# Huangtianyu-caas/MAGOT

Measured on AMD Instinct MI355X. Metric: CDS bases extracted+translated/sec, higher is better.
Workload: dtype u8

## Files before the change

include/magot.h:

```cpp
#ifndef MAGOT_H
#define MAGOT_H

#include <stdint.h>

#ifdef __cplusplus
extern "C" {
#endif

#define MAGOT_ABI_VERSION 1

enum magot_status {
  MAGOT_OK = 0,
  MAGOT_ERR_ARG = -1,
  MAGOT_ERR_HIP = -2,
  MAGOT_ERR_RANGE = -3,
  MAGOT_ERR_STATE = -4,
  MAGOT_ERR_UNSUPPORTED = -5
};

#define MAGOT_OUT_NUC 1u
#define MAGOT_OUT_PEP 2u
#define MAGOT_OUT_GENOME_ORDER 4u

typedef struct magot_exon {
  uint64_t start_rc;
  uint32_t contig;
  uint32_t len;
} magot_exon;

typedef struct magot_tx {
  uint64_t exon_begin;
  uint32_t n_exons;
  uint32_t flags;
} magot_tx;

typedef struct magot_ctx magot_ctx;
typedef struct magot_genome magot_genome;
typedef struct magot_plan magot_plan;

int magot_abi_version(void);

const char* magot_last_error(void);

int magot_device_count(void);

int magot_ctx_create(int device, magot_ctx** out);
void magot_ctx_destroy(magot_ctx* ctx);

int magot_genome_load(magot_ctx* ctx, const uint8_t* const* seqs, const uint64_t* lens,
                      uint32_t n_contigs, magot_genome** out);
#define MAGOT_PACK_HOST 1u
int magot_genome_load_ex(magot_ctx* ctx, const uint8_t* const* seqs, const uint64_t* lens,
                         uint32_t n_contigs, uint32_t flags, magot_genome** out);
int magot_genome_load_fasta(magot_ctx* ctx, const char* text, uint64_t len, int truncate_names,
                            magot_genome** out);
int magot_genome_contigs(const magot_genome* g, uint32_t* n, uint64_t* lens, char* names,
                         uint64_t names_cap, uint64_t* names_len);
int magot_fasta_read(const char* text, uint64_t len, int truncate_names, uint32_t* n,
                     uint64_t* lens, char* names, uint64_t names_cap, uint64_t* names_len,
                     uint8_t* seqs, uint64_t seqs_cap);

int magot_cds_scan(const char* text, uint64_t len, uint64_t* n_seg, uint64_t* seq_bytes,
                   uint64_t* seg_off, uint64_t* hdr_off, uint64_t* hdr_len, uint8_t* seq,
                   uint64_t seq_cap);
int magot_cds_render(const char* text, uint64_t n_seg, const uint64_t* seg_off,
                     const uint64_t* hdr_off, const uint64_t* hdr_len, const uint8_t* pep,
                     const uint64_t* poff, const int64_t* codons, uint8_t* out, uint64_t cap,
                     uint64_t* out_len);

int magot_genome_stats(const magot_genome* g, uint64_t* total_bases, uint64_t* n_exc_runs,
                       uint64_t* device_bytes);
void magot_genome_destroy(magot_genome* g);

int magot_genome_export(const magot_genome* g, uint8_t* meta, uint64_t cap, uint64_t* meta_len,
                        uint64_t* arena_bytes);
int magot_genome_copy_arena(const magot_genome* g, void* dst_dev);
int magot_genome_attach(magot_ctx* ctx, const uint8_t* meta, uint64_t meta_len, void* arena_dev,
                        magot_genome** out);
int magot_genome_wire_ranges(const magot_genome* g, uint64_t* off, uint64_t* len, uint32_t* n);
int magot_genome_attach_wire(magot_ctx* ctx, const uint8_t* meta, uint64_t meta_len,
                             void* arena_dev, magot_genome** out);
int magot_genome_wire_export(const magot_genome* g, void* wire_dev, uint64_t cap,
                             uint64_t* wire_bytes);
int magot_genome_wire_import(magot_ctx* ctx, const uint8_t* meta, uint64_t meta_len,
                             const void* wire_dev, uint64_t wire_bytes, magot_genome** out);

int magot_copy_segments(magot_ctx* ctx, const void* src_dev, uint64_t src_bytes, void* dst_dev,
                        const uint64_t* src_off, const uint64_t* dst_off, uint64_t n);

int magot_plan_create(magot_ctx* ctx, const magot_genome* g, const magot_exon* exons,
                      uint64_t n_exons, const magot_tx* txs, uint64_t n_tx, uint32_t outputs,
                      magot_plan** out, uint64_t* nuc_bytes, uint64_t* pep_bytes);
void magot_plan_destroy(magot_plan* p);

int magot_plan_execute(magot_ctx* ctx, magot_plan* p);

int magot_ctx_sync(magot_ctx* ctx);

int magot_ctx_mark(magot_ctx* ctx, int which);
int magot_ctx_elapsed(magot_ctx* ctx, double* ms);

int magot_ctx_info(const magot_ctx* ctx, int* n_cu, int* extract_blocks_per_cu);

int magot_plan_fetch(magot_ctx* ctx, magot_plan* p, uint8_t* nuc_out, uint64_t* nuc_off,
                     uint8_t* pep_out, uint64_t* pep_off);

int magot_run(magot_ctx* ctx, magot_plan* p, uint8_t* nuc_out, uint64_t* nuc_off,
              uint8_t* pep_out, uint64_t* pep_off);

int magot_plan_time(magot_ctx* ctx, magot_plan* p, int iters, double* avg_ms);
int magot_plan_time_b2b(magot_ctx* ctx, magot_plan* p, int iters, double* avg_ms);

int magot_plan_copy_outputs(magot_ctx* ctx, magot_plan* p, void* nuc_dst_dev, void* pep_dst_dev);

int magot_plan_device_outputs(magot_plan* p, void** nuc_dev, void** pep_dev);

int magot_plan_layout(const magot_plan* p, uint64_t* nuc_start, uint64_t* pep_start);

uint64_t magot_plan_algorithmic_bytes(const magot_plan* p);

int magot_debug_tile_blocks(const uint64_t* ex_g, const uint64_t* ex_out, const uint64_t* tx_nuc,
                            const uint64_t* tx_pep, uint64_t span, uint32_t lane_chunks,
                            const void* tiles, uint64_t n_tiles, uint32_t* geometry, void* blocks,
                            uint64_t* ovf_ex, uint64_t ovf_ex_cap, int64_t* ovf_tx,
                            uint64_t ovf_tx_cap, uint64_t* n_ovf);

int magot_debug_tile_cut(const uint64_t* ex_out, uint64_t n_ex, const uint64_t* tx_nuc,
                         const uint64_t* tx_pep, uint64_t n_rec, uint32_t lane_chunks, void* tiles,
                         uint64_t tiles_cap, uint64_t* n_tiles);

int magot_debug_orf6_tiles(const uint64_t* noff, uint64_t n_rec, const uint64_t* row_start,
                           uint64_t n_rows, uint64_t* t0, uint32_t* r0, uint32_t* e0, uint32_t* m,
                           uint64_t tiles_cap, uint64_t* n_tiles);

int magot_debug_plan(const uint8_t* const* seqs, const uint64_t* lens, uint32_t n_contigs,
                     const magot_exon* exons, uint64_t n_exons, const magot_tx* txs, uint64_t n_tx,
                     uint32_t outputs, uint64_t* info, uint64_t* ex_g, uint64_t* ex_out,
                     uint64_t* tx_nuc, uint64_t* tx_pep, uint64_t* lay_nuc, uint64_t* lay_pep,
                     void* tiles);

int magot_debug_text_index(magot_ctx* ctx, const uint8_t* text, uint64_t len, uint64_t index_len,
                           uint32_t byte, int32_t second_byte, uint64_t* pos_out, uint64_t* n_out,
                           uint64_t* second_count_out);

int magot_debug_text_lines(magot_ctx* ctx, const uint8_t* text, uint64_t len, uint64_t index_len,
                           int check_cr, uint32_t stray_reason, uint64_t* pos_out,
                           uint64_t* n_lines_out, uint64_t* stray_out);

int magot_debug_piece_copy(magot_ctx* ctx, const uint8_t* base, uint64_t base_len,
                           const uint64_t* src, const uint64_t* dst, const uint32_t* len,
                           uint64_t n, uint8_t* out, uint64_t out_len);

#define MAGOT_NO_RECORD 0xFFFFFFFFu
typedef struct magot_text_unit {
  uint64_t text_off;
  uint32_t text_len;
  uint32_t rec;
} magot_text_unit;
int magot_debug_text_assembly(magot_ctx* ctx, const magot_text_unit* units, uint64_t n,
                              const uint8_t* text, uint64_t text_len, const uint64_t* rspan,
                              uint64_t n_rec, const uint8_t* pay, uint64_t pay_len, int protein,
                              uint8_t* out, uint64_t out_len, uint64_t* written);

int magot_revcomp_batch(magot_ctx* ctx, const uint8_t* seqs, const uint64_t* seq_off, uint64_t n,
                        uint8_t* out);

int magot_translate_sizes(const uint64_t* seq_off, uint64_t n, const int32_t* frames,
                          uint64_t* pep_off, int64_t* codons_out);
int magot_translate_batch(magot_ctx* ctx, const uint8_t* seqs, const uint64_t* seq_off, uint64_t n,
                          const int32_t* frames, const uint8_t* strands, const uint8_t* lut64,
                          const uint64_t* pep_off, uint8_t* out);

int magot_revcomp(magot_ctx* ctx, const uint8_t* seq, uint64_t len, uint8_t* out);
int magot_translate(magot_ctx* ctx, const uint8_t* seq, uint64_t len, int frame, int strand,
                    int trimX, uint8_t* out, int64_t* out_len);

int magot_codon_symbols(magot_ctx* ctx, const uint8_t* seq, uint64_t n_codons,
                        const uint8_t* class256, uint32_t n_classes, const uint8_t* lut,
                        uint8_t* out);

int magot_orf6_sizes(const uint64_t* seq_off, uint64_t n, uint64_t* stream_off,
                     uint64_t* stream_len, uint8_t* none_mask);
int magot_orf6_batch(magot_ctx* ctx, const uint8_t* seqs, const uint64_t* seq_off, uint64_t n,
                     const uint8_t* lut64, const uint64_t* stream_off, uint8_t* out);
int magot_debug_orf6_batch(magot_ctx* ctx, const uint8_t* seqs, const uint64_t* seq_off, uint64_t n,
                           const uint8_t* lut64, const uint64_t* stream_off, uint8_t* out,
                           int32_t poison);
typedef struct magot_orf6 magot_orf6;
int magot_plan_orf6(magot_ctx* ctx, magot_plan* p, const uint8_t* lut64, magot_orf6** out,
                    uint64_t* total_res);
int magot_orf6_execute(magot_ctx* ctx, magot_orf6* o);
int magot_orf6_poison(magot_ctx* ctx, magot_orf6* o, uint8_t byte);
int magot_orf6_fetch(magot_ctx* ctx, magot_orf6* o, uint8_t* out, uint64_t* stream_off,
                     uint64_t* stream_len);
int magot_orf6_copy_outputs(magot_ctx* ctx, magot_orf6* o, void* dst_dev);
int magot_orf6_time(magot_ctx* ctx, magot_orf6* o, int iters, double* avg_ms);
int magot_orf6_time_b2b(magot_ctx* ctx, magot_orf6* o, int iters, double* avg_ms);
void magot_orf6_destroy(magot_orf6* o);

#define MAGOT_ORF_FROM_ATG 1u
#define MAGOT_ORF_LONGEST 2u
#define MAGOT_ORF_REC_NONE 1u
#define MAGOT_ORF_REC_NO_LONGEST 2u
typedef struct magot_orfcall magot_orfcall;
uint32_t magot_orfcall_tile(void);
int magot_orfcall_create(magot_ctx* ctx, magot_orf6* o, uint32_t flags, magot_orfcall** out,
                         uint64_t* n_orfs, uint64_t* payload_bytes);
int magot_orfcall_fetch(magot_ctx* ctx, magot_orfcall* c, uint32_t* record, uint8_t* stream,
                        uint32_t* start, uint32_t* length, uint64_t* payload_off,
                        uint8_t* payload, uint8_t* record_flags);
int magot_orfcall_text(magot_ctx* ctx, magot_orfcall* c, const uint64_t* name_off,
                       const uint8_t* names, uint64_t* out_len);
int magot_orfcall_text_fetch(magot_ctx* ctx, magot_orfcall* c, uint8_t* out, uint64_t cap);
int magot_orfcall_time(magot_ctx* ctx, magot_orfcall* c, int text, int iters, double* avg_ms);
void magot_orfcall_destroy(magot_orfcall* c);

typedef struct magot_longorf magot_longorf;
int magot_longorf_create(magot_ctx* ctx, magot_plan* p, const uint8_t* lut64, magot_longorf** out);
int magot_longorf_execute(magot_ctx* ctx, magot_longorf* h, uint64_t* payload_bytes);
int magot_longorf_fetch(magot_ctx* ctx, magot_longorf* h, uint8_t* stream, uint32_t* start,
                        uint32_t* length, uint64_t* payload_off, uint8_t* payload,
                        uint8_t* record_flags);
int magot_longorf_text(magot_ctx* ctx, magot_longorf* h, const uint64_t* name_off,
                       const uint8_t* names, uint64_t n_print, uint64_t* out_len);
int magot_longorf_text_fetch(magot_ctx* ctx, magot_longorf* h, uint8_t* out, uint64_t cap);
int magot_longorf_time(magot_ctx* ctx, magot_longorf* h, int text, int iters, double* avg_ms);
int magot_longorf_params(magot_ctx* ctx, const magot_longorf* h, uint32_t* step, uint64_t* waves);
void magot_longorf_destroy(magot_longorf* h);

#define MAGOT_GFF_PROTEIN 1u
#define MAGOT_GFF_ORDER_PY2 2u
#define MAGOT_GFF_LONGEST 4u
#define MAGOT_GFF_GENOMIC 8u
#define MAGOT_GFF_FROM_EXONS 16u
#define MAGOT_GFF_FOR_WRITE 32u
typedef struct magot_gffplan magot_gffplan;
int magot_gff_plan(const char* gff, uint64_t gff_len, const char* const* seqids,
                   const uint64_t* contig_lens, uint32_t n_contigs, const char* feature,
                   uint32_t flags, magot_gffplan** out, uint64_t* n_exons, uint64_t* n_tx);
int magot_gff_read(const char* gff, uint64_t gff_len, uint32_t flags, magot_gffplan** out);
int magot_gff_lower(magot_gffplan* p, const char* const* seqids, const uint64_t* contig_lens,
                    uint32_t n_contigs, const char* feature, uint32_t flags, uint64_t* n_exons,
                    uint64_t* n_tx);
#define MAGOT_CDS_NAMES_CDS 0u
#define MAGOT_CDS_NAMES_TRANSCRIPT 1u
#define MAGOT_CDS_NAMES_GENE 2u
int magot_gff_lower_cds(magot_gffplan* p, const char* const* seqids, const uint64_t* contig_lens,
                        uint32_t n_contigs, const char* const* filters, uint32_t n_filters,
                        const int64_t* length_filter, uint32_t names_from, uint32_t flags,
                        uint64_t* n_rec, uint64_t* n_groups);
int magot_gffplan_cds_views(const magot_gffplan* p, const uint64_t** name_off,
                            const uint8_t** names, const uint64_t** group_off);
int magot_flank_plan(const char* gff, uint64_t gff_len, const char* const* seqids,
                     const uint64_t* contig_lens, uint32_t n_contigs, const char* feature_type,
                     const char* namefrom, const char* sequence_length, const char* stream,
                     magot_gffplan** out, uint64_t* n_exons, uint64_t* n_tx);
int magot_gffplan_tables(const magot_gffplan* p, magot_exon* exons, magot_tx* txs);
int magot_gffplan_table_views(const magot_gffplan* p, const magot_exon** exons,
                              const magot_tx** txs);
int magot_gffplan_render(const magot_gffplan* p, const uint8_t* nuc, const uint64_t* noff,
                         const uint8_t* pep, const uint64_t* poff, uint8_t* out, uint64_t cap,
                         uint64_t* out_len);
int magot_gffplan_selections(const magot_gffplan* p, uint64_t* n_groups);
void magot_gffplan_destroy(magot_gffplan* p);

typedef struct magot_fasta_text magot_fasta_text;
int magot_fasta_text_create(magot_ctx* ctx, const magot_gffplan* gp, const magot_plan* p,
                            magot_fasta_text** out, uint64_t* max_bytes);
int magot_fasta_text_execute(magot_ctx* ctx, magot_fasta_text* t);
int magot_fasta_text_fetch(magot_ctx* ctx, magot_fasta_text* t, uint8_t* out, uint64_t cap,
                           uint64_t* out_len);
int magot_fasta_text_time(magot_ctx* ctx, magot_fasta_text* t, int iters, double* avg_ms);
void magot_fasta_text_destroy(magot_fasta_text* t);

#define MAGOT_MASK_HARD 1u
#define MAGOT_MASK_KEEP_CASE 2u
typedef struct magot_mask_interval {
  uint32_t contig;
  uint32_t start;
  uint32_t len;
} magot_mask_interval;
typedef struct magot_maskplan magot_maskplan;
typedef struct magot_mask magot_mask;
uint32_t magot_mask_piece(void);
int magot_mask_plan(const char* gff, uint64_t gff_len, const char* const* seqids,
                    const uint64_t* contig_lens, uint32_t n_contigs, const char* feature_type,
                    uint32_t flags, magot_maskplan** out, uint64_t* n_intervals);
int magot_maskplan_table(const magot_maskplan* p, const magot_mask_interval** rows,
                         uint64_t* n_intervals, uint32_t* flags);
void magot_maskplan_destroy(magot_maskplan* p);
int magot_mask_fasta_check(const char* text, uint64_t len, uint32_t n_contigs);
int magot_mask_create(magot_ctx* ctx, const magot_plan* p, const magot_maskplan* mp,
                      const uint32_t* rec_contig, const uint64_t* name_off, const uint8_t* names,
                      magot_mask** out, uint64_t* text_bytes);
int magot_mask_execute(magot_ctx* ctx, magot_mask* m);
int magot_mask_fetch(magot_ctx* ctx, magot_mask* m, uint8_t* out, uint64_t cap);
int magot_mask_coverage_fetch(magot_ctx* ctx, magot_mask* m, uint32_t* words, uint64_t cap_words,
                              uint64_t* n_words);
int magot_mask_time(magot_ctx* ctx, magot_mask* m, int iters, double* paint_ms, double* text_ms);
void magot_mask_destroy(magot_mask* m);

#define MAGOT_TRACK_GC 1u
#define MAGOT_TRACK_REPLACE 2u
typedef struct magot_track magot_track;
typedef struct magot_track_windows magot_track_windows;
uint32_t magot_track_rank_block(void);
int magot_track_create(magot_ctx* ctx, const magot_genome* g, magot_track** out,
                       uint64_t* n_words);
int magot_track_base_class(magot_ctx* ctx, magot_track* t, const magot_genome* g, uint32_t flags);
int magot_track_paint(magot_ctx* ctx, magot_track* t, const magot_mask_interval* rows,
                      uint64_t n_rows, int value);
int magot_track_set_bytes(magot_ctx* ctx, magot_track* t, uint32_t contig, const uint8_t* bytes,
                          uint64_t len);
int magot_track_get_bytes(magot_ctx* ctx, magot_track* t, uint32_t contig, uint8_t* bytes,
                          uint64_t len);
int magot_track_fetch(magot_ctx* ctx, magot_track* t, uint32_t* words, uint64_t cap_words,
                      uint64_t* n_words);
int magot_track_windows_create(magot_ctx* ctx, magot_track* t, uint64_t window, uint64_t jump,
                               const uint8_t* skip, magot_track_windows** out,
                               uint64_t* n_windows, uint64_t* first);
int magot_track_windows_fetch(magot_ctx* ctx, magot_track_windows* w, uint32_t* sums,
                              uint64_t cap);
int magot_track_transitions(magot_ctx* ctx, magot_track_windows* w, uint32_t s_min, uint64_t* n);
int magot_track_transitions_fetch(magot_ctx* ctx, magot_track_windows* w, uint64_t* index,
                                  uint64_t cap);
int magot_track_count(magot_ctx* ctx, magot_track* t, const magot_mask_interval* rows,
                      uint64_t n_rows, uint32_t* ones);
int magot_track_time(magot_ctx* ctx, magot_track* t, magot_track_windows* w, uint32_t s_min,
                     int iters, double* ms5);
void magot_track_windows_destroy(magot_track_windows* w);
void magot_track_destroy(magot_track* t);

#define MAGOT_DEPTH_EMPTY_LINE 1u
#define MAGOT_DEPTH_LEADING_BLANK 2u
#define MAGOT_DEPTH_BAD_BYTE 3u
#define MAGOT_DEPTH_NAME_LONG 4u
#define MAGOT_DEPTH_FEW_FIELDS 5u
#define MAGOT_DEPTH_SIGN 6u
#define MAGOT_DEPTH_NOT_NUMBER 7u
#define MAGOT_DEPTH_NUMBER_RANGE 8u
#define MAGOT_DEPTH_POS_SEQUENCE 9u
#define MAGOT_DEPTH_REPEATED_CONTIG 10u
#define MAGOT_DEPTH_LINE_LONG 11u
#define MAGOT_DEPTH_TOO_MANY_LINES 12u
#define MAGOT_DEPTH_TOO_MANY_RUNS 13u
typedef struct magot_depth magot_depth;
uint32_t magot_depth_block(void);
int magot_depth_parse(magot_ctx* ctx, const char* text, uint64_t len, uint64_t chunk_bytes,
                      uint32_t max_runs, magot_depth** out, uint64_t* n_lines, uint64_t* n_runs,
                      uint32_t* reason, uint64_t* line);
int magot_depth_runs(const magot_depth* t, uint64_t* first, uint64_t* offset, uint32_t* name_len,
                     uint64_t cap);
int magot_depth_values(magot_ctx* ctx, magot_depth* t, uint64_t start, uint64_t n, int32_t* out);
int magot_depth_sums(magot_ctx* ctx, magot_depth* t, const int64_t* start, const int64_t* length,
                     uint64_t n_rows, const uint64_t* group_offsets, uint64_t n_groups,
                     int64_t* sums, int64_t* group_sums);
int magot_depth_time(magot_ctx* ctx, magot_depth* t, int iters, double* ms4,
                     uint64_t* chunk_len);
void magot_depth_destroy(magot_depth* t);

typedef struct magot_fq magot_fq;
uint64_t magot_fq_dense(void);
int magot_fq_parse(magot_ctx* ctx, const char* text, uint64_t len, uint64_t chunk_bytes,
                   magot_fq** out);
int magot_fq_stats(const magot_fq* t, uint64_t* out8, uint32_t* flags);
int magot_fq_histogram(magot_ctx* ctx, magot_fq* t, int64_t* lengths, uint64_t* counts,
                       uint64_t cap, uint64_t* n);
int magot_fq_time(magot_ctx* ctx, magot_fq* t, int iters, double* ms4, uint64_t* chunk_len);
void magot_fq_destroy(magot_fq* t);

#define MAGOT_OVERLAP_NO_SEQ 0xffffffffu
enum {
  MAGOT_OVERLAP_BAD_INT_FIRST = 1,
  MAGOT_OVERLAP_BAD_INT_SECOND = 2,
  MAGOT_OVERLAP_COORD_RANGE = 3,
  MAGOT_OVERLAP_SEQIDS = 4
};
typedef struct magot_overlap magot_overlap;
typedef struct magot_ovplan magot_ovplan;
void magot_overlap_coord_range(int64_t* lo, int64_t* hi);
uint32_t magot_overlap_lane_scan(void);
int magot_overlap_create(magot_ctx* ctx, const uint32_t* seq, const int64_t* p0, const int64_t* p1,
                         uint64_t n, uint32_t n_seq, magot_overlap** out);
int magot_overlap_purge(magot_ctx* ctx, magot_overlap* h, const uint32_t* seq, const int64_t* c0,
                        const int64_t* c1, uint64_t n, uint8_t* drop);
int magot_overlap_counts(magot_ctx* ctx, magot_overlap* h, const uint32_t* seq, const int64_t* q0,
                         const int64_t* q1, uint64_t n, int64_t* counts);
int magot_overlap_time(magot_ctx* ctx, magot_overlap* h, int iters, double* ms6,
                       uint64_t* copy_bytes);
void magot_overlap_destroy(magot_overlap* h);
int magot_overlap_plan(const char* gff1, uint64_t len1, const char* gff2, uint64_t len2,
                       magot_ovplan** out, uint32_t* reason);
int magot_ovplan_table(const magot_ovplan* p, int which, uint64_t* n_lines, uint32_t* n_seq,
                       const uint8_t** flag, const uint32_t** seq, const int64_t** c0,
                       const int64_t** c1, const uint64_t** off, const uint64_t** len);
int magot_ovplan_render(const magot_ovplan* p, const char* gff2, uint64_t len2,
                        const uint8_t* drop, uint8_t* out, uint64_t cap, uint64_t* bytes);
void magot_ovplan_destroy(magot_ovplan* p);

enum {
  MAGOT_PSL_FEW_FIELDS = 1,
  MAGOT_PSL_INTEGER_FORM = 2,
  MAGOT_PSL_NUMBER_RANGE = 3,
  MAGOT_PSL_HASH_COLLISION = 4,
  MAGOT_PSL_TOO_LARGE = 5,
  MAGOT_PSL_TOO_MANY_LINES = 6
};
typedef struct magot_psl magot_psl;
int magot_psl_parse(magot_ctx* ctx, const char* text, uint64_t len, uint32_t hash_bits,
                    uint64_t max_bytes, magot_psl** out, uint32_t* reason, uint64_t* line);
int magot_psl_sizes(const magot_psl* p, uint64_t* n_lines, uint64_t* n_pass, uint64_t* n_data,
                    uint64_t* n_groups);
double magot_psl_upload_ms(const magot_psl* p);
int magot_psl_pass_lines(magot_ctx* ctx, magot_psl* p, uint64_t* off, uint64_t* len);
int magot_psl_groups(magot_ctx* ctx, magot_psl* p, uint64_t* hash, uint32_t* first_line,
                     uint32_t* best_line, int64_t* score, uint64_t* off, uint64_t* len);
int magot_psl_time(magot_ctx* ctx, magot_psl* p, int iters, double* ms8, uint64_t* text_bytes);
void magot_psl_destroy(magot_psl* p);
int magot_psl_order(const uint64_t* hash, uint64_t n, uint64_t* perm);
int magot_psl_render(const char* text, uint64_t len, const uint64_t* off, const uint64_t* row_len,
                     uint64_t n, int whole, uint8_t* out, uint64_t cap, uint64_t* bytes);

typedef struct magot_site magot_site;
int magot_site_create(magot_ctx* ctx, const magot_genome* g, const uint32_t* contig,
// ... 188 lines not shown
```

magot_amd/_lib.py:

```python

import ctypes
import os
import threading

import numpy as np

HERE = os.path.dirname(os.path.abspath(__file__))
LIB_PATH = os.environ.get('MAGOT_LIB') or os.path.join(HERE, 'libmagot.so')

OUT_NUC = 1
OUT_PEP = 2
OUT_GENOME_ORDER = 4

EXON_DTYPE = np.dtype([('start_rc', '<u8'), ('contig', '<u4'), ('len', '<u4')])
TX_DTYPE = np.dtype([('exon_begin', '<u8'), ('n_exons', '<u4'), ('flags', '<u4')])
RC_BIT = np.uint64(1 << 63)

EXPORTS = (
    'magot_abi_version', 'magot_last_error', 'magot_device_count',
    'magot_ctx_create', 'magot_ctx_destroy', 'magot_ctx_sync', 'magot_ctx_info',
    'magot_genome_load', 'magot_genome_stats', 'magot_genome_destroy',
    'magot_plan_create', 'magot_plan_destroy', 'magot_plan_execute', 'magot_plan_fetch',
    'magot_run', 'magot_plan_time', 'magot_plan_time_b2b', 'magot_plan_device_outputs',
    'magot_plan_layout',
    'magot_plan_algorithmic_bytes',
    'magot_revcomp_batch', 'magot_translate_sizes', 'magot_translate_batch',
    'magot_codon_symbols', 'magot_revcomp', 'magot_translate',
    'magot_gff_plan', 'magot_gff_read', 'magot_gff_lower', 'magot_flank_plan',
    'magot_gffplan_tables', 'magot_gffplan_table_views', 'magot_gffplan_render',
    'magot_gffplan_destroy',
    'magot_gffplan_selections', 'magot_cds_scan', 'magot_cds_render',
    'magot_genome_export', 'magot_genome_copy_arena', 'magot_genome_attach',
    'magot_plan_copy_outputs',
    'magot_orf6_sizes', 'magot_orf6_batch', 'magot_plan_orf6', 'magot_orf6_execute',
    'magot_orf6_fetch', 'magot_orf6_time', 'magot_orf6_time_b2b', 'magot_orf6_destroy',
    'magot_genome_load_fasta', 'magot_genome_contigs', 'magot_fasta_read',
    'magot_fasta_text_create', 'magot_fasta_text_execute', 'magot_fasta_text_fetch',
    'magot_fasta_text_time', 'magot_fasta_text_destroy',
    'magot_genome_load_ex', 'magot_genome_wire_ranges', 'magot_genome_attach_wire',
    'magot_copy_segments', 'magot_ctx_mark', 'magot_ctx_elapsed', 'magot_orf6_copy_outputs',
    'magot_genome_wire_export', 'magot_genome_wire_import',
    'magot_debug_tile_blocks', 'magot_debug_tile_cut', 'magot_debug_plan',
    'magot_debug_text_index', 'magot_debug_text_lines', 'magot_debug_piece_copy',
    'magot_debug_text_assembly', 'magot_debug_orf6_tiles', 'magot_debug_orf6_batch',
    'magot_orf6_poison',
    'magot_orfcall_tile', 'magot_orfcall_create', 'magot_orfcall_fetch', 'magot_orfcall_text',
    'magot_orfcall_text_fetch', 'magot_orfcall_time', 'magot_orfcall_destroy',
    'magot_mask_piece', 'magot_mask_plan', 'magot_maskplan_table', 'magot_maskplan_destroy',
    'magot_mask_fasta_check', 'magot_mask_create', 'magot_mask_execute', 'magot_mask_fetch',
    'magot_mask_coverage_fetch', 'magot_mask_time', 'magot_mask_destroy',
    'magot_track_rank_block', 'magot_track_create', 'magot_track_base_class', 'magot_track_paint',
    'magot_track_set_bytes', 'magot_track_get_bytes', 'magot_track_fetch',
    'magot_track_windows_create', 'magot_track_windows_fetch', 'magot_track_transitions',
    'magot_track_transitions_fetch', 'magot_track_count', 'magot_track_time',
    'magot_track_windows_destroy', 'magot_track_destroy',
    'magot_depth_block', 'magot_depth_parse', 'magot_depth_runs', 'magot_depth_values',
    'magot_depth_sums', 'magot_depth_time', 'magot_depth_destroy',
    'magot_fq_dense', 'magot_fq_parse', 'magot_fq_stats', 'magot_fq_histogram', 'magot_fq_time',
    'magot_fq_destroy',
    'magot_overlap_coord_range', 'magot_overlap_lane_scan', 'magot_overlap_create',
    'magot_overlap_purge', 'magot_overlap_counts', 'magot_overlap_time', 'magot_overlap_destroy',
    'magot_overlap_plan', 'magot_ovplan_table', 'magot_ovplan_render', 'magot_ovplan_destroy',
    'magot_psl_parse', 'magot_psl_sizes', 'magot_psl_upload_ms', 'magot_psl_pass_lines',
    'magot_psl_groups', 'magot_psl_time', 'magot_psl_destroy', 'magot_psl_order',
    'magot_psl_render',
    'magot_site_create', 'magot_site_execute', 'magot_site_counts', 'magot_site_time',
    'magot_site_params', 'magot_site_destroy', 'magot_site_render', 'magot_site_text_free',
    'magot_vcf_parse', 'magot_vcf_sizes', 'magot_vcf_upload_ms', 'magot_vcf_header_lines',
    'magot_vcf_runs', 'magot_vcf_resolve', 'magot_vcf_tables', 'magot_vcf_last_of',
    'magot_vcf_count', 'magot_vcf_time', 'magot_vcf_params', 'magot_vcf_destroy',
    'magot_vcf_render',
    'magot_fastarec_parse', 'magot_fastarec_sizes', 'magot_fastarec_upload_ms',
    'magot_fastarec_records', 'magot_fastarec_keys', 'magot_fastarec_exclude',
    'magot_fastarec_render', 'magot_fastarec_render_fetch', 'magot_fastarec_time',
    'magot_fastarec_params', 'magot_fastarec_destroy',
    'magot_rename_parse', 'magot_rename_sizes', 'magot_rename_upload_ms', 'magot_rename_hits',
    'magot_rename_render', 'magot_rename_render_fetch', 'magot_rename_time',
    'magot_rename_params', 'magot_rename_destroy',
    'magot_tabcut_parse', 'magot_tabcut_sizes', 'magot_tabcut_upload_ms', 'magot_tabcut_rows',
    'magot_tabcut_render', 'magot_tabcut_render_fetch', 'magot_tabcut_time',
    'magot_tabcut_params', 'magot_tabcut_destroy',
    'magot_gff_lower_write', 'magot_gffplan_write_views',
    'magot_gffwrite_open', 'magot_gffwrite_sizes', 'magot_gffwrite_upload_ms',
    'magot_gffwrite_render', 'magot_gffwrite_render_fetch', 'magot_gffwrite_time',
    'magot_gffwrite_params', 'magot_gffwrite_destroy',
    'magot_longorf_create', 'magot_longorf_execute', 'magot_longorf_fetch', 'magot_longorf_text',
    'magot_longorf_text_fetch', 'magot_longorf_time', 'magot_longorf_params',
    'magot_longorf_destroy', 'magot_gff_lower_cds', 'magot_gffplan_cds_views',
)

ERR_ARG = -1
ERR_HIP = -2
ERR_RANGE = -3
ERR_STATE = -4
ERR_UNSUPPORTED = -5
GFF_PROTEIN = 1
GFF_ORDER_PY2 = 2
GFF_LONGEST = 4
GFF_GENOMIC = 8
GFF_FROM_EXONS = 16
GFF_FOR_WRITE = 32
GFF_FORMATS = {'simple gff3': 0, 'gtf': 1, 'exon added gff3': 2}
CDS_NAMES = {'CDS': 0, 'transcript': 1, 'gene': 2}
GFFROW_LINE, GFFROW_EXON_TWIN, GFFROW_GTF, GFFROW_MADE_PARENT = 0, 1, 2, 3
GFFROW_HAS_PARENT = 0x100
PACK_HOST = 1
ORF_FROM_ATG = 1
ORF_LONGEST = 2
ORF_REC_NONE = 1
ORF_REC_NO_LONGEST = 2
MASK_HARD = 1
MASK_KEEP_CASE = 2
TRACK_GC = 1
TRACK_REPLACE = 2
DEPTH_REASONS = (None, 'empty line', 'leading blank', 'byte outside the grammar',
                 'name longer than 255 bytes', 'fewer than three fields', 'sign on a number',
                 'not a number', 'number out of range', 'position out of sequence',
                 'repeated contig', 'line longer than a chunk', 'more than 2^31-1 lines',
                 'too many runs')
OVERLAP_NO_SEQ = 0xffffffff
OVERLAP_REASONS = (None, 'bad integer in the first file', 'bad integer in the second file',
                   'coordinate beyond the key range', 'too many seqids')
PSL_REASONS = (None, 'few_fields', 'integer_form', 'number_range', 'hash_collision', 'too_large',
               'too_many_lines')
VCF_REASONS = (None, 'no_header', 'many_headers', 'header_after_data', 'no_samples',
               'too_many_samples', 'no_data', 'field_count', 'chrom_form', 'pos_form', 'pos_range',
               'no_gt', 'empty_gt', 'equals_fixed', 'too_large', 'too_many_lines', 'too_many_runs',
               'line_too_long', 'too_many_counts', 'carriage_return')
FASTAREC_REASONS = (None, 'leading_text', 'stray_cr', 'long_name', 'hash_collision', 'too_large',
                    'too_many_lines')
FASTAREC_STYLES = {'fasta': 0, 'tab': 1}
RENAME_REASONS = (None, 'too_large', 'hash_collision', 'table_too_large')
TABCUT_REASONS = (None, 'stray_cr', 'too_large', 'too_many_lines')
TABCUT_LITERAL, TABCUT_FIELDS = 0, 1
TABCUT_SHORT = {'skip': 0, 'error': 1}
TABCUT_SKIPPED, TABCUT_KEPT, TABCUT_SHORT_LINE = 0, 1, 2
TABCUT_ITEM_DTYPE = np.dtype([('kind', '<u4'), ('a', '<u4'), ('b', '<u4')])
GFFWRITE_REASONS = (None, 'too_large', 'score', 'columns')
GFFROW_DTYPE = np.dtype([('line_off', '<u8'), ('lo', '<i8'), ('hi', '<i8'), ('id_off', '<u8'),
                         ('parent_off', '<u8'), ('type_off', '<u8'), ('id_len', '<u4'),
                         ('parent_len', '<u4'), ('type_len', '<u4'), ('kind', '<u4')])
MASK_INTERVAL_DTYPE = np.dtype([('contig', '<u4'), ('start', '<u4'), ('len', '<u4')])


class MagotError(RuntimeError):
    """A libmagot call failed (status + magot_last_error text)."""


_u8p = ctypes.POINTER(ctypes.c_uint8)
_u64p = ctypes.POINTER(ctypes.c_uint64)
_i64p = ctypes.POINTER(ctypes.c_int64)
_i32p = ctypes.POINTER(ctypes.c_int32)
_vp = ctypes.c_void_p

_lib = None
_lib_lock = threading.RLock()


def _declare(lib):
    sig = {
        'magot_abi_version': (ctypes.c_int, []),
        'magot_last_error': (ctypes.c_char_p, []),
        'magot_device_count': (ctypes.c_int, []),
        'magot_ctx_create': (ctypes.c_int, [ctypes.c_int, ctypes.POINTER(_vp)]),
        'magot_ctx_destroy': (None, [_vp]),
        'magot_ctx_sync': (ctypes.c_int, [_vp]),
        'magot_ctx_info': (ctypes.c_int, [_vp, ctypes.POINTER(ctypes.c_int),
                                          ctypes.POINTER(ctypes.c_int)]),
        'magot_genome_load': (ctypes.c_int, [_vp, ctypes.POINTER(_u8p), _u64p, ctypes.c_uint32,
                                             ctypes.POINTER(_vp)]),
        'magot_genome_stats': (ctypes.c_int, [_vp, _u64p, _u64p, _u64p]),
        'magot_genome_destroy': (None, [_vp]),
        'magot_plan_create': (ctypes.c_int, [_vp, _vp, _vp, ctypes.c_uint64, _vp, ctypes.c_uint64,
                                             ctypes.c_uint32, ctypes.POINTER(_vp), _u64p, _u64p]),
        'magot_plan_destroy': (None, [_vp]),
        'magot_plan_execute': (ctypes.c_int, [_vp, _vp]),
        'magot_plan_fetch': (ctypes.c_int, [_vp, _vp, _vp, _vp, _vp, _vp]),
        'magot_run': (ctypes.c_int, [_vp, _vp, _vp, _vp, _vp, _vp]),
        'magot_plan_time': (ctypes.c_int, [_vp, _vp, ctypes.c_int,
                                           ctypes.POINTER(ctypes.c_double)]),
        'magot_plan_time_b2b': (ctypes.c_int, [_vp, _vp, ctypes.c_int,
                                               ctypes.POINTER(ctypes.c_double)]),
        'magot_plan_layout': (ctypes.c_int, [_vp, _vp, _vp]),
        'magot_plan_device_outputs': (ctypes.c_int, [_vp, ctypes.POINTER(_vp),
                                                     ctypes.POINTER(_vp)]),
        'magot_plan_algorithmic_bytes': (ctypes.c_uint64, [_vp]),
        'magot_debug_tile_blocks': (ctypes.c_int, [_vp, _vp, _vp, _vp, ctypes.c_uint64,
                                                   ctypes.c_uint32, _vp, ctypes.c_uint64, _vp, _vp,
                                                   _vp, ctypes.c_uint64, _vp, ctypes.c_uint64,
                                                   _vp]),
        'magot_debug_tile_cut': (ctypes.c_int, [_vp, ctypes.c_uint64, _vp, _vp, ctypes.c_uint64,
                                                ctypes.c_uint32, _vp, ctypes.c_uint64, _vp]),
        'magot_debug_plan': (ctypes.c_int, [_vp, _vp, ctypes.c_uint32, _vp, ctypes.c_uint64, _vp,
                                            ctypes.c_uint64, ctypes.c_uint32, _vp, _vp, _vp, _vp,
                                            _vp, _vp, _vp, _vp]),
        'magot_debug_text_index': (ctypes.c_int, [_vp, _vp, ctypes.c_uint64, ctypes.c_uint64,
                                                  ctypes.c_uint32, ctypes.c_int32, _vp, _u64p,
                                                  _u64p]),
        'magot_debug_text_lines': (ctypes.c_int, [_vp, _vp, ctypes.c_uint64, ctypes.c_uint64,
                                                  ctypes.c_int, ctypes.c_uint32, _vp, _u64p,
                                                  _u64p]),
        'magot_debug_piece_copy': (ctypes.c_int, [_vp, _vp, ctypes.c_uint64, _vp, _vp, _vp,
                                                  ctypes.c_uint64, _vp, ctypes.c_uint64]),
        'magot_debug_text_assembly': (ctypes.c_int, [_vp, _vp, ctypes.c_uint64, _vp,
                                                     ctypes.c_uint64, _vp, ctypes.c_uint64, _vp,
                                                     ctypes.c_uint64, ctypes.c_int, _vp,
                                                     ctypes.c_uint64, _u64p]),
        'magot_revcomp_batch': (ctypes.c_int, [_vp, _vp, _vp, ctypes.c_uint64, _vp]),
        'magot_translate_sizes': (ctypes.c_int, [_vp, ctypes.c_uint64, _vp, _vp, _vp]),
        'magot_translate_batch': (ctypes.c_int, [_vp, _vp, _vp, ctypes.c_uint64, _vp, _vp, _vp,
                                                 _vp, _vp]),
        'magot_codon_symbols': (ctypes.c_int, [_vp, _vp, ctypes.c_uint64, _vp, ctypes.c_uint32,
                                               _vp, _vp]),
        'magot_revcomp': (ctypes.c_int, [_vp, _vp, ctypes.c_uint64, _vp]),
        'magot_translate': (ctypes.c_int, [_vp, _vp, ctypes.c_uint64, ctypes.c_int, ctypes.c_int,
                                           ctypes.c_int, _vp, _i64p]),
        'magot_gff_plan': (ctypes.c_int, [_vp, ctypes.c_uint64,
                                          ctypes.POINTER(ctypes.c_char_p), _u64p, ctypes.c_uint32,
                                          ctypes.c_char_p, ctypes.c_uint32, ctypes.POINTER(_vp),
                                          _u64p, _u64p]),
        'magot_gff_read': (ctypes.c_int, [_vp, ctypes.c_uint64, ctypes.c_uint32,
                                          ctypes.POINTER(_vp)]),
        'magot_gff_lower': (ctypes.c_int, [_vp, ctypes.POINTER(ctypes.c_char_p), _u64p,
                                           ctypes.c_uint32, ctypes.c_char_p, ctypes.c_uint32,
                                           _u64p, _u64p]),
        'magot_flank_plan': (ctypes.c_int, [_vp, ctypes.c_uint64,
                                            ctypes.POINTER(ctypes.c_char_p), _u64p,
                                            ctypes.c_uint32, ctypes.c_char_p, ctypes.c_char_p,
                                            ctypes.c_char_p, ctypes.c_char_p, ctypes.POINTER(_vp),
                                            _u64p, _u64p]),
        'magot_gffplan_tables': (ctypes.c_int, [_vp, _vp, _vp]),
        'magot_gffplan_table_views': (ctypes.c_int, [_vp, ctypes.POINTER(_vp),
                                                     ctypes.POINTER(_vp)]),
        'magot_gffplan_render': (ctypes.c_int, [_vp, _vp, _vp, _vp, _vp, _vp, ctypes.c_uint64,
                                                _u64p]),
        'magot_gffplan_destroy': (None, [_vp]),
        'magot_gffplan_selections': (ctypes.c_int, [_vp, _u64p]),
        'magot_cds_scan': (ctypes.c_int, [_vp, ctypes.c_uint64, _u64p, _u64p, _vp, _vp, _vp, _vp,
                                          ctypes.c_uint64]),
        'magot_cds_render': (ctypes.c_int, [_vp, ctypes.c_uint64, _vp, _vp, _vp, _vp, _vp, _vp,
                                            _vp, ctypes.c_uint64, _u64p]),
        'magot_genome_export': (ctypes.c_int, [_vp, _vp, ctypes.c_uint64, _u64p, _u64p]),
        'magot_genome_copy_arena': (ctypes.c_int, [_vp, _vp]),
        'magot_genome_attach': (ctypes.c_int, [_vp, _vp, ctypes.c_uint64, _vp,
                                               ctypes.POINTER(_vp)]),
        'magot_plan_copy_outputs': (ctypes.c_int, [_vp, _vp, _vp, _vp]),
        'magot_orf6_sizes': (ctypes.c_int, [_vp, ctypes.c_uint64, _vp, _vp, _vp]),
        'magot_orf6_batch': (ctypes.c_int, [_vp, _vp, _vp, ctypes.c_uint64, _vp, _vp, _vp]),
        'magot_debug_orf6_batch': (ctypes.c_int, [_vp, _vp, _vp, ctypes.c_uint64, _vp, _vp, _vp,
                                                  ctypes.c_int32]),
        'magot_debug_orf6_tiles': (ctypes.c_int, [_vp, ctypes.c_uint64, _vp, ctypes.c_uint64, _vp,
                                                  _vp, _vp, _vp, ctypes.c_uint64, _u64p]),
        'magot_orf6_poison': (ctypes.c_int, [_vp, _vp, ctypes.c_uint8]),
        'magot_plan_orf6': (ctypes.c_int, [_vp, _vp, _vp, ctypes.POINTER(_vp), _u64p]),
        'magot_orf6_execute': (ctypes.c_int, [_vp, _vp]),
        'magot_orf6_fetch': (ctypes.c_int, [_vp, _vp, _vp, _vp, _vp]),
        'magot_orf6_time': (ctypes.c_int, [_vp, _vp, ctypes.c_int,
                                           ctypes.POINTER(ctypes.c_double)]),
        'magot_orf6_time_b2b': (ctypes.c_int, [_vp, _vp, ctypes.c_int,
                                               ctypes.POINTER(ctypes.c_double)]),
        'magot_orf6_destroy': (None, [_vp]),
        'magot_fasta_text_create': (ctypes.c_int, [_vp, _vp, _vp, ctypes.POINTER(_vp), _u64p]),
        'magot_fasta_text_execute': (ctypes.c_int, [_vp, _vp]),
        'magot_fasta_text_fetch': (ctypes.c_int, [_vp, _vp, _vp, ctypes.c_uint64, _u64p]),
        'magot_fasta_text_time': (ctypes.c_int, [_vp, _vp, ctypes.c_int,
                                                 ctypes.POINTER(ctypes.c_double)]),
        'magot_fasta_text_destroy': (None, [_vp]),
        'magot_genome_load_fasta': (ctypes.c_int, [_vp, _vp, ctypes.c_uint64,
                                                   ctypes.c_int, ctypes.POINTER(_vp)]),
        'magot_genome_contigs': (ctypes.c_int, [_vp, ctypes.POINTER(ctypes.c_uint32), _vp, _vp,
                                                ctypes.c_uint64, _u64p]),
        'magot_genome_load_ex': (ctypes.c_int, [_vp, ctypes.POINTER(_u8p), _u64p, ctypes.c_uint32,
                                                ctypes.c_uint32, ctypes.POINTER(_vp)]),
        'magot_genome_wire_ranges': (ctypes.c_int, [_vp, _u64p, _u64p,
                                                    ctypes.POINTER(ctypes.c_uint32)]),
        'magot_genome_attach_wire': (ctypes.c_int, [_vp, _vp, ctypes.c_uint64, _vp,
                                                    ctypes.POINTER(_vp)]),
        'magot_genome_wire_export': (ctypes.c_int, [_vp, _vp, ctypes.c_uint64, _u64p]),
        'magot_genome_wire_import': (ctypes.c_int, [_vp, _vp, ctypes.c_uint64, _vp,
                                                    ctypes.c_uint64, ctypes.POINTER(_vp)]),
        'magot_copy_segments': (ctypes.c_int, [_vp, _vp, ctypes.c_uint64, _vp, _vp, _vp,
                                               ctypes.c_uint64]),
        'magot_ctx_mark': (ctypes.c_int, [_vp, ctypes.c_int]),
        'magot_orf6_copy_outputs': (ctypes.c_int, [_vp, _vp, _vp]),
        'magot_ctx_elapsed': (ctypes.c_int, [_vp, ctypes.POINTER(ctypes.c_double)]),
        'magot_fasta_read': (ctypes.c_int, [_vp, ctypes.c_uint64, ctypes.c_int,
                                            ctypes.POINTER(ctypes.c_uint32), _vp, _vp,
                                            ctypes.c_uint64, _u64p, _vp, ctypes.c_uint64]),
        'magot_orfcall_tile': (ctypes.c_uint32, []),
        'magot_orfcall_create': (ctypes.c_int, [_vp, _vp, ctypes.c_uint32, ctypes.POINTER(_vp),
                                                _u64p, _u64p]),
        'magot_orfcall_fetch': (ctypes.c_int, [_vp, _vp, _vp, _vp, _vp, _vp, _vp, _vp, _vp]),
        'magot_orfcall_text': (ctypes.c_int, [_vp, _vp, _vp, _vp, _u64p]),
        'magot_orfcall_text_fetch': (ctypes.c_int, [_vp, _vp, _vp, ctypes.c_uint64]),
        'magot_orfcall_time': (ctypes.c_int, [_vp, _vp, ctypes.c_int, ctypes.c_int,
                                              ctypes.POINTER(ctypes.c_double)]),
        'magot_orfcall_destroy': (None, [_vp]),
        'magot_longorf_create': (ctypes.c_int, [_vp, _vp, _vp, ctypes.POINTER(_vp)]),
        'magot_longorf_execute': (ctypes.c_int, [_vp, _vp, _u64p]),
        'magot_longorf_fetch': (ctypes.c_int, [_vp, _vp, _vp, _vp, _vp, _vp, _vp, _vp]),
        'magot_longorf_text': (ctypes.c_int, [_vp, _vp, _vp, _vp, ctypes.c_uint64, _u64p]),
        'magot_longorf_text_fetch': (ctypes.c_int, [_vp, _vp, _vp, ctypes.c_uint64]),
        'magot_longorf_time': (ctypes.c_int, [_vp, _vp, ctypes.c_int, ctypes.c_int,
                                              ctypes.POINTER(ctypes.c_double)]),
        'magot_longorf_params': (ctypes.c_int, [_vp, _vp, ctypes.POINTER(ctypes.c_uint32), _u64p]),
        'magot_longorf_destroy': (None, [_vp]),
        'magot_gff_lower_cds': (ctypes.c_int, [_vp, ctypes.POINTER(ctypes.c_char_p), _u64p,
                                               ctypes.c_uint32, ctypes.POINTER(ctypes.c_char_p),
                                               ctypes.c_uint32, _i64p, ctypes.c_uint32,
                                               ctypes.c_uint32, _u64p, _u64p]),
        'magot_gffplan_cds_views': (ctypes.c_int, [_vp, ctypes.POINTER(_vp), ctypes.POINTER(_vp),
                                                   ctypes.POINTER(_vp)]),
        'magot_mask_piece': (ctypes.c_uint32, []),
        'magot_mask_plan': (ctypes.c_int, [_vp, ctypes.c_uint64, ctypes.POINTER(ctypes.c_char_p),
                                           _u64p, ctypes.c_uint32, ctypes.c_char_p,
                                           ctypes.c_uint32, ctypes.POINTER(_vp), _u64p]),
        'magot_maskplan_table': (ctypes.c_int, [_vp, ctypes.POINTER(_vp), _u64p,
                                                ctypes.POINTER(ctypes.c_uint32)]),
        'magot_maskplan_destroy': (None, [_vp]),
        'magot_mask_fasta_check': (ctypes.c_int, [_vp, ctypes.c_uint64, ctypes.c_uint32]),
        'magot_mask_create': (ctypes.c_int, [_vp, _vp, _vp, _vp, _vp, _vp, ctypes.POINTER(_vp),
                                             _u64p]),
        'magot_mask_execute': (ctypes.c_int, [_vp, _vp]),
        'magot_mask_fetch': (ctypes.c_int, [_vp, _vp, _vp, ctypes.c_uint64]),
        'magot_mask_coverage_fetch': (ctypes.c_int, [_vp, _vp, _vp, ctypes.c_uint64, _u64p]),
        'magot_mask_time': (ctypes.c_int, [_vp, _vp, ctypes.c_int,
                                           ctypes.POINTER(ctypes.c_double),
                                           ctypes.POINTER(ctypes.c_double)]),
        'magot_mask_destroy': (None, [_vp]),
        'magot_track_rank_block': (ctypes.c_uint32, []),
        'magot_track_create': (ctypes.c_int, [_vp, _vp, ctypes.POINTER(_vp), _u64p]),
        'magot_track_base_class': (ctypes.c_int, [_vp, _vp, _vp, ctypes.c_uint32]),
        'magot_track_paint': (ctypes.c_int, [_vp, _vp, _vp, ctypes.c_uint64, ctypes.c_int]),
        'magot_track_set_bytes': (ctypes.c_int, [_vp, _vp, ctypes.c_uint32, _vp,
                                                 ctypes.c_uint64]),
        'magot_track_get_bytes': (ctypes.c_int, [_vp, _vp, ctypes.c_uint32, _vp,
                                                 ctypes.c_uint64]),
        'magot_track_fetch': (ctypes.c_int, [_vp, _vp, _vp, ctypes.c_uint64, _u64p]),
        'magot_track_windows_create': (ctypes.c_int, [_vp, _vp, ctypes.c_uint64, ctypes.c_uint64,
                                                      _vp, ctypes.POINTER(_vp), _u64p, _vp]),
        'magot_track_windows_fetch': (ctypes.c_int, [_vp, _vp, _vp, ctypes.c_uint64]),
        'magot_track_transitions': (ctypes.c_int, [_vp, _vp, ctypes.c_uint32, _u64p]),
        'magot_track_transitions_fetch': (ctypes.c_int, [_vp, _vp, _vp, ctypes.c_uint64]),
        'magot_track_count': (ctypes.c_int, [_vp, _vp, _vp, ctypes.c_uint64, _vp]),
        'magot_track_time': (ctypes.c_int, [_vp, _vp, _vp, ctypes.c_uint32, ctypes.c_int, _vp]),
        'magot_track_windows_destroy': (None, [_vp]),
        'magot_track_destroy': (None, [_vp]),
        'magot_depth_block': (ctypes.c_uint32, []),
        'magot_depth_parse': (ctypes.c_int, [_vp, _vp, ctypes.c_uint64, ctypes.c_uint64,
                                             ctypes.c_uint32, ctypes.POINTER(_vp), _u64p, _u64p,
                                             ctypes.POINTER(ctypes.c_uint32), _u64p]),
        'magot_depth_runs': (ctypes.c_int, [_vp, _vp, _vp, _vp, ctypes.c_uint64]),
        'magot_depth_values': (ctypes.c_int, [_vp, _vp, ctypes.c_uint64, ctypes.c_uint64, _vp]),
        'magot_depth_sums': (ctypes.c_int, [_vp, _vp, _vp, _vp, ctypes.c_uint64, _vp,
                                            ctypes.c_uint64, _vp, _vp]),
        'magot_depth_time': (ctypes.c_int, [_vp, _vp, ctypes.c_int, _vp, _u64p]),
        'magot_depth_destroy': (None, [_vp]),
        'magot_fq_dense': (ctypes.c_uint64, []),
        'magot_fq_parse': (ctypes.c_int, [_vp, _vp, ctypes.c_uint64, ctypes.c_uint64,
                                          ctypes.POINTER(_vp)]),
        'magot_fq_stats': (ctypes.c_int, [_vp, _vp, ctypes.POINTER(ctypes.c_uint32)]),
        'magot_fq_histogram': (ctypes.c_int, [_vp, _vp, _vp, _vp, ctypes.c_uint64, _u64p]),
        'magot_fq_time': (ctypes.c_int, [_vp, _vp, ctypes.c_int, _vp, _u64p]),
        'magot_fq_destroy': (None, [_vp]),
        'magot_overlap_coord_range': (None, [_i64p, _i64p]),
        'magot_overlap_lane_scan': (ctypes.c_uint32, []),
        'magot_overlap_create': (ctypes.c_int, [_vp, _vp, _vp, _vp, ctypes.c_uint64,
                                                ctypes.c_uint32, ctypes.POINTER(_vp)]),
        'magot_overlap_purge': (ctypes.c_int, [_vp, _vp, _vp, _vp, _vp, ctypes.c_uint64, _vp]),
        'magot_overlap_counts': (ctypes.c_int, [_vp, _vp, _vp, _vp, _vp, ctypes.c_uint64, _vp]),
        'magot_overlap_time': (ctypes.c_int, [_vp, _vp, ctypes.c_int, _vp, _u64p]),
        'magot_overlap_destroy': (None, [_vp]),
        'magot_overlap_plan': (ctypes.c_int, [_vp, ctypes.c_uint64, _vp, ctypes.c_uint64,
                                              ctypes.POINTER(_vp),
                                              ctypes.POINTER(ctypes.c_uint32)]),
        'magot_ovplan_table': (ctypes.c_int, [_vp, ctypes.c_int, _u64p,
                                              ctypes.POINTER(ctypes.c_uint32)] +
                               [ctypes.POINTER(_vp)] * 6),
        'magot_ovplan_render': (ctypes.c_int, [_vp, _vp, ctypes.c_uint64, _vp, _vp,
                                               ctypes.c_uint64, _u64p]),
        'magot_ovplan_destroy': (None, [_vp]),
        'magot_psl_parse': (ctypes.c_int, [_vp, _vp, ctypes.c_uint64, ctypes.c_uint32,
                                           ctypes.c_uint64, ctypes.POINTER(_vp),
                                           ctypes.POINTER(ctypes.c_uint32), _u64p]),
        'magot_psl_sizes': (ctypes.c_int, [_vp, _u64p, _u64p, _u64p, _u64p]),
        'magot_psl_upload_ms': (ctypes.c_double, [_vp]),
        'magot_psl_pass_lines': (ctypes.c_int, [_vp, _vp, _vp, _vp]),
        'magot_psl_groups': (ctypes.c_int, [_vp, _vp, _vp, _vp, _vp, _vp, _vp, _vp]),
        'magot_psl_time': (ctypes.c_int, [_vp, _vp, ctypes.c_int, _vp, _u64p]),
        'magot_psl_destroy': (None, [_vp]),
        'magot_psl_order': (ctypes.c_int, [_vp, ctypes.c_uint64, _vp]),
        'magot_psl_render': (ctypes.c_int, [_vp, ctypes.c_uint64, _vp, _vp, ctypes.c_uint64,
                                            ctypes.c_int, _vp, ctypes.c_uint64, _u64p]),
        'magot_site_create': (ctypes.c_int, [_vp, _vp, _vp, _vp, ctypes.c_uint64, ctypes.c_uint64,
                                             ctypes.POINTER(_vp)]),
        'magot_site_execute': (ctypes.c_int, [_vp, _vp]),
        'magot_site_counts': (ctypes.c_int, [_vp, _vp, _vp]),
        'magot_site_time': (ctypes.c_int, [_vp, _vp, ctypes.c_int, ctypes.POINTER(ctypes.c_double)]),
        'magot_site_params': (None, [ctypes.POINTER(ctypes.c_uint32)] * 5),
        'magot_site_destroy': (None, [_vp]),
        'magot_site_render': (ctypes.c_int, [_vp, ctypes.c_uint64, ctypes.c_uint32,
                                             ctypes.POINTER(_vp), _u64p, _u64p]),
        'magot_site_text_free': (None, [_vp]),
        'magot_vcf_parse': (ctypes.c_int, [_vp, _vp, ctypes.c_uint64, ctypes.c_uint64,
                                           ctypes.c_uint32, ctypes.c_uint32, ctypes.POINTER(_vp),
                                           ctypes.POINTER(ctypes.c_uint32), _u64p]),
        'magot_vcf_sizes': (ctypes.c_int, [_vp, _u64p, _u64p, _u64p,
                                           ctypes.POINTER(ctypes.c_uint32),
                                           ctypes.POINTER(ctypes.c_uint32), _u64p, _u64p, _u64p]),
        'magot_vcf_upload_ms': (ctypes.c_double, [_vp]),
        'magot_vcf_header_lines': (ctypes.c_int, [_vp, _vp, _vp, _vp]),
        'magot_vcf_runs': (ctypes.c_int, [_vp, _vp, _vp, _vp]),
        'magot_vcf_resolve': (ctypes.c_int, [_vp, _vp, _vp, ctypes.c_uint64]),
        'magot_vcf_tables': (ctypes.c_int, [_vp] * 8),
        'magot_vcf_last_of': (ctypes.c_int, [_vp, _vp, ctypes.c_uint64, _u64p, _u64p, _u64p]),
        'magot_vcf_count': (ctypes.c_int, [_vp, _vp, _vp, _vp, _vp, ctypes.c_uint64, _vp, _vp,
                                           ctypes.POINTER(ctypes.c_uint32),
                                           ctypes.POINTER(ctypes.c_uint32)]),
        'magot_vcf_time': (ctypes.c_int, [_vp, _vp, ctypes.c_int, _vp, _u64p]),
        'magot_vcf_params': (None, [ctypes.POINTER(ctypes.c_uint32)] * 3 + [_u64p]),
        'magot_vcf_destroy': (None, [_vp]),
        'magot_vcf_render': (ctypes.c_int, [_vp, _vp, _vp, _vp, ctypes.c_uint64, ctypes.c_uint32,
                                            _vp, ctypes.c_uint32, ctypes.c_uint32,
                                            ctypes.POINTER(_vp), _u64p]),
        'magot_fastarec_parse': (ctypes.c_int, [_vp, _vp, ctypes.c_uint64, ctypes.c_uint32,
                                                ctypes.c_uint64, ctypes.POINTER(_vp),
                                                ctypes.POINTER(ctypes.c_uint32), _u64p]),
        'magot_fastarec_sizes': (ctypes.c_int, [_vp, _u64p, _u64p, _u64p, _u64p]),
        'magot_fastarec_upload_ms': (ctypes.c_double, [_vp]),
        'magot_fastarec_records': (ctypes.c_int, [_vp] * 11),
        'magot_fastarec_keys': (ctypes.c_int, [_vp] * 6),
        'magot_fastarec_exclude': (ctypes.c_int, [_vp, _vp, _vp, ctypes.c_uint64, _vp,
                                                  ctypes.c_uint64, ctypes.c_int, _vp]),
        'magot_fastarec_render': (ctypes.c_int, [_vp, _vp, _vp, ctypes.c_uint64, ctypes.c_uint32,
                                                 _u64p]),
        'magot_fastarec_render_fetch': (ctypes.c_int, [_vp, _vp, _vp, ctypes.c_uint64]),
        'magot_fastarec_time': (ctypes.c_int, [_vp, _vp, ctypes.c_int, _vp, _u64p, _u64p]),
        'magot_fastarec_params': (None, [ctypes.POINTER(ctypes.c_uint32)] * 3),
        'magot_fastarec_destroy': (None, [_vp]),
        'magot_rename_parse': (ctypes.c_int, [_vp, _vp, ctypes.c_uint64, _vp, _vp, _vp, _vp, _vp,
                                              ctypes.c_uint64, ctypes.c_uint32, ctypes.c_uint32,
                                              ctypes.c_uint64, ctypes.POINTER(_vp),
                                              ctypes.POINTER(ctypes.c_uint32)]),
        'magot_rename_sizes': (ctypes.c_int, [_vp, _u64p, _u64p, _u64p, _u64p]),
        'magot_rename_upload_ms': (ctypes.c_double, [_vp]),
        'magot_rename_hits': (ctypes.c_int, [_vp] * 4),
        'magot_rename_render': (ctypes.c_int, [_vp, _vp, _u64p]),
        'magot_rename_render_fetch': (ctypes.c_int, [_vp, _vp, _vp, ctypes.c_uint64]),
        'magot_rename_time': (ctypes.c_int, [_vp, _vp, ctypes.c_int, _vp, _u64p, _u64p]),
        'magot_rename_params': (None, [ctypes.POINTER(ctypes.c_uint32)] * 3),
        'magot_rename_destroy': (None, [_vp]),
        'magot_tabcut_parse': (ctypes.c_int, [_vp, _vp, ctypes.c_uint64, _vp, ctypes.c_uint32, _vp,
                                              ctypes.c_uint64, ctypes.c_uint32, ctypes.c_uint32,
                                              ctypes.c_uint32, ctypes.c_uint64,
                                              ctypes.POINTER(_vp),
                                              ctypes.POINTER(ctypes.c_uint32)]),
        'magot_tabcut_sizes': (ctypes.c_int, [_vp] + [_u64p] * 6),
        'magot_tabcut_upload_ms': (ctypes.c_double, [_vp]),
        'magot_tabcut_rows': (ctypes.c_int, [_vp] * 4),
        'magot_tabcut_render': (ctypes.c_int, [_vp, _vp, _u64p]),
        'magot_tabcut_render_fetch': (ctypes.c_int, [_vp, _vp, _vp, ctypes.c_uint64]),
        'magot_tabcut_time': (ctypes.c_int, [_vp, _vp, ctypes.c_int, _vp, _u64p, _u64p]),
        'magot_tabcut_params': (None, [ctypes.POINTER(ctypes.c_uint32)] * 3),
        'magot_tabcut_destroy': (None, [_vp]),
        'magot_gff_lower_write': (ctypes.c_int, [_vp, ctypes.c_uint32, ctypes.c_uint32, _u64p,
                                                 _u64p]),
        'magot_gffplan_write_views': (ctypes.c_int, [_vp, ctypes.POINTER(_vp), _u64p,
                                                     ctypes.POINTER(_vp), _u64p]),
        'magot_gffwrite_open': (ctypes.c_int, [_vp, _vp, ctypes.c_uint64, _vp, ctypes.c_uint64,
                                               _vp, ctypes.c_uint64, ctypes.c_uint64,
                                               ctypes.POINTER(_vp),
                                               ctypes.POINTER(ctypes.c_uint32), _u64p]),
        'magot_gffwrite_sizes': (ctypes.c_int, [_vp, _u64p, _u64p]),
        'magot_gffwrite_upload_ms': (ctypes.c_double, [_vp]),
        'magot_gffwrite_render': (ctypes.c_int, [_vp, _vp, _u64p]),
        'magot_gffwrite_render_fetch': (ctypes.c_int, [_vp, _vp, _vp, ctypes.c_uint64]),
        'magot_gffwrite_time': (ctypes.c_int, [_vp, _vp, ctypes.c_int, _vp, _u64p, _u64p]),
        'magot_gffwrite_params': (None, [ctypes.POINTER(ctypes.c_uint32)] * 3),
        'magot_gffwrite_destroy': (None, [_vp]),
    }
    for name, (res, args) in sig.items():
        fn = getattr(lib, name)
        fn.restype = res
        fn.argtypes = args
    return lib


def lib():
    global _lib
    if _lib is None:
# ... 74 lines not shown
```

magot_amd/csrc/abi_plan.hip:

```cpp
#include <cstdio>
#include <cstdlib>

#include "abi_internal.h"

using namespace magot;

namespace {

struct HostPiece {
  uint64_t dev_off;
  const void* src;
  uint64_t bytes;
};

int upload_pieces(magot_ctx* ctx, char* dev, const std::vector<HostPiece>& pieces) {
  std::lock_guard<std::mutex> lock(ctx->pin_mu);
  if (int rc = ensure_pin_ring(ctx)) return rc;
  const unsigned nt = host_threads();
  uint64_t k = 0;
  for (const HostPiece& pc : pieces)
    for (uint64_t q0 = 0; q0 < pc.bytes; q0 += kPinRing, ++k) {
      const int b = (int)(k & 1);
      const uint64_t q1 = std::min(pc.bytes, q0 + kPinRing);
      MAGOT_HIP_TRY(hipEventSynchronize(ctx->pin_ev[b]));
      const char* src = static_cast<const char*>(pc.src) + q0;
      uint8_t* ring = ctx->pin[b];
      parallel_ranges(q1 - q0, q1 - q0 >= (4ull << 20) ? nt : 1u,
                      [&](uint64_t lo, uint64_t hi, unsigned) { memcpy(ring + lo, src + lo, hi - lo); });
      MAGOT_HIP_TRY(hipMemcpyAsync(dev + pc.dev_off + q0, ring, q1 - q0, hipMemcpyHostToDevice,
                                   ctx->stream));
      MAGOT_HIP_TRY(hipEventRecord(ctx->pin_ev[b], ctx->stream));
    }
  MAGOT_HIP_TRY(hipStreamSynchronize(ctx->stream));
  return MAGOT_OK;
}

template <class F>
int upload_generated(magot_ctx* ctx, char* dev, uint64_t n, uint64_t item, unsigned threads, F fill) {
  std::lock_guard<std::mutex> lock(ctx->pin_mu);
  if (int rc = ensure_pin_ring(ctx)) return rc;
  const uint64_t per = kPinRing / item;
  for (uint64_t i0 = 0, k = 0; i0 < n; i0 += per, ++k) {
    const int b = (int)(k & 1);
    const uint64_t i1 = std::min(n, i0 + per);
    MAGOT_HIP_TRY(hipEventSynchronize(ctx->pin_ev[b]));
    uint8_t* ring = ctx->pin[b];
    parallel_ranges(i1 - i0, (i1 - i0) * item >= (1ull << 20) ? threads : 1u,
                    [&](uint64_t lo, uint64_t hi, unsigned) { fill(i0 + lo, i0 + hi, ring + lo * item); });
    MAGOT_HIP_TRY(hipMemcpyAsync(dev + i0 * item, ring, (i1 - i0) * item, hipMemcpyHostToDevice,
                                 ctx->stream));
    MAGOT_HIP_TRY(hipEventRecord(ctx->pin_ev[b], ctx->stream));
  }
  return MAGOT_OK;
}

int plan_reassemble(magot_ctx* ctx, const magot_plan* p, bool residues, void* dst) {
  if (!p->n_tx) return MAGOT_OK;
  launch_segments_copy(residues ? p->args.pep : p->args.nuc,
                       residues ? p->d_lay_pep : p->d_lay_nuc,
                       residues ? p->d_pep_off : p->d_nuc_off, p->n_tx,
                       static_cast<uint8_t*>(dst), ctx->stream);
  MAGOT_HIP_TRY(hipGetLastError());
  return MAGOT_OK;
}

constexpr uint64_t kFetchBatchBytes = 256ull << 20;

uint64_t fetch_batch_bytes() {
  const char* e = std::getenv("MAGOT_FETCH_BATCH_BYTES");
  const uint64_t v = e ? strtoull(e, nullptr, 10) : 0;
  return v ? v : kFetchBatchBytes;
}

int plan_fetch_reordered(magot_ctx* ctx, const magot_plan* p, bool residues, uint8_t* host) {
  const std::vector<uint64_t>& off = residues ? p->pep_off : p->nuc_off;
  const uint64_t T = p->n_tx;
  if (!T || off[T] == 0) return MAGOT_OK;
  uint64_t longest = 0;
  for (uint64_t t = 0; t < T; ++t) longest = std::max(longest, off[t + 1] - off[t]);
  const uint64_t cap = std::max(std::min(off[T], fetch_batch_bytes()), longest);
  DevBuf scratch;
  MAGOT_HIP_TRY(hipMalloc(&scratch.p, cap + 16));
  uint8_t* S = static_cast<uint8_t*>(scratch.p);
  const uint8_t* src = residues ? p->args.pep : p->args.nuc;
  const uint64_t* lay = residues ? p->d_lay_pep : p->d_lay_nuc;
  const uint64_t* doff = residues ? p->d_pep_off : p->d_nuc_off;
  for (uint64_t r0 = 0; r0 < T;) {
    uint64_t r1 = r0 + 1;
    while (r1 < T && off[r1 + 1] - off[r0] <= cap) ++r1;
    const uint64_t base = off[r0], bytes = off[r1] - base;
    if (bytes) {
      launch_segments_copy(src, lay + r0, doff + r0, r1 - r0, S - (base & ~15ull), ctx->stream);
      MAGOT_HIP_TRY(hipGetLastError());
      MAGOT_HIP_TRY(hipMemcpyAsync(host + base, S + (base & 15), bytes, hipMemcpyDeviceToHost,
                                   ctx->stream));
    }
    r0 = r1;
  }
  MAGOT_HIP_TRY(hipStreamSynchronize(ctx->stream));
  return MAGOT_OK;
}

}

extern "C" {

int magot_plan_create(magot_ctx* ctx, const magot_genome* g, const magot_exon* exons,
                      uint64_t n_exons, const magot_tx* txs, uint64_t n_tx, uint32_t outputs,
                      magot_plan** out, uint64_t* nuc_bytes, uint64_t* pep_bytes) {
  if (int rc = bind(ctx)) return rc;
  if (!g || !out) {
    set_error("magot_plan_create: null argument");
    return MAGOT_ERR_ARG;
  }
  if (int rc = plan_check_tables(exons, n_exons, txs, n_tx, outputs)) return rc;
  *out = nullptr;
  Lap lap("MAGOT_PLAN_TIMING", "plan");
  const PlanInput in{GenomeView{g->contig_base.data(), g->contig_len.data(), g->contig_base.size(),
                                g->span, g->host_runs.data(), g->host_dir.data()},
                     exons, n_exons, txs, n_tx, plan_options(outputs)};
  const bool by_genome = in.opt.by_genome;
  PlanCount cnt;
  if (int rc = plan_count(in, &cnt)) return rc;
  const uint64_t T = n_tx, B = cnt.B, P = cnt.P;
  const uint64_t out_nuc = (in.opt.outputs & MAGOT_OUT_NUC) ? B + 64 : 64;
  const uint64_t out_pep = (in.opt.outputs & MAGOT_OUT_PEP) ? P + 64 : 64;
  const uint64_t out_bytes = ((out_nuc + 255) & ~255ull) + out_pep;
  AsyncAlloc out_alloc(ctx->device, out_bytes);
  TilePlan pl;
  if (int rc = plan_build(in, std::move(cnt), lap, &pl)) return rc;
  const uint32_t n_tiles = (uint32_t)pl.tiles.size();
  const TileGeometry geo = pl.geo;

  std::unique_ptr<magot_plan> p(new magot_plan());
  p->ctx = ctx;
  p->g = g;
  Carve cv;
  const uint64_t o_blocks = cv.take(&p->args.blocks, (uint64_t)n_tiles * geo.stride);
  const uint64_t o_ovf_ex = cv.take(&p->args.ovf_ex, pl.n_ovf_ex + 1);
  const uint64_t o_ovf_tx = cv.take(&p->args.ovf_tx, pl.n_ovf_tx + 1);
  const uint64_t lay_rows = by_genome ? T : 0;
  const uint64_t o_lay_nuc = cv.take<uint64_t>(lay_rows);
  const uint64_t o_rec_nuc = cv.take<uint64_t>(by_genome ? T + 1 : 0);
  const uint64_t o_lay_pep = cv.take<uint64_t>(lay_rows);
  const uint64_t o_rec_pep = cv.take<uint64_t>(by_genome ? T + 1 : 0);
  MAGOT_HIP_TRY(hipMalloc(&p->arena, cv.used));
  cv.place(p->arena);
  p->arena_bytes = cv.used;
  const hipError_t out_err = out_alloc.take(&p->out_arena);
  MAGOT_HIP_TRY(out_err);
  p->out_bytes = out_bytes;
  lap("malloc");
  char* base = static_cast<char*>(p->arena);
  HostBuf<uint64_t> ovf_ex(pl.n_ovf_ex + 1);
  HostBuf<TxRow> ovf_tx(pl.n_ovf_tx + 1);
  ovf_ex[pl.n_ovf_ex] = 0;
  ovf_tx[pl.n_ovf_tx] = TxRow{0, 0};
  const TileTables tb{pl.ex_g.data(), pl.ex_out.data(), pl.tn.data(), pl.tp.data(), g->span,
                      pl.lane_chunks};
  if (int rc = upload_generated(
          ctx, base + o_blocks, n_tiles, geo.stride, n_tiles >= (1u << 12) ? pl.nth : 1u,
          [&](uint64_t t0, uint64_t t1, uint8_t* dst) {
            for (uint64_t t = t0; t < t1; ++t)
              pack_tile_block(tb, geo, pl.tiles[t], pl.ovf_at[2 * t], pl.ovf_at[2 * t + 1],
                              dst + (t - t0) * geo.stride, ovf_ex.data(), ovf_tx.data());
          }))
    return rc;
  lap("blocks");
  std::vector<HostPiece> pieces = {{o_ovf_ex, ovf_ex.data(), (pl.n_ovf_ex + 1) * 8},
                                   {o_ovf_tx, ovf_tx.data(), (pl.n_ovf_tx + 1) * sizeof(TxRow)}};
  if (by_genome) {
    pieces.push_back({o_lay_nuc, pl.lay_nuc.data(), T * 8});
    pieces.push_back({o_rec_nuc, pl.nuc_off.data(), (T + 1) * 8});
    pieces.push_back({o_lay_pep, pl.lay_pep.data(), T * 8});
    pieces.push_back({o_rec_pep, pl.pep_off.data(), (T + 1) * 8});
  }
  if (int rc = upload_pieces(ctx, base, pieces)) return rc;
  if (by_genome) {
    p->genome_order = true;
    p->d_lay_nuc = reinterpret_cast<const uint64_t*>(base + o_lay_nuc);
    p->d_nuc_off = reinterpret_cast<const uint64_t*>(base + o_rec_nuc);
    p->d_lay_pep = reinterpret_cast<const uint64_t*>(base + o_lay_pep);
    p->d_pep_off = reinterpret_cast<const uint64_t*>(base + o_rec_pep);
  }
  lap("upload");
  if (lap.on) {
    uint64_t up = (uint64_t)n_tiles * geo.stride;
    for (const HostPiece& pc : pieces) up += pc.bytes;
    fprintf(stderr,
            "[plan] tiles %u, block rows %u + %u (%u bytes), overflow rows %llu + %llu, arena %llu "
            "bytes, uploaded %llu\n",
            n_tiles, geo.ex_rows, geo.tx_rows, geo.stride, (unsigned long long)pl.n_ovf_ex,
            (unsigned long long)pl.n_ovf_tx, (unsigned long long)cv.used, (unsigned long long)up);
  }

  ExtractArgs& a = p->args;
  a.nib = g->nib;
  a.span = g->span;
  a.runs = g->runs;
  a.dir = g->dir;
  a.blk = geo;
  a.nuc = static_cast<uint8_t*>(p->out_arena);
  a.pep = static_cast<uint8_t*>(p->out_arena) + ((out_nuc + 255) & ~255ull);
  a.total_nuc = B;
  a.total_pep = P;
  a.n_tiles = n_tiles;
  a.outputs = in.opt.outputs;
  a.lane_chunks = pl.lane_chunks;
  if (const char* dbg = std::getenv("MAGOT_DEBUG_PATHS")) {
    const int v = std::atoi(dbg);
    if (v & 1) a.outputs |= kDebugSlowNuc;
    if (v & 2) a.outputs |= kDebugSlowPep;
  }
  uint8_t lut[64];
  standard_lut(lut);
  std::memcpy(a.lut, lut, 64);

  p->nuc_off = std::move(pl.nuc_off);
  p->pep_off = std::move(pl.pep_off);
  p->lay_nuc = std::move(pl.lay_nuc);
  p->lay_pep = std::move(pl.lay_pep);
  p->n_exons = n_exons;
  p->n_ex_c = pl.Ec;
  p->n_tx = T;
  if (!by_genome) {
    p->host_ex_g = std::move(pl.ex_g.p);
    p->host_ex_out = std::move(pl.ex_out.p);
  }
  if (nuc_bytes) *nuc_bytes = B;
  if (pep_bytes) *pep_bytes = P;
  *out = p.release();
  return MAGOT_OK;
}

void magot_plan_destroy(magot_plan* p) {
  if (!p) return;
  if (p->ctx) (void)hipSetDevice(p->ctx->device);
  if (p->arena) (void)hipFree(p->arena);
  if (p->out_arena) (void)hipFree(p->out_arena);
  delete p;
}

int magot_plan_execute(magot_ctx* ctx, magot_plan* p) {
  if (int rc = bind(ctx)) return rc;
  if (!p) {
    set_error("magot_plan_execute: null plan");
    return MAGOT_ERR_ARG;
  }
  launch_extract(p->args, ctx->stream);
  MAGOT_HIP_TRY(hipGetLastError());
  p->executed = true;
  return MAGOT_OK;
}

int magot_plan_fetch(magot_ctx* ctx, magot_plan* p, uint8_t* nuc_out, uint64_t* nuc_off,
                     uint8_t* pep_out, uint64_t* pep_off) {
  if (int rc = bind(ctx)) return rc;
  if (!p) {
    set_error("magot_plan_fetch: null plan");
    return MAGOT_ERR_ARG;
  }
  if (!p->executed) {
    set_error("magot_plan_fetch: plan not executed");
    return MAGOT_ERR_STATE;
  }
  MAGOT_HIP_TRY(hipStreamSynchronize(ctx->stream));
  if ((nuc_out && p->args.total_nuc && !(p->args.outputs & MAGOT_OUT_NUC)) ||
      (pep_out && p->args.total_pep && !(p->args.outputs & MAGOT_OUT_PEP))) {
    set_error(std::string("magot_plan_fetch: plan built without ") +
              (nuc_out && !(p->args.outputs & MAGOT_OUT_NUC) ? "MAGOT_OUT_NUC" : "MAGOT_OUT_PEP"));
    return MAGOT_ERR_STATE;
  }
  const bool want_nuc = nuc_out && p->args.total_nuc, want_pep = pep_out && p->args.total_pep;
  if (want_nuc) {
    if (p->genome_order) {
      if (int rc = plan_fetch_reordered(ctx, p, false, nuc_out)) return rc;
    } else {
      MAGOT_HIP_TRY(hipMemcpyAsync(nuc_out, p->args.nuc, p->args.total_nuc,
                                   hipMemcpyDeviceToHost, ctx->stream));
      MAGOT_HIP_TRY(hipStreamSynchronize(ctx->stream));
    }
  }
  if (want_pep) {
    if (p->genome_order) {
      if (int rc = plan_fetch_reordered(ctx, p, true, pep_out)) return rc;
    } else {
      MAGOT_HIP_TRY(hipMemcpyAsync(pep_out, p->args.pep, p->args.total_pep,
                                   hipMemcpyDeviceToHost, ctx->stream));
      MAGOT_HIP_TRY(hipStreamSynchronize(ctx->stream));
    }
  }
  if (nuc_off) std::memcpy(nuc_off, p->nuc_off.data(), p->nuc_off.size() * 8);
  if (pep_off) std::memcpy(pep_off, p->pep_off.data(), p->pep_off.size() * 8);
  return MAGOT_OK;
}

int magot_run(magot_ctx* ctx, magot_plan* p, uint8_t* nuc_out, uint64_t* nuc_off, uint8_t* pep_out,
              uint64_t* pep_off) {
  if (int rc = magot_plan_execute(ctx, p)) return rc;
  return magot_plan_fetch(ctx, p, nuc_out, nuc_off, pep_out, pep_off);
}

int magot_plan_time(magot_ctx* ctx, magot_plan* p, int iters, double* avg_ms) {
  if (int rc = bind(ctx)) return rc;
  if (!p || iters <= 0 || !avg_ms) {
    set_error("magot_plan_time: bad argument");
    return MAGOT_ERR_ARG;
  }
  if (int rc = time_passes(ctx, iters, 1, avg_ms, [&](int) {
        launch_extract(p->args, ctx->stream);
        return hipGetLastError();
      }))
    return rc;
  p->executed = true;
  return MAGOT_OK;
}

int magot_plan_time_b2b(magot_ctx* ctx, magot_plan* p, int iters, double* avg_ms) {
  if (int rc = bind(ctx)) return rc;
  if (!p || iters <= 0 || !avg_ms) {
    set_error("magot_plan_time_b2b: bad argument");
    return MAGOT_ERR_ARG;
  }
  double ms = 0.0;
  if (int rc = time_pass(ctx, &ms, [&] {
        for (int i = 0; i < iters; ++i) launch_extract(p->args, ctx->stream);
        return hipGetLastError();
      }))
    return rc;
  p->executed = true;
  *avg_ms = ms / iters;
  return MAGOT_OK;
}

int magot_plan_copy_outputs(magot_ctx* ctx, magot_plan* p, void* nuc_dst_dev, void* pep_dst_dev) {
  if (int rc = bind(ctx)) return rc;
  if (!p) {
    set_error("magot_plan_copy_outputs: null plan");
    return MAGOT_ERR_ARG;
  }
  if (p->genome_order && ((nuc_dst_dev && (reinterpret_cast<uintptr_t>(nuc_dst_dev) & 15)) ||
                          (pep_dst_dev && (reinterpret_cast<uintptr_t>(pep_dst_dev) & 15)))) {
    set_error("magot_plan_copy_outputs: a genome-ordered plan needs 16-byte aligned destinations");
    return MAGOT_ERR_ARG;
  }
  if (nuc_dst_dev && p->args.total_nuc && (p->args.outputs & MAGOT_OUT_NUC)) {
    if (p->genome_order) {
      if (int rc = plan_reassemble(ctx, p, false, nuc_dst_dev)) return rc;
    } else {
      MAGOT_HIP_TRY(hipMemcpyAsync(nuc_dst_dev, p->args.nuc, p->args.total_nuc,
                                   hipMemcpyDeviceToDevice, ctx->stream));
    }
  }
  if (pep_dst_dev && p->args.total_pep && (p->args.outputs & MAGOT_OUT_PEP)) {
    if (p->genome_order) {
      if (int rc = plan_reassemble(ctx, p, true, pep_dst_dev)) return rc;
    } else {
      MAGOT_HIP_TRY(hipMemcpyAsync(pep_dst_dev, p->args.pep, p->args.total_pep,
                                   hipMemcpyDeviceToDevice, ctx->stream));
    }
  }
  MAGOT_HIP_TRY(hipStreamSynchronize(ctx->stream));
  return MAGOT_OK;
}

int magot_plan_layout(const magot_plan* p, uint64_t* nuc_start, uint64_t* pep_start) {
  if (!p) {
    set_error("magot_plan_layout: null plan");
    return MAGOT_ERR_ARG;
  }
  const uint64_t T = p->n_tx;
  if (nuc_start) {
    if (p->genome_order) std::memcpy(nuc_start, p->lay_nuc.data(), T * 8);
    else std::memcpy(nuc_start, p->nuc_off.data(), T * 8);
  }
  if (pep_start) {
    if (p->genome_order) std::memcpy(pep_start, p->lay_pep.data(), T * 8);
    else std::memcpy(pep_start, p->pep_off.data(), T * 8);
  }
  return MAGOT_OK;
}

int magot_plan_device_outputs(magot_plan* p, void** nuc_dev, void** pep_dev) {
  if (!p) {
    set_error("magot_plan_device_outputs: null plan");
    return MAGOT_ERR_ARG;
  }
  if (nuc_dev) *nuc_dev = p->args.nuc;
  if (pep_dev) *pep_dev = p->args.pep;
  return MAGOT_OK;
}

uint64_t magot_plan_algorithmic_bytes(const magot_plan* p) {
  if (!p) return 0;
  const uint64_t B = p->args.total_nuc, P = p->args.total_pep;
  uint64_t bytes = (B + 3) / 4 + 16 * p->n_exons + 32 * p->n_tx;
  if (p->args.outputs & MAGOT_OUT_NUC) bytes += B;
  if (p->args.outputs & MAGOT_OUT_PEP) bytes += P;
  return bytes;
}

}


struct magot_fasta_text {
  magot_ctx* ctx = nullptr;
  const magot_plan* plan = nullptr;
  void* arena = nullptr;
  const TextUnit* units = nullptr;
  const uint64_t* roff = nullptr;
  const uint8_t* text = nullptr;
  uint64_t* len = nullptr;
  uint64_t* psrc = nullptr;
  uint64_t* end = nullptr;
  void* scan_tmp = nullptr;
  size_t scan_bytes = 0;
  uint8_t* out = nullptr;
  uint64_t n_units = 0, cap = 0;
  int protein = 0;
  void launch(hipStream_t s) const {
    launch_text_assembly(units, n_units, roff, protein ? plan->args.pep : plan->args.nuc,
                         protein, text, len, psrc, end, scan_tmp, scan_bytes, out, s);
  }
};

extern "C" {

int magot_fasta_text_create(magot_ctx* ctx, const magot_gffplan* gp, const magot_plan* p,
                            magot_fasta_text** out, uint64_t* max_bytes) {
  if (int rc = bind(ctx)) return rc;
  if (!gp || !p || !out) {
    set_error("magot_fasta_text_create: null argument");
    return MAGOT_ERR_ARG;
  }
  *out = nullptr;
  const std::string* text = nullptr;
  std::vector<TextUnit> units;
  bool protein = false;
  uint64_t n_rec = 0;
  if (!gffplan_units(gp, &text, &units, &protein, &n_rec)) {
    set_error("magot_fasta_text_create: too many records, or longest=True protein choices "
              "(magot_gffplan_selections; render those on the host)");
    return MAGOT_ERR_ARG;
  }
  if (n_rec != p->n_tx || !(p->args.outputs & (protein ? MAGOT_OUT_PEP : MAGOT_OUT_NUC))) {
    set_error("magot_fasta_text_create: the plan was not built from this skeleton's tables");
    return MAGOT_ERR_ARG;
  }
  std::unique_ptr<magot_fasta_text> o(new magot_fasta_text());
  o->ctx = ctx;
  o->plan = p;
  o->protein = protein;
  o->n_units = units.size();
  const std::vector<uint64_t>& roff = protein ? p->pep_off : p->nuc_off;
  const std::vector<uint64_t>& lay = p->genome_order ? (protein ? p->lay_pep : p->lay_nuc) : roff;
  std::vector<uint64_t> span(2 * n_rec);
  for (uint64_t r = 0; r < n_rec; ++r) {
    span[2 * r] = lay[r];
    span[2 * r + 1] = lay[r] + (roff[r + 1] - roff[r]);
  }
  o->cap = text->size() + (roff.empty() ? 0 : roff.back());
  o->scan_bytes = text_scan_bytes(o->n_units);
// ... 79 lines not shown
```

magot_amd/csrc/common.h:

```cpp
#pragma once

#include <hip/hip_runtime.h>

#include <cstdint>
#include <memory>
#include <string>
#include <vector>

#include "../../include/magot.h"
#include "hostutil.h"
#include "textindex.h"

namespace magot {

constexpr uint64_t kOrigin = 64;
constexpr int kDirShift = 12;
constexpr uint32_t kDirClean = 0x80000000u;
constexpr uint64_t kRcBit = 1ull << 63;

struct ExcRun {
  uint64_t start;
  uint32_t len;
  uint32_t byte;
};
static_assert(sizeof(ExcRun) == 16, "ExcRun must be 16 bytes");

struct HostPacked {
  std::unique_ptr<uint32_t[]> nib;
  uint64_t nib_words = 0;
  uint64_t span = 0;
  std::vector<ExcRun> runs;
  std::vector<uint32_t> dir;
  std::vector<uint64_t> contig_base;
  std::vector<uint64_t> contig_len;
  uint64_t extent = 0;
};

struct ContigSource {
  const uint8_t* ptr;
  uint64_t len;
  uint64_t width;
  uint32_t term;
};

struct FastaContigs {
  std::vector<std::string> names;
  std::vector<ContigSource> src;
  std::vector<std::string> storage;
};
int scan_fasta(const char* text, uint64_t n, bool truncate, FastaContigs* out);
void copy_contig(const ContigSource& src, uint8_t* dst);

void pack_genome(const ContigSource* src, uint32_t n, HostPacked* out);
void pack_layout(const ContigSource* src, uint32_t n, HostPacked* out);
void exc_runs_directory(HostPacked* out);
void copy_bases(const ContigSource& src, uint64_t pos, uint64_t n, uint8_t* dst);

size_t devpack_scan_bytes(uint64_t n_groups);
hipError_t launch_run_count(const uint8_t* raw, uint64_t n, uint32_t* count, uint64_t* slot,
                            void* scan_tmp, size_t scan_bytes, hipStream_t s);
void launch_run_write(const uint8_t* raw, uint64_t n, const uint64_t* slot, uint64_t* run_start,
                      uint64_t* run_end, uint8_t* run_byte, hipStream_t s);
void launch_nib_pack(const uint8_t* raw, uint64_t n, uint32_t* nib, uint64_t nib_words,
                     hipStream_t s);
void launch_segments_copy(const uint8_t* src, const uint64_t* src_off, const uint64_t* dst_off,
                          uint64_t n, uint8_t* dst, hipStream_t s);

constexpr uint64_t kWireMagic = 0x3257544f47414d00ull;
struct WireHeader {
  uint64_t magic;
  uint64_t span;
  uint64_t n_mask;
  uint64_t n_mdir;
  uint64_t o_code2, o_mask, o_mdir, o_exc;
  uint64_t exc_bytes;
  uint64_t total;
  uint64_t meta_hash;
};
size_t wire_scan_bytes(uint64_t groups);
hipError_t launch_wire_count(const uint32_t* nib, uint64_t span, uint32_t* count, uint64_t* slot,
                             void* scan_tmp, size_t scan_bytes, hipStream_t s);
void launch_wire_runs(const uint32_t* nib, uint64_t span, const uint64_t* slot, uint32_t* runs,
                      hipStream_t s);
void launch_wire_mdir(const uint32_t* runs, uint64_t n, uint64_t n_blocks, uint32_t* mdir,
                      hipStream_t s);
void launch_wire_unpack(const uint32_t* code2, const uint32_t* mask, uint64_t n_mask,
                        const uint32_t* mdir, uint64_t n_mdir, const ExcRun* exc, uint64_t n_exc,
                        const uint32_t* edir, uint64_t n_edir, uint64_t span, uint32_t* nib,
                        hipStream_t s);

constexpr int kThreads = 256;
constexpr int kWaves = kThreads / 64;
constexpr int kChunk = 16;
constexpr int kLaneChunksLarge = 6, kLaneChunksSmall = 3;
constexpr int tile_bytes(int lane_chunks) { return (64 * lane_chunks - 3) * 16; }
constexpr uint64_t kSmallTilePlan = 40000;
constexpr uint64_t kTileAlign = 128;
constexpr int kPepPerLane = 2;
constexpr int kHalo = 3 * kChunk;
constexpr int kExonCap = 128;
static_assert((kExonCap & (kExonCap - 1)) == 0, "kExonCap must be a power of two (row index masks)");
constexpr int kTxCap = 64;
constexpr int kPepSlots = 64 * kPepPerLane;
constexpr uint64_t kExcBit = 1ull << 62;
constexpr uint64_t kSlowLitBit = 1ull << 61;
constexpr uint64_t kExFlagBits = kRcBit | kExcBit | kSlowLitBit;

__host__ __device__ constexpr uint32_t lit_class(uint32_t b) {
  return b == 'N' ? 0u : b == 'n' ? 1u : b == '-' ? 2u : b == 'R' ? 3u : b == 'Y' ? 4u
       : b == 'K' ? 5u : b == 'M' ? 6u : 7u;
}
constexpr uint32_t kLitLo = 0x522D6E4Eu;
constexpr uint32_t kLitHi = 0x4E4D4B59u;

__device__ __forceinline__ void store16(uint8_t* dst, uint4 v) {
  typedef uint32_t u32x4 __attribute__((ext_vector_type(4)));
  u32x4 x = {v.x, v.y, v.z, v.w};
  __builtin_nontemporal_store(x, reinterpret_cast<u32x4*>(dst));
}

constexpr uint32_t kDebugSlowNuc = 1u << 8;
constexpr uint32_t kDebugSlowPep = 1u << 9;

struct TileRec {
  uint64_t T0, T1, Q0, Q1;
  uint32_t e1, e2, j1, j2;
};
static_assert(sizeof(TileRec) == 48, "TileRec is 48 bytes");

constexpr uint32_t kFlagRc = 1u;
constexpr uint32_t kFlagExc = 2u;
constexpr uint32_t kFlagSlowLit = 4u;
constexpr uint32_t kBlkExMax = 64;
constexpr uint32_t kBlkTxMax = 14;
constexpr uint32_t kBlkNoChunk = 511;
struct TxRow {
  int64_t tn, tp;
};
struct TileHead {
  uint64_t T0, Q0;
  uint32_t span_res;
  uint32_t counts;
  uint32_t ovf_ex;
  uint32_t ovf_tx;
};
static_assert(sizeof(TileHead) == 32, "TileHead is 32 bytes");
struct TileGeometry {
  uint32_t ex_rows, tx_rows;
  uint32_t stride;
};
constexpr uint32_t tile_block_stride(uint32_t ex_rows, uint32_t tx_rows) {
  return ((uint32_t)sizeof(TileHead) + 8u * ex_rows + 16u * tx_rows + 15u) & ~15u;
}
static_assert(tile_block_stride(kBlkExMax, kBlkTxMax) == 768, "the largest block is six lines");
static_assert(kExonCap <= (int)kBlkExMax + 64 && kTxCap + 1 <= 1 + 64,
              "one inline and one overflow row per lane");
static_assert(tile_bytes(kLaneChunksLarge) + 4 * kHalo < (1 << 13) &&
              (tile_bytes(kLaneChunksLarge) + kHalo + kChunk - 1) / kChunk < (int)kBlkNoChunk,
              "interval row fields");
struct TileTables {
  const uint64_t* ex_g;
  const uint64_t* ex_out;
  const uint64_t* tx_nuc;
  const uint64_t* tx_pep;
  uint64_t span;
  uint32_t lane_chunks;
};
inline uint32_t tile_ovf_ex(const TileGeometry& g, const TileRec& r) {
  return r.e2 - r.e1 > g.ex_rows ? r.e2 - r.e1 - g.ex_rows : 0u;
}
inline uint32_t tile_ovf_tx(const TileGeometry& g, const TileRec& r) {
  const uint32_t rows = r.j2 > r.j1 ? r.j2 - r.j1 + 1 : 0u;
  return rows > g.tx_rows ? rows - g.tx_rows : 0u;
}
TileGeometry tile_geometry(const TileRec* tiles, uint64_t n_tiles, uint32_t force_ex,
                           uint32_t force_tx);
void pack_tile_block(const TileTables& tb, const TileGeometry& g, const TileRec& r, uint32_t oe,
                     uint32_t ot, uint8_t* b, uint64_t* ovf_ex, TxRow* ovf_tx);

struct GenomeView {
  const uint64_t* contig_base;
  const uint64_t* contig_len;
  uint64_t n_contigs;
  uint64_t span;
  const ExcRun* runs;
  const uint32_t* dir;
};
struct PlanOptions {
  uint32_t outputs;
  bool by_genome;
  int lane_chunks;
  uint32_t block_ex, block_tx;
};
int plan_check_tables(const magot_exon* exons, uint64_t n_exons, const magot_tx* txs,
                      uint64_t n_tx, uint32_t outputs);
PlanOptions plan_options(uint32_t outputs);
struct PlanInput {
  GenomeView g;
  const magot_exon* exons;
  uint64_t E;
  const magot_tx* txs;
  uint64_t T;
  PlanOptions opt;
};
struct PlanCount {
  std::vector<uint64_t> rec_ex, rec_len;
  uint64_t Ec = 0, B = 0, P = 0;
  unsigned nth = 1;
};
int plan_count(const PlanInput& in, PlanCount* out);
struct TilePlan {
  HostBuf<uint64_t> ex_g, ex_out;
  std::vector<uint64_t> tn, tp;
  std::vector<uint64_t> nuc_off, pep_off;
  std::vector<uint64_t> lay_nuc, lay_pep;
  uint64_t Ec = 0, Tc = 0;
  uint32_t lane_chunks = 0;
  std::vector<TileRec> tiles;
  TileGeometry geo{};
  std::vector<uint32_t> ovf_at;
  uint64_t n_ovf_ex = 0, n_ovf_tx = 0;
  unsigned nth = 1;
};
int plan_build(const PlanInput& in, PlanCount&& cnt, Lap& lap, TilePlan* out);
int cut_tiles(const uint64_t* ex_out, uint64_t Ec, const uint64_t* tn, const uint64_t* tp,
              uint64_t Tc, uint64_t tile, std::vector<TileRec>* tiles);

struct ExtractArgs {
  const uint32_t* nib;
  uint64_t span;
  const ExcRun* runs;
  const uint32_t* dir;
  const uint8_t* blocks;
  const uint64_t* ovf_ex;
  const TxRow* ovf_tx;
  TileGeometry blk;
  uint8_t* nuc;
  uint8_t* pep;
  uint64_t total_nuc;
  uint64_t total_pep;
  uint32_t n_tiles;
  uint32_t outputs;
  uint32_t lut[16];
  uint32_t lane_chunks;
};

#if defined(__HIP_DEVICE_COMPILE__) && !defined(__GFX9__)
#error "wave_scan uses DPP row_bcast:15/31, which exists only on gfx9 wave64 (gfx950) targets"
#endif
__device__ __forceinline__ uint32_t wave_scan(uint32_t v) {
  v += (uint32_t)__builtin_amdgcn_update_dpp(0, (int)v, 0x111, 0xF, 0xF, true);
  v += (uint32_t)__builtin_amdgcn_update_dpp(0, (int)v, 0x112, 0xF, 0xF, true);
  v += (uint32_t)__builtin_amdgcn_update_dpp(0, (int)v, 0x114, 0xF, 0xF, true);
  v += (uint32_t)__builtin_amdgcn_update_dpp(0, (int)v, 0x118, 0xF, 0xF, true);
  v += (uint32_t)__builtin_amdgcn_update_dpp(0, (int)v, 0x142, 0xA, 0xF, false);
  v += (uint32_t)__builtin_amdgcn_update_dpp(0, (int)v, 0x143, 0xC, 0xF, false);
  return v;
}

__device__ __forceinline__ uint32_t byte_eq_mask4(uint32_t x, uint32_t pat) {
  x ^= pat;
  const uint32_t t = (x & 0x7f7f7f7fu) + 0x7f7f7f7fu;
  const uint32_t z = ~(t | x | 0x7f7f7f7fu) >> 7;
  return (z * 0x00204081u) >> 21 & 0xFu;
}

__device__ __forceinline__ uint32_t byte_eq_mask16(uint4 v, uint32_t pat) {
  return byte_eq_mask4(v.x, pat) | byte_eq_mask4(v.y, pat) << 4 | byte_eq_mask4(v.z, pat) << 8 |
         byte_eq_mask4(v.w, pat) << 12;
}

inline size_t occupancy_lds_pad(const void* fn, int threads, int want) {
  if (want <= 0) return 0;
  int dev = 0, lds_cu = 0, n = 0;
  hipFuncAttributes at{};
  if (hipGetDevice(&dev) != hipSuccess || hipFuncGetAttributes(&at, fn) != hipSuccess ||
      hipDeviceGetAttribute(&lds_cu, hipDeviceAttributeMaxSharedMemoryPerMultiprocessor, dev) !=
          hipSuccess ||
      hipOccupancyMaxActiveBlocksPerMultiprocessor(&n, fn, threads, 0) != hipSuccess || n <= want)
    return 0;
  const size_t need = (size_t)lds_cu / (size_t)(want + 1) + 1;
  return need > at.sharedSizeBytes ? need - at.sharedSizeBytes : 0;
}

void launch_extract(const ExtractArgs& a, hipStream_t s);
int extract_blocks_per_cu();
void launch_mirror_planes(uint32_t* nib, uint64_t span, hipStream_t s);

void launch_revcomp(const uint8_t* in, const uint64_t* off, uint64_t n, uint64_t total,
                    uint8_t* out, hipStream_t s);
constexpr uint32_t kOrf6RowCap = 123;
constexpr uint64_t kOrf6ExcRow = 1ull << 63;
struct Orf6Args {
  const uint8_t* nuc;
  const uint32_t* nib;
  uint64_t nib_words;
  const uint32_t* code2;
  uint64_t code2_words;
  const uint32_t* exc1;
  uint64_t exc1_words;
  const uint64_t* rows;
  uint64_t n_rows;
  const uint64_t* noff;
  uint64_t n_rec;
  uint64_t total;
  const uint64_t* boff;
  const uint64_t* tile_t0;
  const uint32_t* tile_r0;
  const uint32_t* tile_e0;
  const uint32_t* tile_m;
  uint64_t n_tiles;
  const uint8_t* tables;
  uint8_t* out;
};
struct Orf6Tiles {
  std::vector<uint64_t> t0;
  std::vector<uint32_t> r0, e0, m;
};
void orf6_tables(const uint8_t lut64[64], uint8_t out[256]);
void orf6_plan_tiles(const uint64_t* noff, uint64_t n_rec, const uint64_t* row_start,
                     uint64_t n_rows, Orf6Tiles* out);
void launch_orf6(const Orf6Args& a, bool genome, hipStream_t s);
void launch_code2(const uint32_t* nib, uint64_t nib_words, uint32_t* code2, hipStream_t s);
void launch_exc1(const uint32_t* nib, uint64_t nib_words, uint32_t* exc1, hipStream_t s);
void launch_translate(const uint8_t* in, const uint64_t* off, uint64_t n, const int32_t* frames,
                      const uint8_t* strands, const uint64_t* pep_off, uint64_t total_pep,
                      const uint32_t* lut16, uint8_t* out, hipStream_t s);
constexpr uint32_t kMaxSymbolLut = 32768;
void launch_codon_symbols(const uint8_t* in, uint64_t n_codons, const uint8_t* cls, uint32_t K,
                          const uint8_t* lut, uint8_t* out, hipStream_t s);

constexpr uint32_t kNoRecord = 0xFFFFFFFFu;
struct TextUnit {
  uint64_t text_off;
  uint32_t text_len;
  uint32_t rec;
};
void radix_order(const std::vector<uint64_t>& key, std::vector<uint32_t>* out);
bool gffplan_units(const magot_gffplan* p, const std::string** text, std::vector<TextUnit>* units,
                   bool* protein, uint64_t* n_rec);
size_t text_scan_bytes(uint64_t n);
void launch_text_assembly(const TextUnit* units, uint64_t n, const uint64_t* rspan,
                          const uint8_t* pay, int protein, const uint8_t* text, uint64_t* len,
                          uint64_t* psrc, uint64_t* end, void* scan_tmp, size_t scan_bytes,
                          uint8_t* out, hipStream_t s);

constexpr uint32_t kOrfCallTile = 1024;
constexpr uint8_t kOrfFlagNone = 1;
constexpr uint8_t kOrfFlagNoLongest = 2;
constexpr uint32_t kOrfDigits = 12;
struct OrfCallArgs {
  uint32_t mode;
  const uint8_t* res;
  const uint64_t* soff;
  const uint64_t* noff;
  uint64_t n_rec;
  uint32_t* scnt;
  uint64_t* tile_first;
  uint8_t* flags;
  uint64_t n_tiles;
  uint32_t* tile_stream;
  uint32_t *orfs, *kept;
  uint32_t* extra;
  uint8_t *tflags, *tseen;
  uint64_t *obase, *kbase;
  uint64_t n_orfs;
  uint32_t* rec;
  uint8_t* j;
  uint32_t *k, *len;
  uint64_t* poff;
  uint8_t* payload;
  uint64_t* sel;
  uint32_t *valid, *sellen;
  uint64_t *slot, *cpoff;
  uint64_t n_sel;
  uint32_t* c_rec;
  uint8_t* c_j;
  uint32_t *c_k, *c_len;
  uint64_t* c_poff;
  uint8_t* c_payload;
  uint64_t *src_off, *dst_off;
  void* scan_tmp;
  size_t scan_bytes;
};
struct OrfTextArgs {
  int longest;
  uint64_t n;
  const uint32_t* rec;
  const uint8_t* j;
  const uint32_t *k, *len;
  const uint64_t* poff;
  const uint8_t* payload;
  const uint64_t* noff;
  const uint64_t* hoff;
  uint8_t* text;
  uint64_t dig_off;
  uint32_t* tlen;
  uint64_t* tstart;
  uint8_t* out;
  void* scan_tmp;
  size_t scan_bytes;
};
size_t orfcall_scan_bytes(uint64_t n);
hipError_t launch_orfcall_streams(const OrfCallArgs& a, hipStream_t s);
hipError_t launch_orfcall_count(const OrfCallArgs& a, hipStream_t s);
hipError_t launch_orfcall_write(const OrfCallArgs& a, hipStream_t s);
hipError_t launch_orfcall_longest(const OrfCallArgs& a, hipStream_t s);
hipError_t launch_orfcall_compact(const OrfCallArgs& a, hipStream_t s);
hipError_t launch_orftext_sizes(const OrfTextArgs& a, hipStream_t s);
hipError_t launch_orftext_copy(const OrfTextArgs& a, hipStream_t s);

constexpr uint32_t kLongOrfStep = 64;
struct LongOrfArgs {
  const uint8_t* nuc;
  const uint64_t* start;
  const uint64_t* noff;
  uint64_t n;
  const uint8_t* lut;
  uint32_t waves;
  uint8_t* j;
  uint32_t* k;
  uint32_t* ku;
  uint32_t* len;
  uint8_t* flags;
  uint64_t* poff;
  uint8_t* payload;
  void* scan_tmp;
  size_t scan_bytes;
};
struct LongOrfTextArgs {
  uint64_t n_print;
  const uint64_t* name_off;
  const uint8_t* names;
  uint32_t* tlen;
  uint64_t* tstart;
  uint8_t* out;
  void* scan_tmp;
  size_t scan_bytes;
};
size_t longorf_scan_bytes(uint64_t n);
hipError_t launch_longorf_call(const LongOrfArgs& a, hipStream_t s);
hipError_t launch_longorf_write(const LongOrfArgs& a, hipStream_t s);
hipError_t launch_longorf_text_sizes(const LongOrfArgs& a, const LongOrfTextArgs& t, hipStream_t s);
hipError_t launch_longorf_text_write(const LongOrfArgs& a, const LongOrfTextArgs& t, hipStream_t s);

constexpr uint32_t kMaskPiece = 2048;
struct MaskArgs {
  uint32_t flags;
  const uint8_t* src;
  uint64_t src_bytes;
  const magot_mask_interval* rows;
  uint64_t n_rows;
  const uint64_t* contig_src;
  uint32_t* cov;
  uint64_t cov_words;
  uint64_t n_rec;
  const uint64_t* tstart;
  const uint64_t* rsrc;
  const uint32_t* hlen;
  const uint64_t* hoff;
  const uint8_t* hdr;
  uint8_t* out;
  uint64_t text_bytes;
};
hipError_t launch_mask_paint(const MaskArgs& a, hipStream_t s);
hipError_t launch_mask_text(const MaskArgs& a, hipStream_t s);
hipError_t launch_mask_paint_rows(const magot_mask_interval* rows, uint64_t n_rows,
                                  const uint64_t* contig_src, uint32_t* cov, uint64_t n_bits,
                                  hipStream_t s);

constexpr int kRankWords = 16;
constexpr uint64_t track_blocks(uint64_t span) { return (span / 32 + kRankWords - 1) / kRankWords; }
constexpr uint64_t track_plane_words(uint64_t span) { return (track_blocks(span) + 1) * kRankWords; }
struct TrackWindowArgs {
  const uint32_t* track;
  const uint32_t* rank;
  const uint64_t* contig_base;
  const uint64_t* first;
  uint64_t n_contigs;
  uint64_t n_windows;
  uint64_t W, jump;
  uint32_t* sums;
  uint32_t* flip_count;
  uint64_t* flip_slot;
  uint64_t* flip_index;
};
constexpr uint64_t track_flip_groups(uint64_t n_windows) { return (n_windows + 63) / 64; }
size_t track_scan_bytes(uint64_t n);
hipError_t launch_track_class(const uint32_t* nib, uint64_t n_words, uint64_t lo, uint64_t hi,
                              bool gc, bool replace, uint32_t* track, hipStream_t s);
hipError_t launch_track_andnot(uint32_t* track, const uint32_t* clear, uint64_t n_words,
                               hipStream_t s);
hipError_t launch_track_bytes_set(const uint8_t* stage, uint64_t lo, uint64_t hi, uint32_t* track,
                                  hipStream_t s);
hipError_t launch_track_bytes_get(const uint32_t* track, uint64_t lo, uint64_t hi, uint8_t* stage,
                                  hipStream_t s);
hipError_t launch_track_rank(const uint32_t* track, uint64_t n_blocks, uint32_t* count,
                             uint32_t* rank, void* scan_tmp, size_t scan_bytes, hipStream_t s);
hipError_t launch_track_windows(const TrackWindowArgs& a, hipStream_t s);
hipError_t launch_track_flip_count(const TrackWindowArgs& a, uint32_t s_min, void* scan_tmp,
                                   size_t scan_bytes, hipStream_t s);
hipError_t launch_track_flip_write(const TrackWindowArgs& a, uint32_t s_min, uint64_t cap,
                                   hipStream_t s);
hipError_t launch_track_count(const magot_mask_interval* rows, uint64_t n_rows,
                              const uint64_t* contig_base, const uint32_t* track,
                              const uint32_t* rank, uint64_t span, uint32_t* ones, hipStream_t s);

constexpr int kDepthBlock = 256;
constexpr uint64_t depth_blocks(uint64_t n_lines) { return (n_lines + kDepthBlock - 1) / kDepthBlock; }
struct DepthCarry {
  uint64_t lines;
  uint32_t has_prev, name_len, pos, pad;
  uint8_t name[256];
};
struct DepthHead {
  uint64_t line, offset;
  uint32_t name_len, pad;
};
struct DepthParseArgs {
  const uint8_t* text;
  int64_t n;
  uint64_t file_off;
  const uint32_t* blk_first;
  const DepthCarry* in;
  DepthCarry* out;
  int32_t* arena;
  uint64_t arena_cap;
  DepthHead* heads;
  uint32_t* n_heads;
// ... 417 lines not shown
```

magot_amd/csrc/extract.hip:

```cpp
#include "common.h"

namespace magot {
namespace {

constexpr int kGuard = 4;

template <int LC>
struct WaveLds {
  static constexpr int kS = 64 * LC;
  uint4 ex[kExonCap];
  uint32_t vb[kExonCap];
  int64_t tn[kTxCap + 1];
  int64_t tp[kTxCap + 1];
  uint32_t codes_g[kGuard + kS + 8];
  uint32_t valid_g[kGuard + (kS > 2 * kPepSlots ? kS : 2 * kPepSlots) / 2 + 8];
  uint8_t cmap[kS];
  uint8_t pmap[kPepSlots];
};

constexpr uint32_t kFlagRevFwd = 32u;

__device__ __forceinline__ uint32_t funnel(uint32_t hi, uint32_t lo, uint32_t sh) {
  return __builtin_amdgcn_alignbit(hi, lo, sh);
}

__device__ __forceinline__ uint32_t bfi(uint32_t mask, uint32_t a, uint32_t b) {
  return (a & mask) | (b & ~mask);
}

__device__ __forceinline__ uint32_t spread_bits(uint32_t m4) {
  const uint32_t x = m4 | (m4 << 7);
  return (x | (x << 14)) & 0x01010101u;
}

__device__ __forceinline__ uint32_t rc_literal(uint32_t b) {
  return (b == 'n' || b == 'N' || b == '-') ? b : (uint32_t)'n';
}

struct Chunk {
  uint32_t x0, x1;
  uint32_t exc;
  uint32_t lit[4];
};

__device__ __forceinline__ void put_literal(Chunk& o, int ka, int kb, uint32_t byte) {
  const uint32_t n = (uint32_t)(kb - ka + 1);
  const uint32_t bits = ((n >= 32u) ? 0xFFFFFFFFu : ((1u << n) - 1u)) << ka;
  o.exc |= bits;
  const uint32_t rep = byte | (byte << 8) | (byte << 16) | (byte << 24);
#pragma unroll
  for (int q = 0; q < 4; ++q) {
    const uint32_t b01 = spread_bits((bits >> (4 * q)) & 0xFu);
    const uint32_t bm = (b01 << 8) - b01;
    o.lit[q] = (o.lit[q] & ~bm) | (rep & bm);
  }
}

__device__ __forceinline__ void spread_nibbles(uint32_t x, uint32_t& s0, uint32_t& s1) {
  const uint32_t lo = x & 0x0F0F0F0Fu;
  const uint32_t hi = (x >> 4) & 0x0F0F0F0Fu;
  s0 = __builtin_amdgcn_perm(hi, lo, 0x05010400u);
  s1 = __builtin_amdgcn_perm(hi, lo, 0x07030602u);
}

__device__ __forceinline__ uint4 chunk_ascii(uint32_t x0, uint32_t x1, uint32_t exc,
                                             const uint32_t lit[4]) {
  uint32_t s[4];
  spread_nibbles(x0, s[0], s[1]);
  spread_nibbles(x1, s[2], s[3]);
  uint32_t w[4];
#pragma unroll
  for (int q = 0; q < 4; ++q) w[q] = __builtin_amdgcn_perm(0x74676361u, 0x54474341u, s[q]);
  if (exc) {
#pragma unroll
    for (int q = 0; q < 4; ++q) {
      const uint32_t b01 = spread_bits((exc >> (4 * q)) & 0xFu);
      const uint32_t em = (b01 << 8) - b01;
      w[q] = (w[q] & ~em) | (lit[q] & em);
    }
  }
  return make_uint4(w[0], w[1], w[2], w[3]);
}

__device__ __forceinline__ uint4 chunk_ascii_lit(uint32_t x0, uint32_t x1, uint32_t exc,
                                                 const uint32_t lit[4]) {
  uint32_t s[4];
  spread_nibbles(x0, s[0], s[1]);
  spread_nibbles(x1, s[2], s[3]);
  uint32_t w[4];
#pragma unroll
  for (int q = 0; q < 4; ++q) {
    const uint32_t base = __builtin_amdgcn_perm(0x74676361u, 0x54474341u, s[q] & 0x07070707u);
    const uint32_t lits = __builtin_amdgcn_perm(kLitHi, kLitLo, s[q] & 0x07070707u);
    const uint32_t m = ((s[q] >> 3) & 0x01010101u) * 0xFFu;
    w[q] = bfi(m, lits, base);
  }
  if (exc) {
#pragma unroll
    for (int q = 0; q < 4; ++q) {
      const uint32_t b01 = spread_bits((exc >> (4 * q)) & 0xFu);
      const uint32_t em = (b01 << 8) - b01;
      w[q] = (w[q] & ~em) | (lit[q] & em);
    }
  }
  return make_uint4(w[0], w[1], w[2], w[3]);
}

__device__ __forceinline__ uint32_t exc_bits(uint32_t x0, uint32_t x1) {
  uint32_t e0 = (x0 >> 3) & 0x11111111u, e1 = (x1 >> 3) & 0x11111111u;
  e0 = (e0 | (e0 >> 3)) & 0x03030303u;
  e1 = (e1 | (e1 >> 3)) & 0x03030303u;
  e0 = (e0 | (e0 >> 6)) & 0x000F000Fu;
  e1 = (e1 | (e1 >> 6)) & 0x000F000Fu;
  e0 = (e0 | (e0 >> 12)) & 0xFFu;
  e1 = (e1 | (e1 >> 12)) & 0xFFu;
  return e0 | (e1 << 8);
}

__device__ __forceinline__ uint32_t pack_codes(uint32_t x0, uint32_t x1) {
  const uint32_t y0 = bfi(0x03030303u, x0, x0 >> 2), y1 = bfi(0x03030303u, x1, x1 >> 2);
  const uint32_t z0 = bfi(0x0F0F0F0Fu, y0, y0 >> 4), z1 = bfi(0x0F0F0F0Fu, y1, y1 >> 4);
  return __builtin_amdgcn_perm(z1, z0, 0x06040200u);
}

__device__ __forceinline__ void store16_edge(uint8_t* dst, uint4 v, bool edge) {
  if (edge)
    *reinterpret_cast<uint4*>(dst) = v;
  else
    store16(dst, v);
}

struct Planes {
  const uint32_t* __restrict__ nib;
  const uint32_t* __restrict__ dir;
  const ExcRun* __restrict__ runs;
  uint64_t span;
};

__device__ __forceinline__ void window(const uint32_t* nib, uint64_t u, uint32_t& x0,
                                       uint32_t& x1) {
  const uint32_t* w = nib + (u >> 3);
  const uint32_t sh = 4u * (uint32_t)(u & 7);
  const uint32_t w0 = w[0], w1 = w[1], w2 = w[2];
  x0 = funnel(w1, w0, sh);
  x1 = funnel(w2, w1, sh);
}

__device__ __forceinline__ void patch_runs(const Planes& a, uint64_t glo, uint64_t ghi, bool rc,
                                           int j0, Chunk& o) {
  const uint32_t d0 = a.dir[glo >> kDirShift];
  const uint32_t d1 = a.dir[ghi >> kDirShift];
  if ((d0 & kDirClean) && (d1 & kDirClean)) return;
  for (uint32_t d = d0 & ~kDirClean;; ++d) {
    const ExcRun r = a.runs[d];
    if (r.start > ghi) break;
    const uint64_t rend = r.start + r.len;
    if (rend > glo) {
      const uint64_t ovl = max(glo, r.start);
      const uint64_t ovh = min(ghi, rend - 1);
      if (!rc) put_literal(o, j0 + (int)(ovl - glo), j0 + (int)(ovh - glo), r.byte);
      else put_literal(o, j0 + (int)(ghi - ovh), j0 + (int)(ghi - ovl), rc_literal(r.byte));
    }
  }
}

constexpr uint64_t kUMask = (1ull << 33) - 1;

__device__ __noinline__ Chunk build_chunk_slow(Planes a, int p, int lim, int i,
                                               const uint4* ex) {
  Chunk o;
  o.x0 = 0;
  o.x1 = 0;
  o.exc = 0;
  o.lit[0] = o.lit[1] = o.lit[2] = o.lit[3] = 0;
  const int end = min(p + kChunk, lim);
  int pos = p;
  while (pos < end) {
    uint4 X = ex[i];
    while ((int)X.z <= pos) X = ex[++i];
    const int j0 = pos - p;
    const int n = min((int)X.z, end) - pos;
    const bool rc = (X.w & kFlagRc) != 0;
    const uint64_t U = (uint64_t)X.y | ((uint64_t)((X.w >> 12) & 1u) << 32);
    uint32_t x0, x1;
    window(a.nib, (U + (uint64_t)p) & kUMask, x0, x1);
    const uint64_t m = (n >= 16 ? ~0ull : ((1ull << (4 * n)) - 1ull)) << (4 * j0);
    o.x0 = bfi((uint32_t)m, x0, o.x0);
    o.x1 = bfi((uint32_t)(m >> 32), x1, o.x1);
    if (X.w & kFlagExc) {
      const uint64_t u0 = (U + (uint64_t)pos) & kUMask;
      const uint64_t glo = rc ? 2 * a.span - 1 - (u0 + (uint64_t)(n - 1)) : u0;
      patch_runs(a, glo, glo + (uint64_t)(n - 1), rc, j0, o);
    }
    pos += n;
  }
  return o;
}

struct TileDesc {
  uint64_t T0, T1, Q0, Q1;
  uint32_t m, nt, ovf_ex, ovf_tx;
};

struct TileRows {
  uint2 ex[2];
  TxRow tx[2];
};

__device__ __forceinline__ TileDesc load_tile(const ExtractArgs& a, uint32_t t, int lane,
                                              TileRows& r) {
  const uint32_t E = a.blk.ex_rows, X = a.blk.tx_rows;
  const uint8_t* blk = a.blocks + (uint64_t)t * a.blk.stride;
  const uint2* exr = reinterpret_cast<const uint2*>(blk + sizeof(TileHead));
  const TxRow* txr = reinterpret_cast<const TxRow*>(blk + sizeof(TileHead) + 8 * (size_t)E);
  r.ex[0] = make_uint2(0u, 0u);
  r.tx[0] = TxRow{0, 0};
  if ((uint32_t)lane < E) r.ex[0] = exr[lane];
  if ((uint32_t)lane < X) r.tx[0] = txr[lane];
  typedef const __attribute__((address_space(4))) TileHead CT;
  CT* h = (CT*)blk;
  TileDesc d;
  d.T0 = h->T0;
  d.Q0 = h->Q0;
  const uint32_t sr = h->span_res, cn = h->counts;
  d.ovf_ex = h->ovf_ex;
  d.ovf_tx = h->ovf_tx;
  d.T1 = d.T0 + (sr & 0xFFFFu);
  d.Q1 = d.Q0 + (sr >> 16);
  d.m = cn & 0xFFu;
  d.nt = cn >> 8;
  r.ex[1] = make_uint2(0u, 0u);
  r.tx[1] = TxRow{0, 0};
  if (d.m > E && E + (uint32_t)lane < d.m)
    r.ex[1] = reinterpret_cast<const uint2*>(a.ovf_ex)[d.ovf_ex + (uint32_t)lane];
  if (d.nt >= X && X + (uint32_t)lane <= d.nt)
    r.tx[1] = a.ovf_tx[d.ovf_tx + (uint32_t)lane];
  return d;
}

struct TileGeom {
  int span, lim, n_out, n_all, qshift, n_res, n_pc;
  uint64_t qbase;
};

__device__ __forceinline__ TileGeom geom(const ExtractArgs& a, const TileDesc& d) {
  TileGeom g;
  g.span = (int)(d.T1 - d.T0);
  g.lim = (int)min((uint64_t)(g.span + kHalo), a.total_nuc - d.T0);
  g.n_out = (g.span + kChunk - 1) / kChunk;
  g.n_all = (g.lim + kChunk - 1) / kChunk;
  g.qbase = d.Q0 & ~15ull;
  g.qshift = (int)(d.Q0 - g.qbase);
  g.n_res = (int)(d.Q1 - d.Q0);
  g.n_pc = (g.n_res + g.qshift + 15) >> 4;
  return g;
}

template <int LC>
__device__ __forceinline__ void stage(WaveLds<LC>& L, uint32_t* codes, uint32_t* valid32,
                                      const TileDesc& d, const TileGeom& g, const TileRows& rows,
                                      uint64_t span, const TileGeometry& blk, int lane) {
  const int m = (int)d.m, nt = (int)d.nt;
#pragma unroll
  for (int h = 0; h < LC; ++h) codes[lane + 64 * h] = 0;
#pragma unroll
  for (int h = 0; h < kPepPerLane; ++h) valid32[lane + 64 * h] = 0;
  __builtin_amdgcn_wave_barrier();
  const uint64_t vbase = 2 * span - 16;
#pragma unroll
  for (int h = 0; h < 2; ++h) {
    const int j = h ? (int)blk.ex_rows + lane : lane;
    if ((h || lane < (int)blk.ex_rows) && j < m) {
      const uint32_t lo = rows.ex[h].x, hi = rows.ex[h].y;
      const uint32_t u32 = hi & 1u, end32 = (hi >> 1) & 0x1FFFu, f3 = (hi >> 14) & 7u;
      const uint32_t cj = (hi >> 17) & 0x1FFu;
      const bool revfwd = (f3 & (kFlagRc | kFlagExc)) == kFlagRc;
      const uint64_t V = vbase - ((uint64_t)lo | (uint64_t)u32 << 32);
      const uint32_t vlo = (uint32_t)V, v32 = (uint32_t)(V >> 32) & 1u;
      const uint32_t fl = f3 | (lo & 7u) << 8 | u32 << 12 |
                          (revfwd ? kFlagRevFwd | (vlo & 7u) << 13 : 0u);
      L.vb[j] = (vlo >> 3 | v32 << 29) << 2;
      const uint32_t bN = (lo >> 3 | u32 << 29) << 2;
      L.ex[j] = make_uint4(bN, lo, end32, fl);
      if ((int)cj < g.n_all) atomicAdd(&codes[cj], 1u);
    }
  }
#pragma unroll
  for (int h = 0; h < 2; ++h) {
    const int r = h ? (int)blk.tx_rows + lane : lane;
    if ((h || lane < (int)blk.tx_rows) && r <= nt && nt > 0) {
      const int64_t tp = rows.tx[h].tp;
      L.tn[r] = rows.tx[h].tn;
      L.tp[r] = tp;
      if (r >= 1 && r < nt) {
        const int pj = ((int)tp + g.qshift + 15) >> 4;
        if (pj < g.n_pc) atomicAdd(&valid32[pj], 1u);
      }
    }
  }
  __builtin_amdgcn_wave_barrier();
  uint32_t hc[LC], pc[kPepPerLane];
#pragma unroll
  for (int i = 0; i < LC; ++i) hc[i] = codes[LC * lane + i] + (i ? hc[i - 1] : 0u);
#pragma unroll
  for (int i = 0; i < kPepPerLane; ++i) pc[i] = valid32[kPepPerLane * lane + i] + (i ? pc[i - 1] : 0u);
  const uint32_t ct = hc[LC - 1], pt = pc[kPepPerLane - 1];
  const uint32_t sc = wave_scan(ct | (pt << 16));
  const uint32_t cx = (sc & 0xFFFFu) - ct;
  const uint32_t px = (sc >> 16) - pt;
#pragma unroll
  for (int i = 0; i < LC; ++i) L.cmap[LC * lane + i] = (uint8_t)(cx + hc[i]);
#pragma unroll
  for (int i = 0; i < kPepPerLane; ++i) L.pmap[kPepPerLane * lane + i] = (uint8_t)(px + pc[i]);
  __builtin_amdgcn_wave_barrier();
}

__device__ __forceinline__ __amdgpu_buffer_rsrc_t plane_rsrc(const uint32_t* plane) {
  return __builtin_amdgcn_make_buffer_rsrc(const_cast<uint32_t*>(plane), (short)0,
                                           (int)0xFFFFFFFFu, 0x00020000);
}

__device__ __forceinline__ uint3 load_window(__amdgpu_buffer_rsrc_t plane, uint32_t off) {
  const auto v = __builtin_amdgcn_raw_buffer_load_b96(plane, off, 0, 0);
  return make_uint3(v[0], v[1], v[2]);
}

__device__ __forceinline__ uint2 seg_masks(uint32_t n1) {
  const uint32_t mlo = n1 >= 8 ? 0xFFFFFFFFu : ((1u << (4 * n1)) - 1u);
  const uint32_t mhi = n1 >= 16 ? 0xFFFFFFFFu : (n1 <= 8 ? 0u : ((1u << (4 * (n1 - 8))) - 1u));
  return make_uint2(mlo, mhi);
}

__device__ __forceinline__ uint32_t revcomp8(uint32_t w) {
  const uint32_t b = __builtin_amdgcn_perm(0u, w, 0x00010203u);
  return bfi(0x0F0F0F0Fu, b >> 4, b << 4) ^ 0x33333333u;
}

__device__ __forceinline__ void fast_chunk(uint3 A, uint3 B, uint32_t mt, const uint2* masks,
                                           uint32_t& x0, uint32_t& x1) {
  const uint32_t sa = (mt >> 6) & 28u, sb = (mt >> 14) & 28u;
  const uint32_t a0 = funnel(A.y, A.x, sa), a1 = funnel(A.z, A.y, sa);
  const uint32_t b0 = funnel(B.y, B.x, sb), b1 = funnel(B.z, B.y, sb);
  const uint2 m = masks[(mt >> 24) & 63u];
  x0 = bfi(m.x, a0, b0);
  x1 = bfi(m.y, a1, b1);
}

template <int LC>
__global__ __launch_bounds__(kThreads) void extract_kernel(ExtractArgs a) {
  __shared__ WaveLds<LC> s_wave[kWaves];
  __shared__ __attribute__((aligned(16))) uint8_t s_lut[64];
  __shared__ uint2 s_mask[34];

  const int lane = threadIdx.x & 63;
  const int wave = __builtin_amdgcn_readfirstlane(threadIdx.x >> 6);
  WaveLds<LC>& L = s_wave[wave];
  uint32_t* const codes = L.codes_g + kGuard;
  uint32_t* const valid32 = L.valid_g + kGuard;
  uint16_t* const valid16 = reinterpret_cast<uint16_t*>(valid32);
  const bool want_nuc = (a.outputs & MAGOT_OUT_NUC) != 0;
  const bool want_pep = (a.outputs & MAGOT_OUT_PEP) != 0;

  constexpr uint32_t kXcdRun = 16;
  const uint32_t xb = blockIdx.x, grp = xb / (8 * kXcdRun);
  const uint32_t vb = (grp + 1) * 8 * kXcdRun <= gridDim.x
                          ? grp * 8 * kXcdRun + (xb % 8) * kXcdRun + (xb / 8) % kXcdRun : xb;
  const uint32_t t = vb * kWaves + wave;
  if (t >= a.n_tiles) return;
  {
    int v = 0;
#pragma unroll
    for (int i = 0; i < 16; ++i) asm("v_writelane_b32 %0, %1, %2" : "+v"(v) : "s"(a.lut[i]), "i"(i));
    if (lane < 16) reinterpret_cast<uint32_t*>(s_lut)[lane] = (uint32_t)v;
    if (lane < 34) {
      const uint2 lo = seg_masks(lane <= 16 ? (uint32_t)lane : (uint32_t)(33 - lane));
      s_mask[lane] = lane <= 16 ? lo : make_uint2(~lo.x, ~lo.y);
    }
  }
  if (lane < kGuard) {
    L.codes_g[lane] = 0;
    L.valid_g[lane] = 0;
  }
  TileRows rows;
  const TileDesc d = load_tile(a, t, lane, rows);
  const TileGeom g = geom(a, d);
  stage(L, codes, valid32, d, g, rows, a.span, a.blk, lane);
  const uint64_t T0 = d.T0;

  const int edge_lo = (int)((((T0 + 127) >> 7) << 7) - T0);
  const int edge_hi = (int)(((d.T1 >> 7) << 7) - T0);

  const __amdgpu_buffer_rsrc_t nib_rs = plane_rsrc(a.nib);
  uint3 wA[LC], wB[LC];
  uint32_t meta[LC];
#pragma unroll
  for (int k = 0; k < LC; ++k) {
    const int c = min(lane + 64 * k, g.n_all - 1);
    const int p = c * kChunk;
    const int i = L.cmap[c];
    const uint4 X = L.ex[i];
    const uint4 Y = L.ex[min(i + 1, (int)d.m - 1)];
    const int cend = min(p + kChunk, g.lim);
    const int n1 = min((int)X.z, cend) - p;
    const bool two = n1 < cend - p;
    const uint32_t fb = two ? Y.w : X.w;
    const bool slow = ((X.w | fb) & kFlagSlowLit) != 0 || (two && (int)Y.z < cend) ||
                      (a.outputs & kDebugSlowNuc);
    const bool rev = (X.w & fb & kFlagRevFwd) != 0;
    const uint32_t c8 = 8u * (uint32_t)c;
    uint32_t fa = X.x + c8, ra = L.vb[i] - c8;
    const uint32_t ib = (uint32_t)min(i + 1, (int)d.m - 1) & (kExonCap - 1);
    uint32_t fb2 = Y.x + c8, rb = L.vb[ib] - c8;
    __asm__("" : "+v"(fa), "+v"(ra), "+v"(fb2), "+v"(rb));
    const uint32_t offa = rev ? ra : fa;
    const uint32_t offb = two ? (rev ? rb : fb2) : offa;
    const uint32_t sha = (rev ? X.w >> 5 : X.w) & 0x700u, shb = (rev ? fb >> 5 : fb) & 0x700u;
    const uint32_t mi = (uint32_t)(two ? n1 : 16) + (rev ? 17u : 0u);
    meta[k] = ((lane + 64 * k) < g.n_all ? 1u : 0u) | (rev ? 4u : 0u) | (slow ? 16u : 0u) |
              sha | (shb << 8) | (mi << 24);
    wA[k] = load_window(nib_rs, offa);
    wB[k] = load_window(nib_rs, offb);
  }
  uint32_t x0k[LC], x1k[LC];
#pragma unroll
  for (int k = 0; k < LC; ++k) {
    fast_chunk(wA[k], wB[k], meta[k], s_mask, x0k[k], x1k[k]);
    const uint32_t r0 = revcomp8(x1k[k]), r1 = revcomp8(x0k[k]);
    const bool rv = (meta[k] & 4u) != 0;
    x0k[k] = rv ? r0 : x0k[k];
    x1k[k] = rv ? r1 : x1k[k];
  }
  uint32_t slow_any = 0, exc_any = 0;
#pragma unroll
  for (int k = 0; k < LC; ++k) {
    slow_any |= meta[k] & 16u;
    exc_any |= (meta[k] & 1u) ? (x0k[k] | x1k[k]) & 0x88888888u : 0u;
  }
  const bool any_slow = __builtin_amdgcn_readfirstlane(__ballot(slow_any != 0) != 0);
  const bool any_exc = __builtin_amdgcn_readfirstlane(__ballot(exc_any != 0) != 0);
#pragma unroll
  for (int k = 0; k < LC; ++k) {
    const int c = lane + 64 * k;
    const int p = c * kChunk;
    const uint32_t mt = meta[k];
    uint32_t ex = 0;
    uint32_t lit[4] = {0u, 0u, 0u, 0u};
    if (any_slow && (mt & 17u) == 17u) {
      const Planes pl{a.nib, a.dir, a.runs, a.span};
      const Chunk o = build_chunk_slow(pl, p, g.lim, L.cmap[c], L.ex);
      x0k[k] = o.x0;
      x1k[k] = o.x1;
      ex = o.exc;
      lit[0] = o.lit[0];
      lit[1] = o.lit[1];
      lit[2] = o.lit[2];
      lit[3] = o.lit[3];
    }
    if (mt & 1u) {
      if (want_nuc && c < g.n_out)
        store16_edge(a.nuc + T0 + (uint64_t)p,
                     any_exc ? chunk_ascii_lit(x0k[k], x1k[k], ex, lit) : chunk_ascii(x0k[k], x1k[k], ex, lit),
                     p < edge_lo || p >= edge_hi);
      if (want_pep) {
        codes[c] = pack_codes(x0k[k], x1k[k]);
        valid16[c] = (uint16_t)~(any_exc ? (ex | exc_bits(x0k[k], x1k[k])) : ex);
      }
    }
  }
  if (!want_pep || g.n_res <= 0) return;
  if (lane < 5) {
    codes[g.n_all + lane] = 0;
    valid16[g.n_all + lane] = 0;
  }
  __builtin_amdgcn_wave_barrier();

#pragma unroll 1
  for (int c = lane; c < g.n_pc; c += 64) {
  const int q_first = c * 16 - g.qshift;
  const int kk0 = c == 0 ? g.qshift : 0;
  const int kk1 = min(16, g.n_res - q_first);
  const int j = L.pmap[c];
  const int64_t tpj = L.tp[j], tpn = L.tp[j + 1];
  const int r1 = (int)(L.tn[j] + 3 * ((int64_t)q_first - tpj));
  const int s = (int)min(tpn - (int64_t)q_first, (int64_t)16);
  const bool two = s < kk1;
  int r2 = 0;
  bool slow = (a.outputs & kDebugSlowPep) != 0;
  if (two) {
    r2 = (int)L.tn[j + 1] - 3 * s;
    slow = slow || (L.tp[j + 2] - (int64_t)q_first) < (int64_t)kk1;
  }
  uint32_t w[4] = {0u, 0u, 0u, 0u};
  if (!slow) {
    uint32_t Y[2][3], OK[2][2];
#pragma unroll
    for (int seg = 0; seg < 2; ++seg) {
      const int r0 = (seg == 1 && two) ? r2 : r1;
      const int cw = r0 >> 4;
      const uint32_t sh = (uint32_t)(2 * (r0 & 15));
      const uint32_t X0 = codes[cw], X1 = codes[cw + 1], X2 = codes[cw + 2], X3 = codes[cw + 3];
      Y[seg][0] = funnel(X1, X0, sh);
      Y[seg][1] = funnel(X2, X1, sh);
      Y[seg][2] = funnel(X3, X2, sh);
      const int vw = r0 >> 5;
      const uint32_t vsh = (uint32_t)(r0 & 31);
      const uint32_t V0 = valid32[vw], V1 = valid32[vw + 1], V2 = valid32[vw + 2];
      const uint32_t Z0 = funnel(V1, V0, vsh), Z1 = funnel(V2, V1, vsh);
      OK[seg][0] = Z0 & funnel(Z1, Z0, 1) & funnel(Z1, Z0, 2);
      OK[seg][1] = Z1 & (Z1 >> 1) & (Z1 >> 2);
    }
    const int sc = min(s, 16);
    uint32_t Ym[3], ok0, ok1;
#pragma unroll
    for (int q = 0; q < 3; ++q) {
      const int nb = min(max(6 * sc - 32 * q, 0), 32);
      Ym[q] = bfi(nb >= 32 ? 0xFFFFFFFFu : ((1u << nb) - 1u), Y[0][q], Y[1][q]);
    }
    {
      const int n0 = min(3 * sc, 32), n1 = max(3 * sc - 32, 0);
      ok0 = bfi(n0 >= 32 ? 0xFFFFFFFFu : ((1u << n0) - 1u), OK[0][0], OK[1][0]);
      ok1 = bfi((1u << n1) - 1u, OK[0][1], OK[1][1]);
    }
#pragma unroll
    for (int k = 0; k < 16; ++k) {
      const int ob = 6 * k;
      const uint32_t idx = ((ob & 31) <= 26 ? (Ym[ob >> 5] >> (ob & 31))
                                            : funnel(Ym[(ob >> 5) + 1], Ym[ob >> 5], ob & 31)) &
                           63u;
      w[k >> 2] |= (uint32_t)s_lut[idx] << (8 * (k & 3));
    }
    const uint32_t bad0 = ~ok0 & 0x49249249u;
    const uint32_t bad1 = ~ok1 & 0x00002492u;
    if (__builtin_amdgcn_ballot_w64((bad0 | bad1) != 0)) {
      const uint32_t f[4] = {bad0 & 0xFFFu, (bad0 >> 12) & 0xFFFu,
                             ((bad0 >> 24) | (bad1 << 8)) & 0xFFFu, (bad1 >> 4) & 0xFFFu};
#pragma unroll
      for (int q = 0; q < 4; ++q) {
        const uint32_t m = ((f[q] * 0x8421u) & 0x01010101u) * 0xFFu;
        w[q] = (w[q] & ~m) | (0x58585858u & m);
      }
    }
  } else {
    int jj = j;
    for (int kk = kk0; kk < kk1; ++kk) {
      const int q = q_first + kk;
      while ((int64_t)q >= L.tp[jj + 1]) ++jj;
      const int r = (int)(L.tn[jj] + 3 * ((int64_t)q - L.tp[jj]));
      const int cw = r >> 4;
      const uint32_t x = funnel(codes[cw + 1], codes[cw], (uint32_t)(2 * (r & 15))) & 63u;
      const uint32_t vv = funnel(valid32[(r >> 5) + 1], valid32[r >> 5], (uint32_t)(r & 31));
      const uint32_t aa = ((vv & 7u) == 7u) ? s_lut[x] : (uint32_t)'X';
      w[kk >> 2] |= aa << (8 * (kk & 3));
    }
  }
  uint8_t* const pdst = a.pep + g.qbase + 16 * (uint64_t)c;
  if (kk0 == 0 && kk1 == 16) {
    const uint64_t pq = (uint64_t)(pdst - a.pep);
    store16_edge(pdst, make_uint4(w[0], w[1], w[2], w[3]),
                 (pq >> 7) == (d.Q0 >> 7) || (pq >> 7) == ((d.Q1 - 1) >> 7));
  } else {
#pragma unroll
    for (int kk = 0; kk < 16; ++kk)
      if (kk >= kk0 && kk < kk1) pdst[kk] = (uint8_t)(w[kk >> 2] >> (8 * (kk & 3)));
  }
  }
}

__global__ __launch_bounds__(256) void mirror_planes_kernel(uint32_t* __restrict__ nib,
                                                            uint64_t nw) {
  const uint64_t w = (uint64_t)blockIdx.x * blockDim.x + threadIdx.x;
  if (w >= nw) return;
  const uint32_t b = __builtin_bswap32(nib[nw - 1 - w]);
  const uint32_t x = ((b >> 4) & 0x0F0F0F0Fu) | ((b << 4) & 0xF0F0F0F0u);
  const uint32_t e = (x >> 3) & 0x11111111u;
  const uint32_t emask = e * 0xFu;
  const uint32_t cls = x & 0x77777777u;
  const uint32_t big = ((cls + 0x55555555u) >> 3) & 0x11111111u;
  const uint32_t rc = (cls & ~(big * 7u)) | big;
  nib[nw + w] = ((x ^ 0x33333333u) & ~emask) | ((0x88888888u | rc) & emask);
}

}

void launch_mirror_planes(uint32_t* nib, uint64_t span, hipStream_t s) {
  const uint64_t nw = span / 8;
  if (nw == 0) return;
  hipLaunchKernelGGL(mirror_planes_kernel, dim3((uint32_t)((nw + 255) / 256)), dim3(256), 0, s,
                     nib, nw);
}

constexpr int kExtractBlocksPerCu = 6;

template <int LC>
size_t extract_lds_pad() {
  static const size_t pad = occupancy_lds_pad(reinterpret_cast<const void*>(extract_kernel<LC>),
                                              kThreads, kExtractBlocksPerCu);
  return pad;
}

void launch_extract(const ExtractArgs& a, hipStream_t s) {
  if (a.n_tiles == 0) return;
  const uint32_t grid = (a.n_tiles + kWaves - 1) / kWaves;
  if (a.lane_chunks == kLaneChunksSmall)
    hipLaunchKernelGGL(extract_kernel<kLaneChunksSmall>, dim3(grid), dim3(kThreads),
                       extract_lds_pad<kLaneChunksSmall>(), s, a);
  else
    hipLaunchKernelGGL(extract_kernel<kLaneChunksLarge>, dim3(grid), dim3(kThreads),
                       extract_lds_pad<kLaneChunksLarge>(), s, a);
}

int extract_blocks_per_cu() {
  int n = 0;
  if (hipOccupancyMaxActiveBlocksPerMultiprocessor(&n, extract_kernel<kLaneChunksLarge>, kThreads,
                                                   extract_lds_pad<kLaneChunksLarge>()) !=
      hipSuccess)
    return 0;
  return n;
}

}
```

magot_amd/csrc/tileblocks.cpp:

```cpp
#include <algorithm>
#include <cstring>

#include "common.h"

namespace magot {

TileGeometry tile_geometry(const TileRec* tiles, uint64_t n_tiles, uint32_t force_ex,
                           uint32_t force_tx) {
  uint64_t hm[kExonCap + 1] = {0}, hr[kTxCap + 2] = {0};
  uint32_t max_m = 0, max_r = 0;
  for (uint64_t t = 0; t < n_tiles; ++t) {
    const uint32_t m = std::min<uint32_t>(tiles[t].e2 - tiles[t].e1, kExonCap);
    const uint32_t nt = std::min<uint32_t>(tiles[t].j2 - tiles[t].j1, kTxCap);
    const uint32_t r = nt ? nt + 1 : 0u;
    ++hm[m];
    ++hr[r];
    max_m = std::max(max_m, m);
    max_r = std::max(max_r, r);
  }
  auto pct98 = [&](const uint64_t* h, uint32_t top) -> uint32_t {
    uint64_t acc = 0;
    for (uint32_t v = 0; v <= top; ++v) {
      acc += h[v];
      if (acc * 50 >= n_tiles * 49) return v;
    }
    return top;
  };
  uint32_t ex = force_ex ? force_ex : pct98(hm, kExonCap);
  uint32_t tx = force_tx ? force_tx : pct98(hr, kTxCap + 1);
  ex = std::min((std::max({ex, 1u, max_m > 64u ? max_m - 64u : 0u}) + 1u) & ~1u, kBlkExMax);
  tx = std::min(std::max({tx, 1u, max_r > 64u ? max_r - 64u : 0u}), kBlkTxMax);
  return TileGeometry{ex, tx, tile_block_stride(ex, tx)};
}

void pack_tile_block(const TileTables& tb, const TileGeometry& g, const TileRec& r, uint32_t oe,
                     uint32_t ot, uint8_t* b, uint64_t* ovf_ex, TxRow* ovf_tx) {
  const uint32_t m = r.e2 - r.e1, nt = r.j2 - r.j1;
  const uint32_t rows = nt ? nt + 1 : 0u;
  TileHead h;
  h.T0 = r.T0;
  h.Q0 = r.Q0;
  h.span_res = (uint32_t)(r.T1 - r.T0) | (uint32_t)(r.Q1 - r.Q0) << 16;
  h.counts = m | nt << 8;
  h.ovf_ex = m > g.ex_rows ? oe : 0u;
  h.ovf_tx = rows > g.tx_rows ? ot : 0u;
  std::memcpy(b, &h, sizeof h);
  uint64_t* const ex = reinterpret_cast<uint64_t*>(b + sizeof(TileHead));
  TxRow* const tx = reinterpret_cast<TxRow*>(b + sizeof(TileHead) + 8 * (size_t)g.ex_rows);
  const int64_t end_cap = tile_bytes((int)tb.lane_chunks) + 4 * kHalo;
  for (uint32_t j = 0; j < m; ++j) {
    const uint64_t gw = tb.ex_g[r.e1 + j];
    const uint64_t o0 = tb.ex_out[r.e1 + j], o1 = tb.ex_out[r.e1 + j + 1];
    const uint64_t gs = gw & ~kExFlagBits;
    const uint64_t s = o0 - r.T0;
    const uint64_t U = (gw & kRcBit) ? 2 * tb.span - gs - (o1 - o0) - s : gs - s;
    const uint64_t end = (uint64_t)std::min<int64_t>((int64_t)(o1 - r.T0), end_cap);
    const uint64_t cj = j == 0 ? kBlkNoChunk
                               : std::min<uint64_t>((s + kChunk - 1) / kChunk, kBlkNoChunk);
    const uint64_t fl = ((gw & kRcBit) ? kFlagRc : 0u) | ((gw & kExcBit) ? kFlagExc : 0u) |
                        ((gw & kSlowLitBit) ? kFlagSlowLit : 0u);
    const uint64_t hi = ((U >> 32) & 1u) | end << 1 | fl << 14 | cj << 17;
    const uint64_t row = (U & 0xFFFFFFFFull) | hi << 32;
    if (j < g.ex_rows) ex[j] = row;
    else ovf_ex[oe + (j - g.ex_rows)] = row;
  }
  for (uint32_t j = m; j < g.ex_rows; ++j) ex[j] = 0;
  for (uint32_t k = 0; k < rows; ++k) {
    const TxRow x{(int64_t)(tb.tx_nuc[r.j1 + k] - r.T0), (int64_t)(tb.tx_pep[r.j1 + k] - r.Q0)};
    if (k < g.tx_rows) tx[k] = x;
    else ovf_tx[ot + (k - g.tx_rows)] = x;
  }
  for (uint32_t k = rows; k < g.tx_rows; ++k) tx[k] = TxRow{0, 0};
  const size_t used = sizeof(TileHead) + 8 * (size_t)g.ex_rows + 16 * (size_t)g.tx_rows;
  std::memset(b + used, 0, g.stride - used);
}

}

using namespace magot;

extern "C" int magot_debug_tile_blocks(const uint64_t* ex_g, const uint64_t* ex_out,
                                       const uint64_t* tx_nuc, const uint64_t* tx_pep,
                                       uint64_t span, uint32_t lane_chunks, const void* tiles,
                                       uint64_t n_tiles, uint32_t* geometry, void* blocks,
                                       uint64_t* ovf_ex, uint64_t ovf_ex_cap, int64_t* ovf_tx,
                                       uint64_t ovf_tx_cap, uint64_t* n_ovf) {
  if (!ex_g || !ex_out || !tx_nuc || !tx_pep || !n_ovf || !geometry || (n_tiles && !tiles) ||
      geometry[0] > kBlkExMax || geometry[1] > kBlkTxMax ||
      (lane_chunks != (uint32_t)kLaneChunksLarge && lane_chunks != (uint32_t)kLaneChunksSmall)) {
    set_error("magot_debug_tile_blocks: bad argument");
    return MAGOT_ERR_ARG;
  }
  const TileRec* tr = static_cast<const TileRec*>(tiles);
  for (uint64_t t = 0; t < n_tiles; ++t) {
    const uint64_t m = (uint64_t)tr[t].e2 - tr[t].e1, nt = (uint64_t)tr[t].j2 - tr[t].j1;
    if (tr[t].e2 < tr[t].e1 || tr[t].j2 < tr[t].j1 || m > (uint64_t)kExonCap ||
        nt > (uint64_t)kTxCap || tr[t].T1 - tr[t].T0 > 0xFFFFull ||
        tr[t].Q1 - tr[t].Q0 > 0xFFFFull) {
      set_error("magot_debug_tile_blocks: tile " + std::to_string(t) + " out of range");
      return MAGOT_ERR_RANGE;
    }
  }
  const TileGeometry g = tile_geometry(tr, n_tiles, geometry[0], geometry[1]);
  geometry[0] = g.ex_rows;
  geometry[1] = g.tx_rows;
  geometry[2] = g.stride;
  uint64_t ne = 0, nx = 0;
  for (uint64_t t = 0; t < n_tiles; ++t) {
    ne += tile_ovf_ex(g, tr[t]);
    nx += tile_ovf_tx(g, tr[t]);
  }
  n_ovf[0] = ne;
  n_ovf[1] = nx;
  if (!blocks) return MAGOT_OK;
  if (ne > ovf_ex_cap || nx > ovf_tx_cap || (ne && !ovf_ex) || (nx && !ovf_tx) ||
      ne > 0xFFFFFFFFull || nx > 0xFFFFFFFFull) {
    set_error("magot_debug_tile_blocks: overflow arrays too small");
    return MAGOT_ERR_ARG;
  }
  const TileTables tb{ex_g, ex_out, tx_nuc, tx_pep, span, lane_chunks};
  uint64_t oe = 0, ot = 0;
  for (uint64_t t = 0; t < n_tiles; ++t) {
    pack_tile_block(tb, g, tr[t], (uint32_t)oe, (uint32_t)ot,
                    static_cast<uint8_t*>(blocks) + t * g.stride, ovf_ex,
                    reinterpret_cast<TxRow*>(ovf_tx));
    oe += tile_ovf_ex(g, tr[t]);
    ot += tile_ovf_tx(g, tr[t]);
  }
  return MAGOT_OK;
}
```

magot_amd/csrc/tileplan.cpp:

```cpp
#include <algorithm>
#include <cstdio>
#include <cstdlib>
#include <cstring>

#include "common.h"

namespace magot {

int plan_check_tables(const magot_exon* exons, uint64_t n_exons, const magot_tx* txs,
                      uint64_t n_tx, uint32_t outputs) {
  if ((n_exons && !exons) || (n_tx && !txs)) {
    set_error("magot_plan_create: null argument");
    return MAGOT_ERR_ARG;
  }
  if (outputs & ~(MAGOT_OUT_NUC | MAGOT_OUT_PEP | MAGOT_OUT_GENOME_ORDER)) {
    set_error("magot_plan_create: unknown output flags");
    return MAGOT_ERR_ARG;
  }
  if (n_tx >= 0xFFFFFFFFull || n_exons >= 0xFFFFFFFFull) {
    set_error("magot_plan_create: table too large for one plan (split it)");
    return MAGOT_ERR_ARG;
  }
  return MAGOT_OK;
}

PlanOptions plan_options(uint32_t outputs) {
  PlanOptions o{outputs & ~MAGOT_OUT_GENOME_ORDER, (outputs & MAGOT_OUT_GENOME_ORDER) != 0, 0, 0, 0};
  if (const char* e = std::getenv("MAGOT_EXTRACT_LANE_CHUNKS")) o.lane_chunks = std::atoi(e);
  if (const char* e = std::getenv("MAGOT_TILE_BLOCK_ROWS")) {
    unsigned fe = 0, fx = 0;
    if (sscanf(e, "%u,%u", &fe, &fx) == 2) {
      o.block_ex = std::min(fe, kBlkExMax);
      o.block_tx = std::min(fx, kBlkTxMax);
    }
  }
  return o;
}

namespace {


int check_records(const PlanInput& in) {
  uint64_t expect = 0;
  for (uint64_t t = 0; t < in.T; ++t) {
    if (in.txs[t].exon_begin != expect) {
      set_error("magot_plan_create: record " + std::to_string(t) +
                " does not start where the previous one ended");
      return MAGOT_ERR_ARG;
    }
    expect += in.txs[t].n_exons;
    if (expect > in.E) {
      set_error("magot_plan_create: records reference more exons than given");
      return MAGOT_ERR_ARG;
    }
  }
  if (expect != in.E) {
    set_error("magot_plan_create: exons not covered by records");
    return MAGOT_ERR_ARG;
  }
  return MAGOT_OK;
}

uint64_t count_sweep(const PlanInput& in, PlanCount* c) {
  const GenomeView& g = in.g;
  std::vector<uint64_t> first_bad(c->nth, ~0ull);
  parallel_ranges(in.T, c->nth, [&](uint64_t t0, uint64_t t1, unsigned part) {
    for (uint64_t t = t0; t < t1; ++t) {
      uint64_t len = 0, nz = 0;
      const uint64_t e0 = in.txs[t].exon_begin, e1 = e0 + in.txs[t].n_exons;
      for (uint64_t e = e0; e < e1; ++e) {
        const magot_exon& x = in.exons[e];
        const uint64_t st = x.start_rc & ~kRcBit;
        if (x.contig >= g.n_contigs || st > g.contig_len[x.contig] ||
            st + x.len > g.contig_len[x.contig]) {
          first_bad[part] = e;
          return;
        }
        len += x.len;
        nz += x.len != 0;
      }
      c->rec_len[t] = len;
      c->rec_ex[t] = nz;
    }
  });
  for (uint64_t e : first_bad)
    if (e != ~0ull) return e;
  return ~0ull;
}


void word_sweep(const PlanInput& in, const PlanCount& c, uint64_t* w_g, uint32_t* w_len) {
  const GenomeView& g = in.g;
  parallel_ranges(in.T, c.nth, [&](uint64_t t0, uint64_t t1, unsigned) {
    for (uint64_t t = t0; t < t1; ++t) {
      uint64_t k = c.rec_ex[t];
      const uint64_t e0 = in.txs[t].exon_begin, e1 = e0 + in.txs[t].n_exons;
      for (uint64_t e = e0; e < e1; ++e) {
        const magot_exon& x = in.exons[e];
        if (x.len == 0) continue;
        const uint64_t gs = g.contig_base[x.contig] + (x.start_rc & ~kRcBit);
        uint64_t d = g.dir[gs >> kDirShift] & ~kDirClean;
        while (g.runs[d].start + g.runs[d].len <= gs) ++d;
        uint64_t exc = g.runs[d].start < gs + x.len ? kExcBit : 0;
        if (exc && !(x.start_rc & kRcBit)) {
          for (uint64_t r = d; g.runs[r].start < gs + x.len; ++r)
            if (lit_class(g.runs[r].byte) == 7u) {
              exc |= kSlowLitBit;
              break;
            }
        }
        w_g[k] = gs | (x.start_rc & kRcBit) | exc;
        w_len[k] = x.len;
        ++k;
      }
    }
  });
}

std::vector<uint32_t> layout_order(const PlanInput& in, const PlanCount& c, const uint64_t* w_g) {
  std::vector<uint32_t> order;
  if (in.opt.by_genome) {
    std::vector<uint64_t> key(in.T);
    for (uint64_t t = 0; t < in.T; ++t)
      key[t] = c.rec_ex[t] < c.rec_ex[t + 1] ? w_g[c.rec_ex[t]] & ~kExFlagBits : in.g.span;
    radix_order(key, &order);
  }
  return order;
}

void lay_out(const PlanInput& in, const PlanCount& c, const std::vector<uint32_t>& order,
             HostBuf<uint64_t>&& w_g, const uint32_t* w_len, TilePlan* p) {
  const uint64_t T = in.T, Ec = c.Ec;
  const bool by_genome = in.opt.by_genome;
  p->lay_nuc.resize(T);
  p->lay_pep.resize(T);
  uint64_t* const lay_nuc = p->lay_nuc.data();
  uint64_t* const lay_pep = p->lay_pep.data();
  HostBuf<uint64_t> lay_ex(T);
  uint64_t acc = 0, q = 0, ek = 0;
  for (uint64_t k = 0; k < T; ++k) {
    const uint64_t t = by_genome ? order[k] : k;
    lay_nuc[t] = acc;
    lay_pep[t] = q;
    lay_ex[t] = ek;
    acc += c.rec_len[t];
    q += c.rec_len[t] / 3;
    ek += c.rec_ex[t + 1] - c.rec_ex[t];
  }
  p->ex_g = by_genome ? HostBuf<uint64_t>(Ec + 1) : std::move(w_g);
  p->ex_out = HostBuf<uint64_t>(Ec + 2);
  uint64_t* const ex_g = p->ex_g.data();
  uint64_t* const ex_out = p->ex_out.data();
  parallel_ranges(T, c.nth, [&](uint64_t t0, uint64_t t1, unsigned) {
    for (uint64_t t = t0; t < t1; ++t) {
      uint64_t k = lay_ex[t], o = lay_nuc[t];
      for (uint64_t i = c.rec_ex[t]; i < c.rec_ex[t + 1]; ++i, ++k) {
        if (by_genome) ex_g[k] = w_g[i];
        ex_out[k] = o;
        o += w_len[i];
      }
    }
  });
  ex_g[Ec] = 0;
  ex_out[Ec] = c.B;
  ex_out[Ec + 1] = c.B;
}

void record_tables(const PlanInput& in, const PlanCount& c, const std::vector<uint32_t>& order,
                   TilePlan* p) {
  const uint64_t T = in.T;
  std::vector<uint64_t> tn, tp;
  tn.reserve(T + 3);
  tp.reserve(T + 3);
  for (uint64_t k = 0; k < T; ++k) {
    const uint64_t t = in.opt.by_genome ? order[k] : k;
    if (c.rec_len[t] >= 3) {
      tn.push_back(p->lay_nuc[t]);
      tp.push_back(p->lay_pep[t]);
    }
  }
  std::vector<uint64_t> nuc_off(T + 1), pep_off(T + 1);
  nuc_off[0] = pep_off[0] = 0;
  for (uint64_t t = 0; t < T; ++t) {
    nuc_off[t + 1] = nuc_off[t] + c.rec_len[t];
    pep_off[t + 1] = pep_off[t] + c.rec_len[t] / 3;
  }
  p->Tc = tn.size();
  tn.push_back(c.B);
  tp.push_back(c.P);
  p->tn = std::move(tn);
  p->tp = std::move(tp);
  p->nuc_off = std::move(nuc_off);
  p->pep_off = std::move(pep_off);
}

struct Cursor {
  const uint64_t* v;
  uint64_t n, j;
  uint64_t operator()(uint64_t x) {
    while (j < n && v[j] <= x) ++j;
    return j;
  }
};

}

int cut_tiles(const uint64_t* ex_out, uint64_t Ec, const uint64_t* tn, const uint64_t* tp,
              uint64_t Tc, uint64_t tile, std::vector<TileRec>* tiles) {
  const uint64_t B = ex_out[Ec], P = tp[Tc];
  auto pcount = [&](Cursor& c, uint64_t T) -> uint64_t {
    const uint64_t j = c(T);
    if (j == 0) return 0;
    const uint64_t into = T - tn[j - 1];
    return tp[j - 1] + std::min((into + 2) / 3, tp[j] - tp[j - 1]);
  };
  auto rec_of = [&](Cursor& c, uint64_t q) -> uint64_t {
    return c(q) - 1;
  };
  Cursor c_end{tn, Tc, 0}, c_dec{tn, Tc, 0};
  Cursor c_r0{tp, Tc, 0}, c_r1{tp, Tc, 0};
  uint64_t e1 = 0, e2 = 0;
  uint64_t T0 = 0, R0 = 0;
  while (T0 < B) {
    while (e1 < Ec && ex_out[e1 + 1] <= T0) ++e1;
    const uint64_t j1 = R0 < P ? rec_of(c_r0, R0) : Tc;
    uint64_t T1 = std::min<uint64_t>(T0 + tile, B);
    if (e1 + kExonCap < Ec) T1 = std::min<uint64_t>(T1, ex_out[e1 + kExonCap] - kHalo);
    if (j1 + kTxCap - kChunk < Tc) T1 = std::min<uint64_t>(T1, tn[j1 + kTxCap - kChunk]);
    if (T1 < B) T1 = (T1 & ~(uint64_t)(kTileAlign - 1)) > T0 ? T1 & ~(uint64_t)(kTileAlign - 1)
                                                           : T1 & ~(uint64_t)(kChunk - 1);
    if (T1 < T0 + kChunk) T1 = std::min<uint64_t>(T0 + kChunk, B);
    const uint64_t dec_end = std::min<uint64_t>(T1 + kHalo, B);
    uint64_t R1 = P;
    if (T1 < B) {
      R1 = std::min<uint64_t>((pcount(c_end, T1) + kChunk - 1) & ~(uint64_t)(kChunk - 1), P);
      R1 = std::min<uint64_t>(R1, pcount(c_dec, dec_end - 2));
      R1 = std::min<uint64_t>(R1, (R0 & ~(uint64_t)(kChunk - 1)) + kPepSlots * kChunk);
    }
    if (R1 < R0) R1 = R0;
    if (e2 < e1) e2 = e1;
    while (e2 < Ec && ex_out[e2] < dec_end) ++e2;
    const uint64_t jl = R1 > R0 ? rec_of(c_r1, R1 - 1) : 0;
    const uint64_t j2 = R1 > R0 ? jl + 1 : j1;
    if (e2 - e1 > (uint64_t)kExonCap || (R1 > R0 && j2 - j1 > (uint64_t)kTxCap) ||
        (R1 > R0 && tn[jl] + 3 * (R1 - 1 - tp[jl]) + 3 > dec_end)) {
      set_error("magot_plan_create: internal tiling error");
      return MAGOT_ERR_STATE;
    }
    tiles->push_back(TileRec{T0, T1, R0, R1, (uint32_t)e1, (uint32_t)e2,
                             (uint32_t)(R1 > R0 ? j1 : 0), (uint32_t)(R1 > R0 ? j2 : 0)});
    T0 = T1;
    R0 = R1;
  }
  if (R0 != P) {
    set_error("magot_plan_create: internal tiling error (residues)");
    return MAGOT_ERR_STATE;
  }
  return MAGOT_OK;
}

namespace {

int choose_tiles(const PlanOptions& opt, TilePlan* p) {
  auto cut = [&](int lane_chunks) {
    p->lane_chunks = (uint32_t)lane_chunks;
    p->tiles.clear();
    return cut_tiles(p->ex_out.data(), p->Ec, p->tn.data(), p->tp.data(), p->Tc,
                     tile_bytes(lane_chunks), &p->tiles);
  };
  if (int rc = cut(kLaneChunksLarge)) return rc;
  if (opt.lane_chunks == kLaneChunksSmall ||
      (opt.lane_chunks != kLaneChunksLarge && (opt.outputs & MAGOT_OUT_PEP) &&
       p->tiles.size() < kSmallTilePlan))
    return cut(kLaneChunksSmall);
  return MAGOT_OK;
}

void launch_order(TilePlan* p) {
  const uint64_t n = p->tiles.size();
  const uint64_t* ex_g = p->ex_g.data();
  const uint64_t* ex_out = p->ex_out.data();
  const std::vector<TileRec> cut = std::move(p->tiles);
  std::vector<uint8_t> slow_tile(n);
  parallel_ranges(n, n >= (1u << 14) ? p->nth : 1u, [&](uint64_t t0, uint64_t t1, unsigned) {
    for (uint64_t t = t0; t < t1; ++t) {
      bool slow = false;
      for (uint32_t e = cut[t].e1; e < cut[t].e2 && !slow; ++e)
        slow = (ex_g[e] & kSlowLitBit) || ex_out[e + 1] - ex_out[e] < (uint64_t)kChunk;
      slow_tile[t] = slow;
    }
  });
  p->tiles.assign(n, TileRec{});
  const uint64_t n_first = std::count(slow_tile.begin(), slow_tile.end(), 1);
  uint64_t at[2] = {n_first, 0};
  for (uint64_t t = 0; t < n; ++t) p->tiles[at[slow_tile[t]]++] = cut[t];
}

int place_overflow(const PlanOptions& opt, TilePlan* p) {
  const uint64_t n = p->tiles.size();
  p->geo = tile_geometry(p->tiles.data(), n, opt.block_ex, opt.block_tx);
  p->ovf_at.resize(2 * n);
  for (uint64_t t = 0; t < n; ++t) {
    const TileRec& r = p->tiles[t];
    if (r.T1 - r.T0 > 0xFFFFull || r.Q1 - r.Q0 > 0xFFFFull) {
      set_error("magot_plan_create: internal tiling error (tile block fields)");
      return MAGOT_ERR_STATE;
    }
    p->ovf_at[2 * t] = (uint32_t)p->n_ovf_ex;
    p->ovf_at[2 * t + 1] = (uint32_t)p->n_ovf_tx;
    p->n_ovf_ex += tile_ovf_ex(p->geo, r);
    p->n_ovf_tx += tile_ovf_tx(p->geo, r);
  }
  if (p->n_ovf_ex >= 0xFFFFFFFFull || p->n_ovf_tx >= 0xFFFFFFFFull) {
    set_error("magot_plan_create: table too large for one plan (split it)");
    return MAGOT_ERR_ARG;
  }
  return MAGOT_OK;
}

}

int plan_count(const PlanInput& in, PlanCount* c) {
  if (int rc = check_records(in)) return rc;
  c->nth = in.T >= (1u << 15) ? host_threads() : 1u;
  c->rec_ex.resize(in.T + 1);
  c->rec_len.resize(in.T);
  const uint64_t bad = count_sweep(in, c);
  if (bad != ~0ull) {
    set_error("magot_plan_create: exon " + std::to_string(bad) + " outside its contig");
    return MAGOT_ERR_RANGE;
  }
  for (uint64_t t = 0; t < in.T; ++t) {
    const uint64_t n = c->rec_ex[t];
    c->rec_ex[t] = c->Ec;
    c->Ec += n;
    c->B += c->rec_len[t];
    c->P += c->rec_len[t] / 3;
  }
  c->rec_ex[in.T] = c->Ec;
  return MAGOT_OK;
}

int plan_build(const PlanInput& in, PlanCount&& c, Lap& lap, TilePlan* p) {
  p->Ec = c.Ec;
  p->nth = c.nth;
  HostBuf<uint64_t> w_g(c.Ec + 1);
  HostBuf<uint32_t> w_len(c.Ec);
  word_sweep(in, c, w_g.data(), w_len.data());
  lap("pass1");
  const std::vector<uint32_t> order = layout_order(in, c, w_g.data());
  lap("order");
  lay_out(in, c, order, std::move(w_g), w_len.data(), p);
  record_tables(in, c, order, p);
  lap("pass2");
  if (p->Ec >= 0xFFFFFFFFull || p->Tc >= 0xFFFFFFFFull) {
    set_error("magot_plan_create: table too large for one plan (split it)");
    return MAGOT_ERR_ARG;
  }
  if (int rc = choose_tiles(in.opt, p)) return rc;
  lap("tiles");
  if (p->tiles.size() >= 0x7FFFFFFFull) {
    set_error("magot_plan_create: output too large for one launch");
    return MAGOT_ERR_ARG;
  }
  launch_order(p);
  if (int rc = place_overflow(in.opt, p)) return rc;
  lap("launch_ord");
  return MAGOT_OK;
}

}

using namespace magot;

extern "C" int magot_debug_tile_cut(const uint64_t* ex_out, uint64_t n_ex, const uint64_t* tx_nuc,
                                    const uint64_t* tx_pep, uint64_t n_rec, uint32_t lane_chunks,
                                    void* tiles, uint64_t tiles_cap, uint64_t* n_tiles) {
  if (!ex_out || !tx_nuc || !tx_pep || !n_tiles ||
      (lane_chunks != (uint32_t)kLaneChunksLarge && lane_chunks != (uint32_t)kLaneChunksSmall)) {
    set_error("magot_debug_tile_cut: bad argument");
    return MAGOT_ERR_ARG;
  }
  std::vector<TileRec> cut;
  if (int rc = cut_tiles(ex_out, n_ex, tx_nuc, tx_pep, n_rec, tile_bytes((int)lane_chunks), &cut))
    return rc;
  *n_tiles = cut.size();
  if (!tiles) return MAGOT_OK;
  if (cut.size() > tiles_cap) {
    set_error("magot_debug_tile_cut: tile array too small");
    return MAGOT_ERR_ARG;
  }
  if (!cut.empty()) std::memcpy(tiles, cut.data(), cut.size() * sizeof(TileRec));
  return MAGOT_OK;
}

extern "C" int magot_debug_plan(const uint8_t* const* seqs, const uint64_t* lens,
                                uint32_t n_contigs, const magot_exon* exons, uint64_t n_exons,
                                const magot_tx* txs, uint64_t n_tx, uint32_t outputs,
                                uint64_t* info, uint64_t* ex_g, uint64_t* ex_out, uint64_t* tx_nuc,
                                uint64_t* tx_pep, uint64_t* lay_nuc, uint64_t* lay_pep,
                                void* tiles) {
  if (!info || (n_contigs && (!seqs || !lens))) {
    set_error("magot_debug_plan: null argument");
    return MAGOT_ERR_ARG;
  }
  if (int rc = plan_check_tables(exons, n_exons, txs, n_tx, outputs)) return rc;
  std::vector<ContigSource> src(n_contigs);
  for (uint32_t i = 0; i < n_contigs; ++i) src[i] = ContigSource{seqs[i], lens[i], 0, 0};
  HostPacked hp;
  pack_genome(src.data(), n_contigs, &hp);
  if (hp.runs.size() >= (size_t)kDirClean) {
    set_error("magot_debug_plan: too many exception runs");
    return MAGOT_ERR_ARG;
  }
  const PlanInput in{GenomeView{hp.contig_base.data(), hp.contig_len.data(), n_contigs, hp.span,
                                hp.runs.data(), hp.dir.data()},
                     exons, n_exons, txs, n_tx, plan_options(outputs)};
  Lap lap("MAGOT_PLAN_TIMING", "plan");
  PlanCount cnt;
  if (int rc = plan_count(in, &cnt)) return rc;
  const uint64_t B = cnt.B, P = cnt.P;
  TilePlan p;
  if (int rc = plan_build(in, std::move(cnt), lap, &p)) return rc;
  const uint64_t sizes[9] = {B, P, p.Ec, p.Tc, p.tiles.size(), p.lane_chunks, p.geo.ex_rows,
                             p.geo.tx_rows, p.geo.stride};
  if (!tiles) {
    std::memcpy(info, sizes, sizeof sizes);
    return MAGOT_OK;
  }
  if (!ex_g || !ex_out || !tx_nuc || !tx_pep || !lay_nuc || !lay_pep ||
      std::memcmp(info, sizes, sizeof sizes) != 0) {
    set_error("magot_debug_plan: tables need the sizes of a first call in info");
    return MAGOT_ERR_ARG;
  }
  std::memcpy(ex_g, p.ex_g.data(), (p.Ec + 1) * 8);
  std::memcpy(ex_out, p.ex_out.data(), (p.Ec + 1) * 8);
  std::memcpy(tx_nuc, p.tn.data(), (p.Tc + 1) * 8);
  std::memcpy(tx_pep, p.tp.data(), (p.Tc + 1) * 8);
  if (n_tx) std::memcpy(lay_nuc, p.lay_nuc.data(), n_tx * 8);
  if (n_tx) std::memcpy(lay_pep, p.lay_pep.data(), n_tx * 8);
  if (!p.tiles.empty()) std::memcpy(tiles, p.tiles.data(), p.tiles.size() * sizeof(TileRec));
  return MAGOT_OK;
}
```

Measured before the change: 2598 billion.

## Shrink extract kernel LDS and registers, add per-tile path bits for fast/slow dispatch

The extract kernel's per-wave LDS shrinks: the separate vb array is dropped (the mirror offset is folded into ex rows), tx offsets narrow to 32 bits, and per-slot metadata packs two slots per register. Launch bounds now request 6 waves per SIMD. Tile headers carry may-slow and may-exception path bits so the kernel can pick specialised fused or slow slot routines. Lane-chunk support is widened up to 8 with parametrised row field widths, though the default huge setting still equals the large one. The risk is register spilling under the tighter launch bound and added complexity in the row encodings.

After: 2583 billion. About the same (-0.6%).

```diff
diff --git a/include/magot.h b/include/magot.h
--- a/include/magot.h
+++ b/include/magot.h
@@ -120,6 +120,11 @@
 uint64_t magot_plan_algorithmic_bytes(const magot_plan* p);
 
 int magot_debug_tile_blocks(const uint64_t* ex_g, const uint64_t* ex_out, const uint64_t* tx_nuc,
+                            const uint64_t* tx_pep, uint64_t span, uint32_t lane_chunks,
+                            const void* tiles, uint64_t n_tiles, uint32_t* geometry, void* blocks,
+                            uint64_t* ovf_ex, uint64_t ovf_ex_cap, int64_t* ovf_tx,
+                            uint64_t ovf_tx_cap, uint64_t* n_ovf);
+int magot_debug_plan_blocks(const uint64_t* ex_g, const uint64_t* ex_out, const uint64_t* tx_nuc,
                             const uint64_t* tx_pep, uint64_t span, uint32_t lane_chunks,
                             const void* tiles, uint64_t n_tiles, uint32_t* geometry, void* blocks,
                             uint64_t* ovf_ex, uint64_t ovf_ex_cap, int64_t* ovf_tx,
diff --git a/magot_amd/_lib.py b/magot_amd/_lib.py
--- a/magot_amd/_lib.py
+++ b/magot_amd/_lib.py
@@ -40,7 +40,8 @@
     'magot_genome_load_ex', 'magot_genome_wire_ranges', 'magot_genome_attach_wire',
     'magot_copy_segments', 'magot_ctx_mark', 'magot_ctx_elapsed', 'magot_orf6_copy_outputs',
     'magot_genome_wire_export', 'magot_genome_wire_import',
-    'magot_debug_tile_blocks', 'magot_debug_tile_cut', 'magot_debug_plan',
+    'magot_debug_tile_blocks', 'magot_debug_plan_blocks', 'magot_debug_tile_cut',
+    'magot_debug_plan',
     'magot_debug_text_index', 'magot_debug_text_lines', 'magot_debug_piece_copy',
     'magot_debug_text_assembly', 'magot_debug_orf6_tiles', 'magot_debug_orf6_batch',
     'magot_orf6_poison',
@@ -186,6 +187,10 @@
                                                      ctypes.POINTER(_vp)]),
         'magot_plan_algorithmic_bytes': (ctypes.c_uint64, [_vp]),
         'magot_debug_tile_blocks': (ctypes.c_int, [_vp, _vp, _vp, _vp, ctypes.c_uint64,
+                                                   ctypes.c_uint32, _vp, ctypes.c_uint64, _vp, _vp,
+                                                   _vp, ctypes.c_uint64, _vp, ctypes.c_uint64,
+                                                   _vp]),
+        'magot_debug_plan_blocks': (ctypes.c_int, [_vp, _vp, _vp, _vp, ctypes.c_uint64,
                                                    ctypes.c_uint32, _vp, ctypes.c_uint64, _vp, _vp,
                                                    _vp, ctypes.c_uint64, _vp, ctypes.c_uint64,
                                                    _vp]),
diff --git a/magot_amd/csrc/abi_plan.hip b/magot_amd/csrc/abi_plan.hip
--- a/magot_amd/csrc/abi_plan.hip
+++ b/magot_amd/csrc/abi_plan.hip
@@ -157,7 +157,7 @@
   ovf_ex[pl.n_ovf_ex] = 0;
   ovf_tx[pl.n_ovf_tx] = TxRow{0, 0};
   const TileTables tb{pl.ex_g.data(), pl.ex_out.data(), pl.tn.data(), pl.tp.data(), g->span,
-                      pl.lane_chunks};
+                      pl.lane_chunks, true};
   if (int rc = upload_generated(
           ctx, base + o_blocks, n_tiles, geo.stride, n_tiles >= (1u << 12) ? pl.nth : 1u,
           [&](uint64_t t0, uint64_t t1, uint8_t* dst) {
diff --git a/magot_amd/csrc/common.h b/magot_amd/csrc/common.h
--- a/magot_amd/csrc/common.h
+++ b/magot_amd/csrc/common.h
@@ -93,15 +93,24 @@
 constexpr int kWaves = kThreads / 64;
 constexpr int kChunk = 16;
 constexpr int kLaneChunksLarge = 6, kLaneChunksSmall = 3;
+constexpr int kLaneChunksMax = 8;
+constexpr int kLaneChunksHuge = kLaneChunksLarge;
+constexpr bool lane_chunks_ok(int lc) {
+  return lc == kLaneChunksSmall || (lc >= kLaneChunksLarge && lc <= kLaneChunksMax);
+}
 constexpr int tile_bytes(int lane_chunks) { return (64 * lane_chunks - 3) * 16; }
+constexpr int pep_per_lane(int lane_chunks) { return lane_chunks > kLaneChunksLarge ? 3 : 2; }
+constexpr int pep_slots(int lane_chunks) { return 64 * pep_per_lane(lane_chunks); }
+static_assert((tile_bytes(kLaneChunksLarge) / 3 + 2 * kChunk - 1) / kChunk <= pep_slots(kLaneChunksLarge) &&
+              (tile_bytes(kLaneChunksMax) / 3 + 2 * kChunk - 1) / kChunk <= pep_slots(kLaneChunksMax),
+              "a tile's residues fit its residue chunk slots");
 constexpr uint64_t kSmallTilePlan = 40000;
+constexpr uint64_t kHugeTilePlan = 12 * 6144;
 constexpr uint64_t kTileAlign = 128;
-constexpr int kPepPerLane = 2;
 constexpr int kHalo = 3 * kChunk;
 constexpr int kExonCap = 128;
 static_assert((kExonCap & (kExonCap - 1)) == 0, "kExonCap must be a power of two (row index masks)");
 constexpr int kTxCap = 64;
-constexpr int kPepSlots = 64 * kPepPerLane;
 constexpr uint64_t kExcBit = 1ull << 62;
 constexpr uint64_t kSlowLitBit = 1ull << 61;
 constexpr uint64_t kExFlagBits = kRcBit | kExcBit | kSlowLitBit;
@@ -133,7 +142,13 @@
 constexpr uint32_t kFlagSlowLit = 4u;
 constexpr uint32_t kBlkExMax = 64;
 constexpr uint32_t kBlkTxMax = 14;
-constexpr uint32_t kBlkNoChunk = 511;
+constexpr uint32_t row_end_bits(int lane_chunks) { return lane_chunks > kLaneChunksLarge ? 14u : 13u; }
+constexpr uint32_t row_chunk_bits(int lane_chunks) { return lane_chunks > kLaneChunksLarge ? 10u : 9u; }
+constexpr uint32_t row_flag_shift(int lane_chunks) { return 1u + row_end_bits(lane_chunks); }
+constexpr uint32_t row_chunk_shift(int lane_chunks) { return 4u + row_end_bits(lane_chunks); }
+constexpr uint32_t row_no_chunk(int lane_chunks) { return (1u << row_chunk_bits(lane_chunks)) - 1u; }
+constexpr uint32_t kHeadMaySlow = 1u << 16;
+constexpr uint32_t kHeadMayExc = 1u << 17;
 struct TxRow {
   int64_t tn, tp;
 };
@@ -155,9 +170,13 @@
 static_assert(tile_block_stride(kBlkExMax, kBlkTxMax) == 768, "the largest block is six lines");
 static_assert(kExonCap <= (int)kBlkExMax + 64 && kTxCap + 1 <= 1 + 64,
               "one inline and one overflow row per lane");
-static_assert(tile_bytes(kLaneChunksLarge) + 4 * kHalo < (1 << 13) &&
-              (tile_bytes(kLaneChunksLarge) + kHalo + kChunk - 1) / kChunk < (int)kBlkNoChunk,
-              "interval row fields");
+constexpr bool row_fields_hold(int lc) {
+  return tile_bytes(lc) + 4 * kHalo < (1 << row_end_bits(lc)) &&
+         (tile_bytes(lc) + kHalo + kChunk - 1) / kChunk < (int)row_no_chunk(lc) &&
+         row_chunk_shift(lc) + row_chunk_bits(lc) <= 32u;
+}
+static_assert(row_fields_hold(kLaneChunksSmall) && row_fields_hold(kLaneChunksLarge) &&
+              row_fields_hold(7) && row_fields_hold(kLaneChunksMax), "interval row fields");
 struct TileTables {
   const uint64_t* ex_g;
   const uint64_t* ex_out;
@@ -165,7 +184,11 @@
   const uint64_t* tx_pep;
   uint64_t span;
   uint32_t lane_chunks;
-};
+  bool path_bits;
+};
+inline bool tile_interval_slow(uint64_t gw, uint64_t len) {
+  return (gw & kSlowLitBit) != 0 || len < (uint64_t)kChunk;
+}
 inline uint32_t tile_ovf_ex(const TileGeometry& g, const TileRec& r) {
   return r.e2 - r.e1 > g.ex_rows ? r.e2 - r.e1 - g.ex_rows : 0u;
 }
@@ -224,7 +247,7 @@
 };
 int plan_build(const PlanInput& in, PlanCount&& cnt, Lap& lap, TilePlan* out);
 int cut_tiles(const uint64_t* ex_out, uint64_t Ec, const uint64_t* tn, const uint64_t* tp,
-              uint64_t Tc, uint64_t tile, std::vector<TileRec>* tiles);
+              uint64_t Tc, int lane_chunks, std::vector<TileRec>* tiles);
 
 struct ExtractArgs {
   const uint32_t* nib;
diff --git a/magot_amd/csrc/extract.hip b/magot_amd/csrc/extract.hip
--- a/magot_amd/csrc/extract.hip
+++ b/magot_amd/csrc/extract.hip
@@ -8,14 +8,15 @@
 template <int LC>
 struct WaveLds {
   static constexpr int kS = 64 * LC;
+  static constexpr int kPPL = pep_per_lane(LC);
+  static constexpr int kPS = pep_slots(LC);
   uint4 ex[kExonCap];
-  uint32_t vb[kExonCap];
-  int64_t tn[kTxCap + 1];
-  int64_t tp[kTxCap + 1];
+  uint32_t tn[kTxCap + 1];
+  int32_t tp[kTxCap + 1];
   uint32_t codes_g[kGuard + kS + 8];
-  uint32_t valid_g[kGuard + (kS > 2 * kPepSlots ? kS : 2 * kPepSlots) / 2 + 8];
+  uint32_t valid_g[kGuard + (kS > 2 * kPS ? kS : 2 * kPS) / 2 + 8];
   uint8_t cmap[kS];
-  uint8_t pmap[kPepSlots];
+  uint8_t pmap[kPS];
 };
 
 constexpr uint32_t kFlagRevFwd = 32u;
@@ -200,6 +201,7 @@
 struct TileDesc {
   uint64_t T0, T1, Q0, Q1;
   uint32_t m, nt, ovf_ex, ovf_tx;
+  uint32_t path;
 };
 
 struct TileRows {
@@ -228,7 +230,8 @@
   d.T1 = d.T0 + (sr & 0xFFFFu);
   d.Q1 = d.Q0 + (sr >> 16);
   d.m = cn & 0xFFu;
-  d.nt = cn >> 8;
+  d.nt = (cn >> 8) & 0xFFu;
+  d.path = cn & (kHeadMaySlow | kHeadMayExc);
   r.ex[1] = make_uint2(0u, 0u);
   r.tx[1] = TxRow{0, 0};
   if (d.m > E && E + (uint32_t)lane < d.m)
@@ -263,8 +266,9 @@
   const int m = (int)d.m, nt = (int)d.nt;
 #pragma unroll
   for (int h = 0; h < LC; ++h) codes[lane + 64 * h] = 0;
-#pragma unroll
-  for (int h = 0; h < kPepPerLane; ++h) valid32[lane + 64 * h] = 0;
+  constexpr int kPPL = WaveLds<LC>::kPPL;
+#pragma unroll
+  for (int h = 0; h < kPPL; ++h) valid32[lane + 64 * h] = 0;
   __builtin_amdgcn_wave_barrier();
   const uint64_t vbase = 2 * span - 16;
 #pragma unroll
@@ -272,16 +276,17 @@
     const int j = h ? (int)blk.ex_rows + lane : lane;
     if ((h || lane < (int)blk.ex_rows) && j < m) {
       const uint32_t lo = rows.ex[h].x, hi = rows.ex[h].y;
-      const uint32_t u32 = hi & 1u, end32 = (hi >> 1) & 0x1FFFu, f3 = (hi >> 14) & 7u;
-      const uint32_t cj = (hi >> 17) & 0x1FFu;
+      const uint32_t u32 = hi & 1u, end32 = (hi >> 1) & ((1u << row_end_bits(LC)) - 1u);
+      const uint32_t f3 = (hi >> row_flag_shift(LC)) & 7u;
+      const uint32_t cj = (hi >> row_chunk_shift(LC)) & row_no_chunk(LC);
       const bool revfwd = (f3 & (kFlagRc | kFlagExc)) == kFlagRc;
       const uint64_t V = vbase - ((uint64_t)lo | (uint64_t)u32 << 32);
       const uint32_t vlo = (uint32_t)V, v32 = (uint32_t)(V >> 32) & 1u;
       const uint32_t fl = f3 | (lo & 7u) << 8 | u32 << 12 |
                           (revfwd ? kFlagRevFwd | (vlo & 7u) << 13 : 0u);
-      L.vb[j] = (vlo >> 3 | v32 << 29) << 2;
       const uint32_t bN = (lo >> 3 | u32 << 29) << 2;
-      L.ex[j] = make_uint4(bN, lo, end32, fl);
+      const uint32_t bV = (vlo >> 3 | v32 << 29) << 2;
+      L.ex[j] = make_uint4(revfwd ? bV : bN, lo, end32, fl);
       if ((int)cj < g.n_all) atomicAdd(&codes[cj], 1u);
     }
   }
@@ -289,29 +294,29 @@
   for (int h = 0; h < 2; ++h) {
     const int r = h ? (int)blk.tx_rows + lane : lane;
     if ((h || lane < (int)blk.tx_rows) && r <= nt && nt > 0) {
-      const int64_t tp = rows.tx[h].tp;
-      L.tn[r] = rows.tx[h].tn;
+      const int32_t tp = (int32_t)rows.tx[h].tp;
+      L.tn[r] = (uint32_t)rows.tx[h].tn;
       L.tp[r] = tp;
       if (r >= 1 && r < nt) {
-        const int pj = ((int)tp + g.qshift + 15) >> 4;
+        const int pj = (tp + g.qshift + 15) >> 4;
         if (pj < g.n_pc) atomicAdd(&valid32[pj], 1u);
       }
     }
   }
   __builtin_amdgcn_wave_barrier();
-  uint32_t hc[LC], pc[kPepPerLane];
+  uint32_t hc[LC], pc[kPPL];
 #pragma unroll
   for (int i = 0; i < LC; ++i) hc[i] = codes[LC * lane + i] + (i ? hc[i - 1] : 0u);
 #pragma unroll
-  for (int i = 0; i < kPepPerLane; ++i) pc[i] = valid32[kPepPerLane * lane + i] + (i ? pc[i - 1] : 0u);
-  const uint32_t ct = hc[LC - 1], pt = pc[kPepPerLane - 1];
+  for (int i = 0; i < kPPL; ++i) pc[i] = valid32[kPPL * lane + i] + (i ? pc[i - 1] : 0u);
+  const uint32_t ct = hc[LC - 1], pt = pc[kPPL - 1];
   const uint32_t sc = wave_scan(ct | (pt << 16));
   const uint32_t cx = (sc & 0xFFFFu) - ct;
   const uint32_t px = (sc >> 16) - pt;
 #pragma unroll
   for (int i = 0; i < LC; ++i) L.cmap[LC * lane + i] = (uint8_t)(cx + hc[i]);
 #pragma unroll
-  for (int i = 0; i < kPepPerLane; ++i) L.pmap[kPepPerLane * lane + i] = (uint8_t)(px + pc[i]);
+  for (int i = 0; i < kPPL; ++i) L.pmap[kPPL * lane + i] = (uint8_t)(px + pc[i]);
   __builtin_amdgcn_wave_barrier();
 }
 
@@ -336,18 +341,84 @@
   return bfi(0x0F0F0F0Fu, b >> 4, b << 4) ^ 0x33333333u;
 }
 
+constexpr uint32_t kMetaActive = 1u;
+constexpr uint32_t kMetaRev = 2u;
+constexpr uint32_t kMetaSlow = 4u;
+template <int LC>
+__device__ __forceinline__ uint32_t slot_meta(const uint32_t (&meta)[(LC + 1) / 2], int k) {
+  return (k & 1) ? meta[k / 2] >> 16 : meta[k / 2];
+}
+
 __device__ __forceinline__ void fast_chunk(uint3 A, uint3 B, uint32_t mt, const uint2* masks,
                                            uint32_t& x0, uint32_t& x1) {
-  const uint32_t sa = (mt >> 6) & 28u, sb = (mt >> 14) & 28u;
+  const uint32_t sa = (mt >> 1) & 28u, sb = (mt >> 4) & 28u;
   const uint32_t a0 = funnel(A.y, A.x, sa), a1 = funnel(A.z, A.y, sa);
   const uint32_t b0 = funnel(B.y, B.x, sb), b1 = funnel(B.z, B.y, sb);
-  const uint2 m = masks[(mt >> 24) & 63u];
+  const uint2 m = masks[(mt >> 9) & 63u];
   x0 = bfi(m.x, a0, b0);
   x1 = bfi(m.y, a1, b1);
 }
 
-template <int LC>
-__global__ __launch_bounds__(kThreads) void extract_kernel(ExtractArgs a) {
+__device__ __forceinline__ uint32_t mirror_offset(uint4 X) {
+  return (X.y >> 3 | ((X.w >> 12) & 1u) << 29) << 2;
+}
+
+template <int LC, bool EXC, bool SKIP_SLOW>
+__device__ __forceinline__ void fused_slots(const ExtractArgs& a, const uint3 (&wA)[LC],
+                                            const uint3 (&wB)[LC], const uint32_t (&meta)[(LC + 1) / 2],
+                                            const uint2* masks, uint64_t T0, int n_out,
+                                            int edge_lo, int edge_hi, bool want_nuc, bool want_pep,
+                                            uint32_t* codes, uint16_t* valid16, int lane) {
+  const uint32_t lit[4] = {0u, 0u, 0u, 0u};
+#pragma unroll
+  for (int k = 0; k < LC; ++k) {
+    const int c = lane + 64 * k;
+    const int p = c * kChunk;
+    const uint32_t mt = slot_meta<LC>(meta, k);
+    uint32_t x0, x1;
+    fast_chunk(wA[k], wB[k], mt, masks, x0, x1);
+    const uint32_t r0 = revcomp8(x1), r1 = revcomp8(x0);
+    const bool rv = (mt & kMetaRev) != 0;
+    x0 = rv ? r0 : x0;
+    x1 = rv ? r1 : x1;
+    if ((mt & kMetaActive) && !(SKIP_SLOW && (mt & kMetaSlow))) {
+      if (want_nuc && c < n_out)
+        store16_edge(a.nuc + T0 + (uint64_t)p,
+                     EXC ? chunk_ascii_lit(x0, x1, 0u, lit) : chunk_ascii(x0, x1, 0u, lit),
+                     p < edge_lo || p >= edge_hi);
+      if (want_pep) {
+        codes[c] = pack_codes(x0, x1);
+        valid16[c] = (uint16_t)~(EXC ? exc_bits(x0, x1) : 0u);
+      }
+    }
+  }
+}
+
+template <int LC>
+__device__ __forceinline__ void slow_slots(const ExtractArgs& a, const uint32_t (&meta)[(LC + 1) / 2],
+                                           uint64_t T0, int n_out, int lim, int edge_lo,
+                                           int edge_hi, bool want_nuc, bool want_pep,
+                                           const uint8_t* cmap, const uint4* ex_rows,
+                                           uint32_t* codes, uint16_t* valid16, int lane) {
+#pragma unroll
+  for (int k = 0; k < LC; ++k) {
+    const int c = lane + 64 * k;
+    const int p = c * kChunk;
+    if ((slot_meta<LC>(meta, k) & (kMetaActive | kMetaSlow)) != (kMetaActive | kMetaSlow)) continue;
+    const Planes pl{a.nib, a.dir, a.runs, a.span};
+    const Chunk o = build_chunk_slow(pl, p, lim, cmap[c], ex_rows);
+    if (want_nuc && c < n_out)
+      store16_edge(a.nuc + T0 + (uint64_t)p, chunk_ascii_lit(o.x0, o.x1, o.exc, o.lit),
+                   p < edge_lo || p >= edge_hi);
+    if (want_pep) {
+      codes[c] = pack_codes(o.x0, o.x1);
+      valid16[c] = (uint16_t)~(o.exc | exc_bits(o.x0, o.x1));
+    }
+  }
+}
+
+template <int LC>
+__global__ __launch_bounds__(kThreads, 6) void extract_kernel(ExtractArgs a) {
   __shared__ WaveLds<LC> s_wave[kWaves];
   __shared__ __attribute__((aligned(16))) uint8_t s_lut[64];
   __shared__ uint2 s_mask[34];
@@ -392,7 +463,7 @@
 
   const __amdgpu_buffer_rsrc_t nib_rs = plane_rsrc(a.nib);
   uint3 wA[LC], wB[LC];
-  uint32_t meta[LC];
+  uint32_t meta[(LC + 1) / 2];
 #pragma unroll
   for (int k = 0; k < LC; ++k) {
     const int c = min(lane + 64 * k, g.n_all - 1);
@@ -408,64 +479,34 @@
                       (a.outputs & kDebugSlowNuc);
     const bool rev = (X.w & fb & kFlagRevFwd) != 0;
     const uint32_t c8 = 8u * (uint32_t)c;
-    uint32_t fa = X.x + c8, ra = L.vb[i] - c8;
-    const uint32_t ib = (uint32_t)min(i + 1, (int)d.m - 1) & (kExonCap - 1);
-    uint32_t fb2 = Y.x + c8, rb = L.vb[ib] - c8;
+    uint32_t fa = ((X.w & kFlagRevFwd) ? mirror_offset(X) : X.x) + c8, ra = X.x - c8;
+    uint32_t fb2 = ((Y.w & kFlagRevFwd) ? mirror_offset(Y) : Y.x) + c8, rb = Y.x - c8;
     __asm__("" : "+v"(fa), "+v"(ra), "+v"(fb2), "+v"(rb));
     const uint32_t offa = rev ? ra : fa;
     const uint32_t offb = two ? (rev ? rb : fb2) : offa;
-    const uint32_t sha = (rev ? X.w >> 5 : X.w) & 0x700u, shb = (rev ? fb >> 5 : fb) & 0x700u;
+    const uint32_t sha = (rev ? X.w >> 10 : X.w >> 5) & 0x38u;
+    const uint32_t shb = (rev ? fb >> 7 : fb >> 2) & 0x1C0u;
     const uint32_t mi = (uint32_t)(two ? n1 : 16) + (rev ? 17u : 0u);
-    meta[k] = ((lane + 64 * k) < g.n_all ? 1u : 0u) | (rev ? 4u : 0u) | (slow ? 16u : 0u) |
-              sha | (shb << 8) | (mi << 24);
+    const uint32_t mt = ((lane + 64 * k) < g.n_all ? kMetaActive : 0u) | (rev ? kMetaRev : 0u) |
+                        (slow ? kMetaSlow : 0u) | sha | shb | (mi << 9);
+    meta[k / 2] = (k & 1) ? meta[k / 2] | mt << 16 : mt;
+    __asm__ volatile("" : "+v"(meta[k / 2]));
     wA[k] = load_window(nib_rs, offa);
     wB[k] = load_window(nib_rs, offb);
   }
-  uint32_t x0k[LC], x1k[LC];
-#pragma unroll
-  for (int k = 0; k < LC; ++k) {
-    fast_chunk(wA[k], wB[k], meta[k], s_mask, x0k[k], x1k[k]);
-    const uint32_t r0 = revcomp8(x1k[k]), r1 = revcomp8(x0k[k]);
-    const bool rv = (meta[k] & 4u) != 0;
-    x0k[k] = rv ? r0 : x0k[k];
-    x1k[k] = rv ? r1 : x1k[k];
-  }
-  uint32_t slow_any = 0, exc_any = 0;
-#pragma unroll
-  for (int k = 0; k < LC; ++k) {
-    slow_any |= meta[k] & 16u;
-    exc_any |= (meta[k] & 1u) ? (x0k[k] | x1k[k]) & 0x88888888u : 0u;
-  }
-  const bool any_slow = __builtin_amdgcn_readfirstlane(__ballot(slow_any != 0) != 0);
-  const bool any_exc = __builtin_amdgcn_readfirstlane(__ballot(exc_any != 0) != 0);
-#pragma unroll
-  for (int k = 0; k < LC; ++k) {
-    const int c = lane + 64 * k;
-    const int p = c * kChunk;
-    const uint32_t mt = meta[k];
-    uint32_t ex = 0;
-    uint32_t lit[4] = {0u, 0u, 0u, 0u};
-    if (any_slow && (mt & 17u) == 17u) {
-      const Planes pl{a.nib, a.dir, a.runs, a.span};
-      const Chunk o = build_chunk_slow(pl, p, g.lim, L.cmap[c], L.ex);
-      x0k[k] = o.x0;
-      x1k[k] = o.x1;
-      ex = o.exc;
-      lit[0] = o.lit[0];
-      lit[1] = o.lit[1];
-      lit[2] = o.lit[2];
-      lit[3] = o.lit[3];
-    }
-    if (mt & 1u) {
-      if (want_nuc && c < g.n_out)
-        store16_edge(a.nuc + T0 + (uint64_t)p,
-                     any_exc ? chunk_ascii_lit(x0k[k], x1k[k], ex, lit) : chunk_ascii(x0k[k], x1k[k], ex, lit),
-                     p < edge_lo || p >= edge_hi);
-      if (want_pep) {
-        codes[c] = pack_codes(x0k[k], x1k[k]);
-        valid16[c] = (uint16_t)~(any_exc ? (ex | exc_bits(x0k[k], x1k[k])) : ex);
-      }
-    }
+  const bool may_slow = (d.path & kHeadMaySlow) != 0 || (a.outputs & kDebugSlowNuc) != 0;
+  if (!may_slow) {
+    if (d.path & kHeadMayExc)
+      fused_slots<LC, true, false>(a, wA, wB, meta, s_mask, T0, g.n_out, edge_lo, edge_hi,
+                                   want_nuc, want_pep, codes, valid16, lane);
+    else
+      fused_slots<LC, false, false>(a, wA, wB, meta, s_mask, T0, g.n_out, edge_lo, edge_hi,
+                                    want_nuc, want_pep, codes, valid16, lane);
+  } else {
+    fused_slots<LC, true, true>(a, wA, wB, meta, s_mask, T0, g.n_out, edge_lo, edge_hi, want_nuc,
+                                want_pep, codes, valid16, lane);
+    slow_slots<LC>(a, meta, T0, g.n_out, g.lim, edge_lo, edge_hi, want_nuc, want_pep, L.cmap, L.ex,
+                   codes, valid16, lane);
   }
   if (!want_pep || g.n_res <= 0) return;
   if (lane < 5) {
@@ -480,15 +521,15 @@
   const int kk0 = c == 0 ? g.qshift : 0;
   const int kk1 = min(16, g.n_res - q_first);
   const int j = L.pmap[c];
-  const int64_t tpj = L.tp[j], tpn = L.tp[j + 1];
-  const int r1 = (int)(L.tn[j] + 3 * ((int64_t)q_first - tpj));
-  const int s = (int)min(tpn - (int64_t)q_first, (int64_t)16);
+  const int tpj = L.tp[j], tpn = L.tp[j + 1];
+  const int r1 = (int)(L.tn[j] + 3u * (uint32_t)(q_first - tpj));
+  const int s = min(tpn - q_first, 16);
   const bool two = s < kk1;
   int r2 = 0;
   bool slow = (a.outputs & kDebugSlowPep) != 0;
   if (two) {
     r2 = (int)L.tn[j + 1] - 3 * s;
-    slow = slow || (L.tp[j + 2] - (int64_t)q_first) < (int64_t)kk1;
+    slow = slow || (L.tp[j + 2] - q_first) < kk1;
   }
   uint32_t w[4] = {0u, 0u, 0u, 0u};
   if (!slow) {
@@ -544,8 +585,8 @@
     int jj = j;
     for (int kk = kk0; kk < kk1; ++kk) {
       const int q = q_first + kk;
-      while ((int64_t)q >= L.tp[jj + 1]) ++jj;
-      const int r = (int)(L.tn[jj] + 3 * ((int64_t)q - L.tp[jj]));
+      while (q >= L.tp[jj + 1]) ++jj;
+      const int r = (int)(L.tn[jj] + 3u * (uint32_t)(q - L.tp[jj]));
       const int cw = r >> 4;
       const uint32_t x = funnel(codes[cw + 1], codes[cw], (uint32_t)(2 * (r & 15))) & 63u;
       const uint32_t vv = funnel(valid32[(r >> 5) + 1], valid32[r >> 5], (uint32_t)(r & 31));
@@ -598,24 +639,31 @@
   return pad;
 }
 
+template <int LC>
+void launch_extract_lc(const ExtractArgs& a, uint32_t grid, hipStream_t s) {
+  hipLaunchKernelGGL(extract_kernel<LC>, dim3(grid), dim3(kThreads), extract_lds_pad<LC>(), s, a);
+}
+
+template <int LC>
+int extract_blocks_lc() {
+  int n = 0;
+  if (hipOccupancyMaxActiveBlocksPerMultiprocessor(&n, extract_kernel<LC>, kThreads,
+                                                   extract_lds_pad<LC>()) != hipSuccess)
+    return 0;
+  return n;
+}
+
 void launch_extract(const ExtractArgs& a, hipStream_t s) {
   if (a.n_tiles == 0) return;
   const uint32_t grid = (a.n_tiles + kWaves - 1) / kWaves;
-  if (a.lane_chunks == kLaneChunksSmall)
-    hipLaunchKernelGGL(extract_kernel<kLaneChunksSmall>, dim3(grid), dim3(kThreads),
-                       extract_lds_pad<kLaneChunksSmall>(), s, a);
-  else
-    hipLaunchKernelGGL(extract_kernel<kLaneChunksLarge>, dim3(grid), dim3(kThreads),
-                       extract_lds_pad<kLaneChunksLarge>(), s, a);
-}
-
-int extract_blocks_per_cu() {
-  int n = 0;
-  if (hipOccupancyMaxActiveBlocksPerMultiprocessor(&n, extract_kernel<kLaneChunksLarge>, kThreads,
-                                                   extract_lds_pad<kLaneChunksLarge>()) !=
-      hipSuccess)
-    return 0;
-  return n;
-}
-
-}
+  switch (a.lane_chunks) {
+    case kLaneChunksSmall: return launch_extract_lc<kLaneChunksSmall>(a, grid, s);
+    case 7: return launch_extract_lc<7>(a, grid, s);
+    case 8: return launch_extract_lc<8>(a, grid, s);
+    default: return launch_extract_lc<kLaneChunksLarge>(a, grid, s);
+  }
+}
+
+int extract_blocks_per_cu() { return extract_blocks_lc<kLaneChunksHuge>(); }
+
+}
diff --git a/magot_amd/csrc/tileblocks.cpp b/magot_amd/csrc/tileblocks.cpp
--- a/magot_amd/csrc/tileblocks.cpp
+++ b/magot_amd/csrc/tileblocks.cpp
@@ -41,13 +41,15 @@
   h.T0 = r.T0;
   h.Q0 = r.Q0;
   h.span_res = (uint32_t)(r.T1 - r.T0) | (uint32_t)(r.Q1 - r.Q0) << 16;
-  h.counts = m | nt << 8;
   h.ovf_ex = m > g.ex_rows ? oe : 0u;
   h.ovf_tx = rows > g.tx_rows ? ot : 0u;
-  std::memcpy(b, &h, sizeof h);
   uint64_t* const ex = reinterpret_cast<uint64_t*>(b + sizeof(TileHead));
   TxRow* const tx = reinterpret_cast<TxRow*>(b + sizeof(TileHead) + 8 * (size_t)g.ex_rows);
-  const int64_t end_cap = tile_bytes((int)tb.lane_chunks) + 4 * kHalo;
+  const int lc = (int)tb.lane_chunks;
+  const int64_t end_cap = tile_bytes(lc) + 4 * kHalo;
+  const uint64_t no_chunk = row_no_chunk(lc);
+  const uint32_t flag_shift = row_flag_shift(lc), chunk_shift = row_chunk_shift(lc);
+  uint32_t path = 0;
   for (uint32_t j = 0; j < m; ++j) {
     const uint64_t gw = tb.ex_g[r.e1 + j];
     const uint64_t o0 = tb.ex_out[r.e1 + j], o1 = tb.ex_out[r.e1 + j + 1];
@@ -55,15 +57,18 @@
     const uint64_t s = o0 - r.T0;
     const uint64_t U = (gw & kRcBit) ? 2 * tb.span - gs - (o1 - o0) - s : gs - s;
     const uint64_t end = (uint64_t)std::min<int64_t>((int64_t)(o1 - r.T0), end_cap);
-    const uint64_t cj = j == 0 ? kBlkNoChunk
-                               : std::min<uint64_t>((s + kChunk - 1) / kChunk, kBlkNoChunk);
+    const uint64_t cj = j == 0 ? no_chunk : std::min<uint64_t>((s + kChunk - 1) / kChunk, no_chunk);
     const uint64_t fl = ((gw & kRcBit) ? kFlagRc : 0u) | ((gw & kExcBit) ? kFlagExc : 0u) |
                         ((gw & kSlowLitBit) ? kFlagSlowLit : 0u);
-    const uint64_t hi = ((U >> 32) & 1u) | end << 1 | fl << 14 | cj << 17;
+    const uint64_t hi = ((U >> 32) & 1u) | end << 1 | fl << flag_shift | cj << chunk_shift;
     const uint64_t row = (U & 0xFFFFFFFFull) | hi << 32;
     if (j < g.ex_rows) ex[j] = row;
     else ovf_ex[oe + (j - g.ex_rows)] = row;
+    if (tile_interval_slow(gw, o1 - o0)) path |= kHeadMaySlow;
+    if (gw & kExcBit) path |= kHeadMayExc;
   }
+  h.counts = m | nt << 8 | (tb.path_bits ? path : 0u);
+  std::memcpy(b, &h, sizeof h);
   for (uint32_t j = m; j < g.ex_rows; ++j) ex[j] = 0;
   for (uint32_t k = 0; k < rows; ++k) {
     const TxRow x{(int64_t)(tb.tx_nuc[r.j1 + k] - r.T0), (int64_t)(tb.tx_pep[r.j1 + k] - r.Q0)};
@@ -79,16 +84,18 @@
 
 using namespace magot;
 
-extern "C" int magot_debug_tile_blocks(const uint64_t* ex_g, const uint64_t* ex_out,
-                                       const uint64_t* tx_nuc, const uint64_t* tx_pep,
-                                       uint64_t span, uint32_t lane_chunks, const void* tiles,
-                                       uint64_t n_tiles, uint32_t* geometry, void* blocks,
-                                       uint64_t* ovf_ex, uint64_t ovf_ex_cap, int64_t* ovf_tx,
-                                       uint64_t ovf_tx_cap, uint64_t* n_ovf) {
+namespace {
+
+int debug_tile_blocks(const char* who, bool path_bits, const uint64_t* ex_g, const uint64_t* ex_out,
+                      const uint64_t* tx_nuc, const uint64_t* tx_pep, uint64_t span,
+                      uint32_t lane_chunks, const void* tiles, uint64_t n_tiles, uint32_t* geometry,
+                      void* blocks, uint64_t* ovf_ex, uint64_t ovf_ex_cap, int64_t* ovf_tx,
+                      uint64_t ovf_tx_cap, uint64_t* n_ovf) {
+  const std::string name(who);
   if (!ex_g || !ex_out || !tx_nuc || !tx_pep || !n_ovf || !geometry || (n_tiles && !tiles) ||
-      geometry[0] > kBlkExMax || geometry[1] > kBlkTxMax ||
-      (lane_chunks != (uint32_t)kLaneChunksLarge && lane_chunks != (uint32_t)kLaneChunksSmall)) {
-    set_error("magot_debug_tile_blocks: bad argument");
+      geometry[0] > kBlkExMax || geometry[1] > kBlkTxMax || lane_chunks > (uint32_t)kLaneChunksMax ||
+      !lane_chunks_ok((int)lane_chunks)) {
+    set_error(name + ": bad argument");
     return MAGOT_ERR_ARG;
   }
   const TileRec* tr = static_cast<const TileRec*>(tiles);
@@ -97,7 +104,7 @@
     if (tr[t].e2 < tr[t].e1 || tr[t].j2 < tr[t].j1 || m > (uint64_t)kExonCap ||
         nt > (uint64_t)kTxCap || tr[t].T1 - tr[t].T0 > 0xFFFFull ||
         tr[t].Q1 - tr[t].Q0 > 0xFFFFull) {
-      set_error("magot_debug_tile_blocks: tile " + std::to_string(t) + " out of range");
+      set_error(name + ": tile " + std::to_string(t) + " out of range");
       return MAGOT_ERR_RANGE;
     }
   }
@@ -115,10 +122,10 @@
   if (!blocks) return MAGOT_OK;
   if (ne > ovf_ex_cap || nx > ovf_tx_cap || (ne && !ovf_ex) || (nx && !ovf_tx) ||
       ne > 0xFFFFFFFFull || nx > 0xFFFFFFFFull) {
-    set_error("magot_debug_tile_blocks: overflow arrays too small");
+    set_error(name + ": overflow arrays too small");
     return MAGOT_ERR_ARG;
   }
-  const TileTables tb{ex_g, ex_out, tx_nuc, tx_pep, span, lane_chunks};
+  const TileTables tb{ex_g, ex_out, tx_nuc, tx_pep, span, lane_chunks, path_bits};
   uint64_t oe = 0, ot = 0;
   for (uint64_t t = 0; t < n_tiles; ++t) {
     pack_tile_block(tb, g, tr[t], (uint32_t)oe, (uint32_t)ot,
@@ -129,3 +136,27 @@
   }
   return MAGOT_OK;
 }
+
+}
+
+extern "C" int magot_debug_tile_blocks(const uint64_t* ex_g, const uint64_t* ex_out,
+                                       const uint64_t* tx_nuc, const uint64_t* tx_pep,
+                                       uint64_t span, uint32_t lane_chunks, const void* tiles,
+                                       uint64_t n_tiles, uint32_t* geometry, void* blocks,
+                                       uint64_t* ovf_ex, uint64_t ovf_ex_cap, int64_t* ovf_tx,
+                                       uint64_t ovf_tx_cap, uint64_t* n_ovf) {
+  return debug_tile_blocks("magot_debug_tile_blocks", false, ex_g, ex_out, tx_nuc, tx_pep, span,
+                           lane_chunks, tiles, n_tiles, geometry, blocks, ovf_ex, ovf_ex_cap, ovf_tx,
+                           ovf_tx_cap, n_ovf);
+}
+
+extern "C" int magot_debug_plan_blocks(const uint64_t* ex_g, const uint64_t* ex_out,
+                                       const uint64_t* tx_nuc, const uint64_t* tx_pep,
+                                       uint64_t span, uint32_t lane_chunks, const void* tiles,
+                                       uint64_t n_tiles, uint32_t* geometry, void* blocks,
+                                       uint64_t* ovf_ex, uint64_t ovf_ex_cap, int64_t* ovf_tx,
+                                       uint64_t ovf_tx_cap, uint64_t* n_ovf) {
+  return debug_tile_blocks("magot_debug_plan_blocks", true, ex_g, ex_out, tx_nuc, tx_pep, span,
+                           lane_chunks, tiles, n_tiles, geometry, blocks, ovf_ex, ovf_ex_cap, ovf_tx,
+                           ovf_tx_cap, n_ovf);
+}
diff --git a/magot_amd/csrc/tileplan.cpp b/magot_amd/csrc/tileplan.cpp
--- a/magot_amd/csrc/tileplan.cpp
+++ b/magot_amd/csrc/tileplan.cpp
@@ -206,8 +206,10 @@
 }
 
 int cut_tiles(const uint64_t* ex_out, uint64_t Ec, const uint64_t* tn, const uint64_t* tp,
-              uint64_t Tc, uint64_t tile, std::vector<TileRec>* tiles) {
+              uint64_t Tc, int lane_chunks, std::vector<TileRec>* tiles) {
   const uint64_t B = ex_out[Ec], P = tp[Tc];
+  const uint64_t tile = (uint64_t)tile_bytes(lane_chunks);
+  const uint64_t res_cap = (uint64_t)pep_slots(lane_chunks) * kChunk;
   auto pcount = [&](Cursor& c, uint64_t T) -> uint64_t {
     const uint64_t j = c(T);
     if (j == 0) return 0;
@@ -235,7 +237,7 @@
     if (T1 < B) {
       R1 = std::min<uint64_t>((pcount(c_end, T1) + kChunk - 1) & ~(uint64_t)(kChunk - 1), P);
       R1 = std::min<uint64_t>(R1, pcount(c_dec, dec_end - 2));
-      R1 = std::min<uint64_t>(R1, (R0 & ~(uint64_t)(kChunk - 1)) + kPepSlots * kChunk);
+      R1 = std::min<uint64_t>(R1, (R0 & ~(uint64_t)(kChunk - 1)) + res_cap);
     }
     if (R1 < R0) R1 = R0;
     if (e2 < e1) e2 = e1;
@@ -265,14 +267,15 @@
   auto cut = [&](int lane_chunks) {
     p->lane_chunks = (uint32_t)lane_chunks;
     p->tiles.clear();
-    return cut_tiles(p->ex_out.data(), p->Ec, p->tn.data(), p->tp.data(), p->Tc,
-                     tile_bytes(lane_chunks), &p->tiles);
+    return cut_tiles(p->ex_out.data(), p->Ec, p->tn.data(), p->tp.data(), p->Tc, lane_chunks,
+                     &p->tiles);
   };
+  if (lane_chunks_ok(opt.lane_chunks)) return cut(opt.lane_chunks);
   if (int rc = cut(kLaneChunksLarge)) return rc;
-  if (opt.lane_chunks == kLaneChunksSmall ||
-      (opt.lane_chunks != kLaneChunksLarge && (opt.outputs & MAGOT_OUT_PEP) &&
-       p->tiles.size() < kSmallTilePlan))
+  if ((opt.outputs & MAGOT_OUT_PEP) && p->tiles.size() < kSmallTilePlan)
     return cut(kLaneChunksSmall);
+  if (kLaneChunksHuge != kLaneChunksLarge && p->tiles.size() >= kHugeTilePlan)
+    return cut(kLaneChunksHuge);
   return MAGOT_OK;
 }
 
@@ -286,7 +289,7 @@
     for (uint64_t t = t0; t < t1; ++t) {
       bool slow = false;
       for (uint32_t e = cut[t].e1; e < cut[t].e2 && !slow; ++e)
-        slow = (ex_g[e] & kSlowLitBit) || ex_out[e + 1] - ex_out[e] < (uint64_t)kChunk;
+        slow = tile_interval_slow(ex_g[e], ex_out[e + 1] - ex_out[e]);
       slow_tile[t] = slow;
     }
   });
@@ -302,7 +305,9 @@
   p->ovf_at.resize(2 * n);
   for (uint64_t t = 0; t < n; ++t) {
     const TileRec& r = p->tiles[t];
-    if (r.T1 - r.T0 > 0xFFFFull || r.Q1 - r.Q0 > 0xFFFFull) {
+    const bool res = r.j2 > r.j1;
+    if (r.T1 - r.T0 > 0xFFFFull || r.Q1 - r.Q0 > 0xFFFFull ||
+        (res && (r.Q0 - p->tp[r.j1] > 0x7FFFFFFFull || p->tp[r.j2] - r.Q0 > 0x7FFFFFFFull))) {
       set_error("magot_plan_create: internal tiling error (tile block fields)");
       return MAGOT_ERR_STATE;
     }
@@ -376,13 +381,13 @@
 extern "C" int magot_debug_tile_cut(const uint64_t* ex_out, uint64_t n_ex, const uint64_t* tx_nuc,
                                     const uint64_t* tx_pep, uint64_t n_rec, uint32_t lane_chunks,
                                     void* tiles, uint64_t tiles_cap, uint64_t* n_tiles) {
-  if (!ex_out || !tx_nuc || !tx_pep || !n_tiles ||
-      (lane_chunks != (uint32_t)kLaneChunksLarge && lane_chunks != (uint32_t)kLaneChunksSmall)) {
+  if (!ex_out || !tx_nuc || !tx_pep || !n_tiles || lane_chunks > (uint32_t)kLaneChunksMax ||
+      !lane_chunks_ok((int)lane_chunks)) {
     set_error("magot_debug_tile_cut: bad argument");
     return MAGOT_ERR_ARG;
   }
   std::vector<TileRec> cut;
-  if (int rc = cut_tiles(ex_out, n_ex, tx_nuc, tx_pep, n_rec, tile_bytes((int)lane_chunks), &cut))
+  if (int rc = cut_tiles(ex_out, n_ex, tx_nuc, tx_pep, n_rec, (int)lane_chunks, &cut))
     return rc;
   *n_tiles = cut.size();
   if (!tiles) return MAGOT_OK;
```
